# pixray/pixray

Hardware: AMD Instinct MI355X
Metric: optimisation iters/sec, VQGAN 256^2 + ViT-B/32 + 64 cutouts (higher is better)
Workload: dtype fp16

## Files before the change

### include/prx.h

```cpp
#ifndef PRX_H_
#define PRX_H_
#include <stddef.h>
#include <stdint.h>

#ifdef __cplusplus
extern "C" {
#endif

#define PRX_ABI_VERSION 3

typedef void* prx_stream_t;

const char* prx_last_error(void);
int prx_abi_version(void);
int prx_device_info(int* cu_count, char* arch_name, int arch_name_len);


#define PRX_ACT_NONE 0
#define PRX_ACT_QUICKGELU 1
#define PRX_ACT_MUL_DQUICKGELU 2
#define PRX_ACT_RELU 3
#define PRX_ACT_MUL_RELUMASK 4
#define PRX_ACT_RELUMASK_POST 5
#define PRX_ACT_GELU 6
// ... 38 lines not shown
long long prx_gemm_row_launches(void);

int prx_k_groupnorm_fwd(const float* x, const float* gamma, const float* beta, double* stats, void* out_bf16,
                        float* out_f32, int NB, int P, int C, int swish, float eps, prx_stream_t s);
int prx_k_groupnorm_bwd(const float* g, const float* x, const float* gamma, const float* beta, const double* fstats,
                        double* bstats, const float* add, float* dx, int NB, int P, int C, int swish, float eps,
                        prx_stream_t s);
int prx_k_layernorm_fwd(const float* x, long long ldx, const float* gamma, const float* beta, void* out_bf16,
                        float* out_f32, float* mean, float* rstd, int rows, int C, float eps, prx_stream_t s);
int prx_k_layernorm_bwd(const float* g, long long ldg, const float* x, long long ldx, const float* gamma,
                        const float* mean, const float* rstd, const float* add, long long ldadd, float* dx,
                        long long lddx, int rows, int C, prx_stream_t s);
int prx_k_transpose_bf16(const void* in, int ldin, void* out, int ldout, int R, int C, prx_stream_t s);
int prx_k_softmax_rows(const float* S, int lds_, float scale, void* P, int ldp, void* PT, int ldpt, int rows, int cols,
                       prx_stream_t s);
int prx_k_softmax_rows_bwd(const void* P, int ldp, const float* dP, int lddp, float scale, void* dS, int ldds,
                           void* dST, int lddst, int rows, int cols, prx_stream_t s);
int prx_k_upsample2x_bwd(const float* hi, float* low, int NB, int Hl, int Wl, int C, prx_stream_t s);
int prx_k_nchw_to_nhwc(const float* in, float* out_f32, void* out_bf16, int NB, int C, int HW, int Cpad,
                       prx_stream_t s);
int prx_k_nhwc_to_nchw(const float* in, int ldc, float* out, int NB, int C, int HW, prx_stream_t s);
int prx_k_image_head_fwd(const float* x, int ldc, float* img, int NB, int C, int HW, prx_stream_t s);
int prx_k_image_head_bwd(const float* x, int ldc, const float* gimg, float* dx, void* dx_bf16, int ldo, int NB, int C,
                         int HW, prx_stream_t s);
int prx_k_mha_fwd(const void* qkv, void* out, int N, int T, int C, int heads, prx_stream_t s);
int prx_k_mha_bwd(const void* qkv, const void* dout, void* dqkv, int N, int T, int C, int heads, prx_stream_t s);

int prx_k_groupnorm_fwd_op(const void* x, const float* gamma, const float* beta, double* stats, void* out16, float* out_f32,
                           int NB, int P, int C, int swish, float eps, int zero_stats, int stats_ready, int h16, int s16,
                           prx_stream_t s);
int prx_k_groupnorm_bwd_op(const void* g, const void* x, const float* gamma, const float* beta, const double* fstats,
                           double* bstats, const void* add, float* dx, void* dx16, int NB, int P, int C, int swish, float eps,
                           int zero_stats, int stats_ready, int h16, int s16, prx_stream_t s);
int prx_k_layernorm_fwd_op(const void* x, long long ldx, const float* gamma, const float* beta, void* out16, float* out_f32,
                           float* mean, float* rstd, int rows, int C, float eps, int h16, int s16, prx_stream_t s);
int prx_k_layernorm_bwd_op(const void* g, long long ldg, const void* x, long long ldx, const float* gamma, const float* mean,
                           const float* rstd, const void* add, long long ldadd, float* dx, long long lddx, void* dx16,
                           long long lddxb, int rows, int C, int h16, int add_every, int s16, prx_stream_t s);
int prx_k_mha_fwd_op(const void* qkv, void* out, int N, int T, int C, int heads, int h16, prx_stream_t s);
int prx_k_mha_bwd_op(const void* qkv, const void* dout, void* dqkv, int N, int T, int C, int heads, int h16, prx_stream_t s);
int prx_k_mha_fwd_gen_op(const void* qkv, void* out, float* lse, int N, int T, int C, int heads, int h16, prx_stream_t s);
int prx_k_mha_bwd_gen_op(const void* qkv, const void* out, const void* dout, const float* lse, void* dqkv, int N, int T, int C,
                         int heads, int h16, prx_stream_t s);
int prx_k_mha_fwd_hd_op(const void* qkv, void* out, float* lse, int N, int T, int C, int heads, int h16, int head_cols, prx_stream_t s);
int prx_k_mha_bwd_hd_op(const void* qkv, const void* out, const void* dout, const float* lse, void* dqkv, int N, int T, int C,
                        int heads, int h16, int head_cols, prx_stream_t s);
int prx_k_vit_pad_heads(const float* qkv_w, float* qkv_w_pad, const float* out_w, float* out_w_pad, int width, int heads, int hd, int hp,
                        prx_stream_t s);
int prx_k_mha_fwd_causal_op(const void* qkv, void* out, int N, int T, int C, int heads, int h16, prx_stream_t s);
int prx_k_softmax_rows_op(const float* S, int lds_, float scale, void* P, int ldp, void* PT, int ldpt, int rows, int cols,
                          int prec, prx_stream_t s);
int prx_k_softmax_rows_bwd_op(const void* P, int ldp, const float* dP, int lddp, float scale, void* dS, int ldds, void* dST,
                              int lddst, int rows, int cols, int prec, prx_stream_t s);
int prx_k_transpose_op(const void* in, int ldin, void* out, int ldout, int R, int C, int f32, prx_stream_t s);
int prx_k_upsample2x_bwd_op(const void* hi, float* low, void* low16, int NB, int Hl, int Wl, int C, int h16, int s16,
                            prx_stream_t s);
int prx_k_nchw_to_nhwc_op(const float* in, float* out_f32, void* out16, int NB, int C, int HW, int Cpad, int h16, prx_stream_t s);
int prx_k_image_head_bwd_op(const float* x, int ldc, const float* gimg, float* dx, void* dx16, int ldo, int NB, int C, int HW,
                            int h16, const float* gscale, prx_stream_t s);
int prx_k_image_head_bwd_im2col(const float* x, int ldc, const float* gimg, void* col, int ldk, int C, int H, int W, int h16,
                                const float* gscale, prx_stream_t s);
int prx_k_grad_scale(const float* g, size_t n, float* part, int nparts, int target_log2, float* scale2, prx_stream_t s);
int prx_k_grad_scale_multi(const float* const* gs, const size_t* ns, int count, float* part, int nparts_each, int target_log2,
                           float* scale2, prx_stream_t s);
int prx_k_scale_dev(float* x, size_t n, const float* scale, void* out16, int h16, prx_stream_t s);
int prx_k_f32_to_op16(const float* in, void* out16, size_t n, int h16, prx_stream_t s);
int prx_k_add_f32(const float* a, const float* b, float* out, size_t n, prx_stream_t s);

int prx_k_rn_pack_conv3x3(const float* w, void* Wf, void* Wd, int Cout, int Cin, int prec, prx_stream_t s);
int prx_k_stem1_fwd(const float* cut, const float* mm, const float* w, const float* b, void* out, int N, int S, int CO, int prec,
                    prx_stream_t s);
int prx_k_stem1_bwd(const void* g, const float* w, float* dY, int N, int S, int CO, const float* oscale_dev, int prec, prx_stream_t s);
int prx_k_avgpool2_fwd(const void* x, void* out, int N, int H, int W, int C, int prec, prx_stream_t s);
int prx_k_avgpool2_bwd(const float* g, const void* mask, float* dx_f32, void* dx_op, int N, int H, int W, int C, int prec,
                       prx_stream_t s);
int prx_k_relu_mask(float* g, const void* out, void* g_op, size_t n, int prec, prx_stream_t s);
int prx_k_tokens_fwd(const float* x, const float* pos, void* t, int N, int P, int C, int prec, prx_stream_t s);
int prx_k_tokens_bwd(const float* dt, float* dx, int N, int P, int C, int prec, prx_stream_t s);
int prx_k_tok0_gather(const void* t, void* out, int N, int T, int C, int prec, prx_stream_t s);
int prx_k_tok0_scatter(const void* g0, void* dt, int N, int T, int C, int prec, prx_stream_t s);
int prx_k_minmax(const float* x, size_t n, float* part, int nparts, float* mm, prx_stream_t s);
int prx_k_patchify_fwd(const float* cut, const float* mm, void* A, int prec, int N, int S, int P, int T, float m0, float m1, float m2,
                       float s0, float s1, float s2, prx_stream_t s);
int prx_k_patchify_bwd_reduce(const float* cut, const float* mm, const float* dA, double* acc, int N, int S, int P, int T, float m0,
                              float m1, float m2, float s0, float s1, float s2, prx_stream_t s);
int prx_k_patchify_bwd_apply(const float* cut, const float* mm, const float* dA, const double* acc, float* gcut, int N, int S, int P,
                             int T, float m0, float m1, float m2, float s0, float s1, float s2, prx_stream_t s);
int prx_k_preproc_bwd_reduce(const float* cut, const float* mm, const float* dY, double* acc, int N, int S, prx_stream_t s);
int prx_k_preproc_bwd_apply(const float* cut, const float* mm, const float* dY, const double* acc, float* gcut, int N, int S,
                            prx_stream_t s);
int prx_k_pool_fwd(const float* img, float* pooled, int* argmax, const unsigned char* mask, int C, int H, int W, int S, prx_stream_t s);
int prx_k_pool_bwd(const float* g, const int* argmax, const unsigned char* mask, float* gimg, int C, int H, int W, int S, prx_stream_t s);
int prx_k_rescale_fwd(const float* pooled, float* base, int C, int S, int Hb, int Wb, prx_stream_t s);
int prx_k_rescale_bwd(const float* g_base, float* g_pooled, int C, int S, int Hb, int Wb, prx_stream_t s);
int prx_k_warp_a_fwd(const float* src, int Hs, int Ws, const double* desc, float* out, int n_cut, int Ha, int Wa, prx_stream_t s);
// ... 323 lines not shown
```

### pixray_amd/csrc/api_kernels.hip

```cpp
#include "common.h"
#include "norms.h"
#include "elementwise.h"
#include "attention.h"
#include "resnet.h"
#include "cutouts.h"
#include "vgg.h"
#include "vit.h"
#include "clip_text.h"
#include "prompt_vq.h"
#include "vqgan.h"
#include "vqgan_enc.h"
#include "../../include/prx.h"

#define S_(x) ((hipStream_t)(x))
#define B_(x) ((bf16_t*)(x))
#define CB_(x) ((const bf16_t*)(x))

extern "C" {

int prx_k_groupnorm_fwd(const float* x, const float* gamma, const float* beta, double* stats, void* out_bf16,
                        float* out_f32, int NB, int P, int C, int swish, float eps, prx_stream_t s) {
    return prx_groupnorm_fwd(x, gamma, beta, stats, B_(out_bf16), out_f32, NB, P, C, swish, eps, S_(s));
}
int prx_k_groupnorm_bwd(const float* g, const float* x, const float* gamma, const float* beta, const double* fstats,
// ... 42 lines not shown
    return prx_mha_fwd(CB_(qkv), B_(out), N, T, C, heads, S_(s));
}
int prx_k_mha_bwd(const void* qkv, const void* dout, void* dqkv, int N, int T, int C, int heads, prx_stream_t s) {
    return prx_mha_bwd(CB_(qkv), CB_(dout), B_(dqkv), N, T, C, heads, S_(s));
}

int prx_k_mha_fwd_gen(const void* qkv, void* out, float* lse, int N, int T, int C, int heads, prx_stream_t s) {
    return prx_mha_fwd_gen(CB_(qkv), B_(out), lse, N, T, C, heads, S_(s));
}
int prx_k_mha_bwd_gen(const void* qkv, const void* out, const void* dout, const float* lse, void* dqkv, int N, int T, int C,
                      int heads, prx_stream_t s) {
    return prx_mha_bwd_gen(CB_(qkv), CB_(out), CB_(dout), lse, B_(dqkv), N, T, C, heads, S_(s));
}

int prx_k_mha_fwd_f32(const float* qkv, float* out, float* lse, int N, int T, int C, int heads, prx_stream_t s) {
    return prx_mha_fwd_f32(qkv, out, lse, N, T, C, heads, S_(s));
}
int prx_k_mha_bwd_f32(const float* qkv, const float* out, const float* dout, const float* lse, float* dqkv, int N, int T, int C,
                      int heads, prx_stream_t s) {
    return prx_mha_bwd_f32(qkv, out, dout, lse, dqkv, N, T, C, heads, S_(s));
}

int prx_k_groupnorm_fwd_op(const void* x, const float* gamma, const float* beta, double* stats, void* out16, float* out_f32,
                           int NB, int P, int C, int swish, float eps, int zero_stats, int stats_ready, int h16, int s16,
                           prx_stream_t s) {
    return prx_groupnorm_fwd(x, gamma, beta, stats, B_(out16), out_f32, NB, P, C, swish, eps, S_(s), zero_stats, stats_ready, h16, s16);
}
int prx_k_groupnorm_bwd_op(const void* g, const void* x, const float* gamma, const float* beta, const double* fstats,
                           double* bstats, const void* add, float* dx, void* dx16, int NB, int P, int C, int swish, float eps,
                           int zero_stats, int stats_ready, int h16, int s16, prx_stream_t s) {
    return prx_groupnorm_bwd(g, x, gamma, beta, fstats, bstats, add, dx, B_(dx16), NB, P, C, swish, eps, S_(s), zero_stats,
                             stats_ready, h16, s16);
}
int prx_k_layernorm_fwd_op(const void* x, long long ldx, const float* gamma, const float* beta, void* out16, float* out_f32,
                           float* mean, float* rstd, int rows, int C, float eps, int h16, int s16, prx_stream_t s) {
    return prx_layernorm_fwd(x, ldx, gamma, beta, B_(out16), out_f32, mean, rstd, rows, C, eps, S_(s), h16, s16);
}
int prx_k_layernorm_bwd_op(const void* g, long long ldg, const void* x, long long ldx, const float* gamma, const float* mean,
                           const float* rstd, const void* add, long long ldadd, float* dx, long long lddx, void* dx16,
                           long long lddxb, int rows, int C, int h16, int add_every, int s16, prx_stream_t s) {
    return prx_layernorm_bwd(g, ldg, x, ldx, gamma, mean, rstd, add, ldadd, dx, lddx, B_(dx16), lddxb, rows, C, S_(s), h16,
                             add_every, s16);
}
int prx_k_mha_fwd_op(const void* qkv, void* out, int N, int T, int C, int heads, int h16, prx_stream_t s) {
    return prx_mha_fwd(CB_(qkv), B_(out), N, T, C, heads, S_(s), h16);
}
int prx_k_mha_bwd_op(const void* qkv, const void* dout, void* dqkv, int N, int T, int C, int heads, int h16, prx_stream_t s) {
    return prx_mha_bwd(CB_(qkv), CB_(dout), B_(dqkv), N, T, C, heads, S_(s), h16);
}
int prx_k_mha_fwd_gen_op(const void* qkv, void* out, float* lse, int N, int T, int C, int heads, int h16, prx_stream_t s) {
    return prx_mha_fwd_gen(CB_(qkv), B_(out), lse, N, T, C, heads, S_(s), h16);
}
int prx_k_mha_bwd_gen_op(const void* qkv, const void* out, const void* dout, const float* lse, void* dqkv, int N, int T, int C,
                         int heads, int h16, prx_stream_t s) {
    return prx_mha_bwd_gen(CB_(qkv), CB_(out), CB_(dout), lse, B_(dqkv), N, T, C, heads, S_(s), h16);
}
int prx_k_mha_fwd_hd_op(const void* qkv, void* out, float* lse, int N, int T, int C, int heads, int h16, int head_cols, prx_stream_t s) {
    PRX_REQUIRE(head_cols == 64 || head_cols == 96, "mha_fwd_hd: %d columns per head (64 | 96)", head_cols);
    if (head_cols == 64) return prx_mha_fwd_gen(CB_(qkv), B_(out), lse, N, T, C, heads, S_(s), h16);
    return prx_mha_fwd_hd96(CB_(qkv), B_(out), lse, N, T, C, heads, 1.f / sqrtf(80.f), S_(s), h16);
}
int prx_k_mha_bwd_hd_op(const void* qkv, const void* out, const void* dout, const float* lse, void* dqkv, int N, int T, int C,
                        int heads, int h16, int head_cols, prx_stream_t s) {
    PRX_REQUIRE(head_cols == 64 || head_cols == 96, "mha_bwd_hd: %d columns per head (64 | 96)", head_cols);
    if (head_cols == 64) return prx_mha_bwd_gen(CB_(qkv), CB_(out), CB_(dout), lse, B_(dqkv), N, T, C, heads, S_(s), h16);
    return prx_mha_bwd_hd96(CB_(qkv), CB_(out), CB_(dout), lse, B_(dqkv), N, T, C, heads, 1.f / sqrtf(80.f), S_(s), h16);
}
int prx_k_vit_pad_heads(const float* qkv_w, float* qkv_w_pad, const float* out_w, float* out_w_pad, int width, int heads, int hd, int hp,
                        prx_stream_t s) {
    PRX_REQUIRE(qkv_w && qkv_w_pad && out_w && out_w_pad && width == heads * hd, "vit_pad_heads: null argument or width != heads * head dim");
    int r = prx_vit_pad_head_rows(qkv_w, qkv_w_pad, heads, hd, hp, width, S_(s));
    return r ? r : prx_vit_pad_head_cols(out_w, out_w_pad, width, heads, hd, hp, S_(s));
}
int prx_k_mha_fwd_causal_op(const void* qkv, void* out, int N, int T, int C, int heads, int h16, prx_stream_t s) {
    return prx_mha_fwd_causal(CB_(qkv), B_(out), N, T, C, heads, S_(s), h16);
}
int prx_k_softmax_rows_op(const float* S, int lds_, float scale, void* P, int ldp, void* PT, int ldpt, int rows, int cols,
                          int prec, prx_stream_t s) {
    PRX_REQUIRE(prec_valid(prec), "softmax_rows: unknown precision %d", prec);
    return prx_softmax_rows(S, lds_, scale, P, ldp, PT, ldpt, rows, cols, prec, S_(s));
}
int prx_k_softmax_rows_bwd_op(const void* P, int ldp, const float* dP, int lddp, float scale, void* dS, int ldds, void* dST,
                              int lddst, int rows, int cols, int prec, prx_stream_t s) {
    PRX_REQUIRE(prec_valid(prec), "softmax_rows_bwd: unknown precision %d", prec);
    return prx_softmax_rows_bwd(P, ldp, dP, lddp, scale, dS, ldds, dST, lddst, rows, cols, prec, S_(s));
}
int prx_k_transpose_op(const void* in, int ldin, void* out, int ldout, int R, int C, int f32, prx_stream_t s) {
    return prx_transpose_op(in, ldin, out, ldout, R, C, f32, S_(s));
}
int prx_k_upsample2x_bwd_op(const void* hi, float* low, void* low16, int NB, int Hl, int Wl, int C, int h16, int s16,
                            prx_stream_t s) {
    return prx_upsample2x_bwd(hi, low, B_(low16), NB, Hl, Wl, C, S_(s), h16, s16);
}
int prx_k_nchw_to_nhwc_op(const float* in, float* out_f32, void* out16, int NB, int C, int HW, int Cpad, int h16, prx_stream_t s) {
    return prx_nchw_to_nhwc(in, out_f32, B_(out16), NB, C, HW, Cpad, S_(s), h16);
}
int prx_k_image_head_bwd_op(const float* x, int ldc, const float* gimg, float* dx, void* dx16, int ldo, int NB, int C, int HW,
                            int h16, const float* gscale, prx_stream_t s) {
    return prx_image_head_bwd(x, ldc, gimg, dx, B_(dx16), ldo, NB, C, HW, S_(s), h16, gscale);
}
int prx_k_image_head_bwd_im2col(const float* x, int ldc, const float* gimg, void* col, int ldk, int C, int H, int W, int h16,
                                const float* gscale, prx_stream_t s) {
    return prx_image_head_bwd_im2col(x, ldc, gimg, B_(col), ldk, C, H, W, S_(s), h16, gscale);
}
int prx_k_grad_scale(const float* g, size_t n, float* part, int nparts, int target_log2, float* scale2, prx_stream_t s) {
    return prx_grad_scale(g, n, part, nparts, target_log2, scale2, S_(s));
}
int prx_k_grad_scale_multi(const float* const* gs, const size_t* ns, int count, float* part, int nparts_each, int target_log2,
                           float* scale2, prx_stream_t s) {
    return prx_grad_scale_multi(gs, ns, count, part, nparts_each, target_log2, scale2, S_(s));
}
int prx_k_scale_dev(float* x, size_t n, const float* scale, void* out16, int h16, prx_stream_t s) {
    return prx_scale_dev(x, n, scale, S_(s), B_(out16), h16);
}
int prx_k_f32_to_op16(const float* in, void* out16, size_t n, int h16, prx_stream_t s) {
    return prx_f32_to_bf16(in, B_(out16), n, S_(s), h16);
}
int prx_k_add_f32(const float* a, const float* b, float* out, size_t n, prx_stream_t s) {
    return prx_add_f32(a, b, out, n, S_(s));
}

int prx_k_rn_pack_conv3x3(const float* w, void* Wf, void* Wd, int Cout, int Cin, int prec, prx_stream_t s) {
    return prx_rn_pack_conv3x3(w, Wf, Wd, Cout, Cin, prec, S_(s));
}
int prx_k_stem1_fwd(const float* cut, const float* mm, const float* w, const float* b, void* out, int N, int S, int CO, int prec, prx_stream_t s) {
    return prx_stem1_fwd(cut, mm, w, b, out, N, S, CO, prec, S_(s));
}
int prx_k_stem1_bwd(const void* g, const float* w, float* dY, int N, int S, int CO, const float* oscale_dev, int prec, prx_stream_t s) {
    return prx_stem1_bwd(g, w, dY, N, S, CO, oscale_dev, prec, S_(s));
}
int prx_k_avgpool2_fwd(const void* x, void* out, int N, int H, int W, int C, int prec, prx_stream_t s) {
    return prx_avgpool2_fwd(x, out, N, H, W, C, prec, S_(s));
}
int prx_k_avgpool2_bwd(const float* g, const void* mask, float* dx_f32, void* dx_op, int N, int H, int W, int C, int prec, prx_stream_t s) {
    return prx_avgpool2_bwd(g, mask, dx_f32, dx_op, N, H, W, C, prec, S_(s));
}
int prx_k_relu_mask(float* g, const void* out, void* g_op, size_t n, int prec, prx_stream_t s) {
    return prx_relu_mask(g, out, g_op, n, prec, S_(s));
}
int prx_k_tokens_fwd(const float* x, const float* pos, void* t, int N, int P, int C, int prec, prx_stream_t s) {
// ... 125 lines not shown
```

### pixray_amd/csrc/attention.h

```cpp
#pragma once
#include "common.h"
int prx_mha_fwd(const bf16_t* qkv, bf16_t* out, int N, int T, int C, int heads, hipStream_t s, int h16 = 0);
int prx_mha_bwd(const bf16_t* qkv, const bf16_t* dout, bf16_t* dqkv, int N, int T, int C, int heads, hipStream_t s, int h16 = 0);
int prx_mha_fwd_gen(const bf16_t* qkv, bf16_t* out, float* lse, int N, int T, int C, int heads, hipStream_t s, int h16 = 0);
int prx_mha_bwd_gen(const bf16_t* qkv, const bf16_t* out, const bf16_t* dout, const float* lse, bf16_t* dqkv, int N, int T,
                    int C, int heads, hipStream_t s, int h16 = 0);
int prx_mha_fwd_causal(const bf16_t* qkv, bf16_t* out, int N, int T, int C, int heads, hipStream_t s, int h16 = 0);
int prx_mha_fwd_f32(const float* qkv, float* out, float* lse, int N, int T, int C, int heads, hipStream_t s);
int prx_mha_bwd_f32(const float* qkv, const float* out, const float* dout, const float* lse, float* dqkv, int N, int T, int C,
                    int heads, hipStream_t s);
int prx_mha_fwd_hd96(const bf16_t* qkv, bf16_t* out, float* lse, int N, int T, int C, int heads, float scale, hipStream_t s, int h16 = 0);
int prx_mha_bwd_hd96(const bf16_t* qkv, const bf16_t* out, const bf16_t* dout, const float* lse, bf16_t* dqkv, int N, int T, int C,
                     int heads, float scale, hipStream_t s, int h16 = 0);
int prx_mha_fwd_f32_hd96(const float* qkv, float* out, float* lse, int N, int T, int C, int heads, hipStream_t s);
int prx_mha_bwd_f32_hd96(const float* qkv, const float* out, const float* dout, const float* lse, float* dqkv, int N, int T, int C,
                         int heads, hipStream_t s);
```

### pixray_amd/csrc/attention.hip

```cpp
#include "attention.h"
#include <stdlib.h>
#include <atomic>

constexpr int MHA_BLK_MAX_T = 640;
static std::atomic<int> g_mha_route{-1};
extern "C" int prx_mha_route(int route) { return g_mha_route.exchange(route < 0 ? -1 : (route ? 1 : 0)); }
static bool prx_mha_blk_route(int T) {
    static const bool env_tiles = [] { const char* e = getenv("PRX_MHA_TILES"); return e && e[0] == '1'; }();
    const int route = g_mha_route.load(std::memory_order_relaxed);
    return T <= MHA_BLK_MAX_T && route != 1 && !(route < 0 && env_tiles);
}

#define A16_NS att_bf16
#define a16_t bf16_t
#define a16x8 bf16x8
#define a16x4 bf16x4
#define A16_MFMA __builtin_amdgcn_mfma_f32_32x32x16_bf16
#include "attention_kernels.inc"
#undef A16_NS
#undef a16_t
#undef a16x8
#undef a16x4
#undef A16_MFMA

#define A16_NS att_f16
#define a16_t half_t
#define a16x8 f16x8
#define a16x4 f16x4
#define A16_MFMA __builtin_amdgcn_mfma_f32_32x32x16_f16
#include "attention_kernels.inc"
#undef A16_NS
#undef a16_t
#undef a16x8
#undef a16x4
#undef A16_MFMA

#define H(p) reinterpret_cast<const half_t*>(p)
#define HM(p) reinterpret_cast<half_t*>(p)
int prx_mha_fwd(const bf16_t* qkv, bf16_t* out, int N, int T, int C, int heads, hipStream_t s, int h16) {
    return h16 ? att_f16::mha_fwd(H(qkv), HM(out), N, T, C, heads, s) : att_bf16::mha_fwd(qkv, out, N, T, C, heads, s);
}
int prx_mha_bwd(const bf16_t* qkv, const bf16_t* dout, bf16_t* dqkv, int N, int T, int C, int heads, hipStream_t s, int h16) {
    return h16 ? att_f16::mha_bwd(H(qkv), H(dout), HM(dqkv), N, T, C, heads, s) : att_bf16::mha_bwd(qkv, dout, dqkv, N, T, C, heads, s);
}
int prx_mha_fwd_gen(const bf16_t* qkv, bf16_t* out, float* lse, int N, int T, int C, int heads, hipStream_t s, int h16) {
    return h16 ? att_f16::mha_fwd_gen(H(qkv), HM(out), lse, N, T, C, heads, s) : att_bf16::mha_fwd_gen(qkv, out, lse, N, T, C, heads, s);
}
int prx_mha_fwd_causal(const bf16_t* qkv, bf16_t* out, int N, int T, int C, int heads, hipStream_t s, int h16) {
    return h16 ? att_f16::mha_fwd_causal(H(qkv), HM(out), N, T, C, heads, s) : att_bf16::mha_fwd_causal(qkv, out, N, T, C, heads, s);
}
int prx_mha_bwd_gen(const bf16_t* qkv, const bf16_t* out, const bf16_t* dout, const float* lse, bf16_t* dqkv, int N, int T,
                    int C, int heads, hipStream_t s, int h16) {
    return h16 ? att_f16::mha_bwd_gen(H(qkv), H(out), H(dout), lse, HM(dqkv), N, T, C, heads, s)
               : att_bf16::mha_bwd_gen(qkv, out, dout, lse, dqkv, N, T, C, heads, s);
}
```

### pixray_amd/csrc/attention_kernels.inc

```
namespace A16_NS {
namespace {

constexpr int LD = 72;
constexpr int TILE = 64 * LD;

__device__ __forceinline__ float half_max(float v) {
#pragma unroll
    for (int o = 16; o > 0; o >>= 1) v = fmaxf(v, __shfl_xor(v, o, 64));
    return v;
}
__device__ __forceinline__ float half_sum(float v) {
#pragma unroll
    for (int o = 16; o > 0; o >>= 1) v += __shfl_xor(v, o, 64);
    return v;
}

__device__ __forceinline__ void mma_64x64x64(const a16_t* A, const a16_t* B, f32x16 (&acc)[2][2], int lane) {
    const int fr = lane & 31, fk = 8 * (lane >> 5);
#pragma unroll
    for (int ks = 0; ks < 4; ++ks) {
        a16x8 a[2], b[2];
#pragma unroll
        for (int i = 0; i < 2; ++i) {
            a[i] = *reinterpret_cast<const a16x8*>(&A[(i * 32 + fr) * LD + ks * 16 + fk]);
            b[i] = *reinterpret_cast<const a16x8*>(&B[(i * 32 + fr) * LD + ks * 16 + fk]);
        }
#pragma unroll
        for (int i = 0; i < 2; ++i)
#pragma unroll
            for (int j = 0; j < 2; ++j) acc[i][j] = A16_MFMA(a[i], b[j], acc[i][j], 0, 0, 0);
    }
}

__device__ __forceinline__ void zero_acc(f32x16 (&acc)[2][2]) {
#pragma unroll
    for (int i = 0; i < 2; ++i)
#pragma unroll
        for (int j = 0; j < 2; ++j)
#pragma unroll
            for (int r = 0; r < 16; ++r) acc[i][j][r] = 0.f;
}

__device__ __forceinline__ int tr_swz(int d) { return (((d >> 4) & 1) * 12) ^ (((d >> 5) & 1) * 16); }

__device__ __forceinline__ void tile_get(const a16_t* src, long long ld, int T, int tid, a16x8 (&v)[4]) {
#pragma unroll
    for (int i = 0; i < 4; ++i) {
        const int c = tid + 128 * i;
        const int row = c >> 3, kc = c & 7;
        const a16x8 z = {0, 0, 0, 0, 0, 0, 0, 0};
        const a16x8 x = *reinterpret_cast<const a16x8*>(src + (long long)(row < T ? row : T - 1) * ld + kc * 8);
        v[i] = row < T ? x : z;
    }
}
__device__ __forceinline__ void tile_put(const a16x8 (&v)[4], a16_t* dst, a16_t* dstT, int tid) {
#pragma unroll
    for (int i = 0; i < 4; ++i) {
        const int c = tid + 128 * i;
        const int row = c >> 3, kc = c & 7;
        if (dst) *reinterpret_cast<a16x8*>(&dst[row * LD + kc * 8]) = v[i];
        if (dstT) {
#pragma unroll
            for (int e = 0; e < 8; ++e) dstT[(kc * 8 + e) * LD + (row ^ tr_swz(kc * 8))] = v[i][e];
        }
    }
}

__device__ __forceinline__ void mma_64x32x64(const a16_t* A, const a16_t* B, int nb, f32x16 (&acc)[2], int lane) {
    const int fr = lane & 31, fk = 8 * (lane >> 5);
#pragma unroll
    for (int ks = 0; ks < 4; ++ks) {
        const a16x8 b = *reinterpret_cast<const a16x8*>(&B[(nb * 32 + fr) * LD + ks * 16 + fk]);
#pragma unroll
        for (int i = 0; i < 2; ++i) {
            const a16x8 a = *reinterpret_cast<const a16x8*>(&A[(i * 32 + fr) * LD + ks * 16 + fk]);
            acc[i] = A16_MFMA(a, b, acc[i], 0, 0, 0);
        }
    }
}
__device__ __forceinline__ void zero_acc2(f32x16 (&acc)[2]) {
#pragma unroll
    for (int i = 0; i < 2; ++i)
#pragma unroll
        for (int r = 0; r < 16; ++r) acc[i][r] = 0.f;
}
// ... 107 lines not shown
        float m = -INFINITY;
#pragma unroll
        for (int mi = 0; mi < 2; ++mi)
#pragma unroll
            for (int r = 0; r < 16; ++r) {
                const int j = mi * 32 + (r & 3) + 8 * (r >> 2) + 4 * hh;
                const float v = (j < T) ? st[mi][r] * scale : -INFINITY;
                st[mi][r] = v;
                m = fmaxf(m, v);
            }
        m = fmaxf(m, __shfl_xor(m, 32, 64));
        float sum = 0.f;
#pragma unroll
        for (int mi = 0; mi < 2; ++mi)
#pragma unroll
            for (int r = 0; r < 16; ++r) {
                const float e = __expf(st[mi][r] - m);
                st[mi][r] = e;
                sum += e;
            }
        sum += __shfl_xor(sum, 32, 64);
        const float inv = 1.f / sum;
#pragma unroll
        for (int mi = 0; mi < 2; ++mi)
#pragma unroll
            for (int r = 0; r < 16; ++r) st[mi][r] *= inv;
    }
    f32x16 o[2];
    zero_acc2(o);
    mma_acc_tr(st, Vt, o, lane);
    store_rows_global(o, w, out + (long long)n * T * C + h * 64, C, T, lane);
}

__global__ __launch_bounds__(128) void mha_bwd_kernel(const a16_t* __restrict__ qkv, const a16_t* __restrict__ dout,
                                                      a16_t* __restrict__ dqkv, int T, int C, float scale, int xcd) {
    __shared__ __attribute__((aligned(16))) a16_t smem[5 * TILE];
    __shared__ __attribute__((aligned(16))) float s_lse[64], s_D[64];
    a16_t* Qs = smem;
    a16_t* Ks = smem + TILE;
    a16_t* Vs = smem + 2 * TILE;
    a16_t* dOs = smem + 3 * TILE;
    a16_t* Tt = smem + 4 * TILE;
    const int tid = threadIdx.x, lane = tid & 63, w = tid >> 6;
    const unsigned flat = blockIdx.y * gridDim.x + blockIdx.x, nwg = gridDim.x * gridDim.y;
    const unsigned lin = xcd ? xcd_linear(flat, nwg) : flat;
    const int h = (int)(lin % gridDim.x), n = (int)(lin / gridDim.x);
    const int hh = lane >> 5;
    const long long ld = 3LL * C;
    const a16_t* base = qkv + (long long)n * T * ld + h * 64;
    const a16_t* dobase = dout + (long long)n * T * C + h * 64;
    a16x8 tq[4], tdo[4];
    {
        a16x8 tk[4], tv[4];
        tile_get(base, ld, T, tid, tq);
        tile_get(base + C, ld, T, tid, tk);
        tile_get(base + 2 * C, ld, T, tid, tv);
        tile_get(dobase, C, T, tid, tdo);
        tile_put(tq, Qs, nullptr, tid);
        tile_put(tk, Ks, Tt, tid);
        tile_put(tv, Vs, nullptr, tid);
        tile_put(tdo, dOs, nullptr, tid);
    }
    __syncthreads();
    a16_t* obase = dqkv + (long long)n * T * ld + h * 64;
    {
        f32x16 pt[2], dpt[2];
        zero_acc2(pt);
        mma_64x32x64(Ks, Qs, w, pt, lane);
        zero_acc2(dpt);
        mma_64x32x64(Vs, dOs, w, dpt, lane);
        float m = -INFINITY;
#pragma unroll
        for (int mi = 0; mi < 2; ++mi)
#pragma unroll
            for (int r = 0; r < 16; ++r) {
                const int j = mi * 32 + (r & 3) + 8 * (r >> 2) + 4 * hh;
                const float v = (j < T) ? pt[mi][r] * scale : -INFINITY;
                pt[mi][r] = v;
                m = fmaxf(m, v);
            }
        m = fmaxf(m, __shfl_xor(m, 32, 64));
        float sum = 0.f;
#pragma unroll
        for (int mi = 0; mi < 2; ++mi)
#pragma unroll
            for (int r = 0; r < 16; ++r) {
                const float e = __expf(pt[mi][r] - m);
                pt[mi][r] = e;
                sum += e;
            }
// ... 560 lines not shown
            for (int rg = 0; rg < 4; ++rg) {
                const int i0 = sb * 32 + 8 * rg + 4 * hh;
                const float4 l4 = *reinterpret_cast<const float4*>(&s_lse[i0]);
                const float4 d4 = *reinterpret_cast<const float4*>(&s_D[i0]);
                const float lv[4] = {l4.x, l4.y, l4.z, l4.w}, dvv[4] = {d4.x, d4.y, d4.z, d4.w};
#pragma unroll
                for (int qq = 0; qq < 4; ++qq) {
                    const int r = rg * 4 + qq;
                    const float pv = key_ok ? __builtin_amdgcn_exp2f(p[r] * sl2 - lv[qq]) : 0.f;
                    p[r] = pv;
                    dp[r] = scale * pv * (dp[r] - dvv[qq]);
                }
            }
            mma_acc_tr_chunk(dp, Qt, sb, dk, lane);
            mma_acc_tr_chunk(p, dOt, sb, dv, lane);
        }
    }
    if (!active) return;
    a16_t* obase = dqkv + (long long)n * T * ld + h * 64;
    store_rows_global(dk, w, obase + C, ld, T, lane);
    store_rows_global(dv, w, obase + 2 * C, ld, T, lane);
}

}


inline int mha_fwd(const a16_t* qkv, a16_t* out, int N, int T, int C, int heads, hipStream_t s) {
    PRX_REQUIRE(T <= 64 && C == heads * 64, "mha: needs T <= 64 and head dim 64 (T=%d C=%d heads=%d)", T, C, heads);
    hipLaunchKernelGGL(mha_fwd_kernel, dim3(heads, N), dim3(128), 0, s, qkv, out, T, C, 0.125f, prx_xcd_local());
    PRX_LAUNCH_CHECK();
    return 0;
}

inline int mha_bwd(const a16_t* qkv, const a16_t* dout, a16_t* dqkv, int N, int T, int C, int heads, hipStream_t s) {
    PRX_REQUIRE(T <= 64 && C == heads * 64, "mha bwd: needs T <= 64 and head dim 64 (T=%d C=%d heads=%d)", T, C, heads);
    hipLaunchKernelGGL(mha_bwd_kernel, dim3(heads, N), dim3(128), 0, s, qkv, dout, dqkv, T, C, 0.125f, prx_xcd_local());
    PRX_LAUNCH_CHECK();
    return 0;
}

inline int mha_fwd_gen(const a16_t* qkv, a16_t* out, float* lse, int N, int T, int C, int heads, hipStream_t s) {
    PRX_REQUIRE(C == heads * 64 && T >= 1, "mha(gen): needs head dim 64 (T=%d C=%d heads=%d)", T, C, heads);
    if (prx_mha_blk_route(T)) {
        const int nw = ceil_div(T, 32), nsplit = ceil_div(nw, 5), wpb = ceil_div(nw, nsplit);
        hipLaunchKernelGGL(mha_fwd_blk_kernel, dim3(heads, N, nsplit), dim3(64 * wpb), 0, s, qkv, out, lse, T, C, heads, 0.125f, prx_xcd_local());
        PRX_LAUNCH_CHECK();
        return 0;
    }
    hipLaunchKernelGGL(mha_fwd_gen_kernel<false>, dim3(ceil_div(T, 64), heads, N), dim3(64), 0, s, qkv, out, lse, T, C, heads, 0.125f);
    PRX_LAUNCH_CHECK();
    return 0;
}
inline int mha_fwd_causal(const a16_t* qkv, a16_t* out, int N, int T, int C, int heads, hipStream_t s) {
    PRX_REQUIRE(C == heads * 64 && T >= 1, "mha(causal): needs head dim 64 (T=%d C=%d heads=%d)", T, C, heads);
    hipLaunchKernelGGL(mha_fwd_gen_kernel<true>, dim3(ceil_div(T, 64), heads, N), dim3(64), 0, s, qkv, out, (float*)nullptr, T, C, heads,
                       0.125f);
    PRX_LAUNCH_CHECK();
    return 0;
}
inline int mha_bwd_gen(const a16_t* qkv, const a16_t* out, const a16_t* dout, const float* lse, a16_t* dqkv, int N, int T,
                    int C, int heads, hipStream_t s) {
    PRX_REQUIRE(C == heads * 64 && T >= 1, "mha(gen) bwd: needs head dim 64 (T=%d C=%d heads=%d)", T, C, heads);
    if (prx_mha_blk_route(T)) {
        const int nw = ceil_div(T, 32), nsplit = ceil_div(nw, 5), wpb = ceil_div(nw, nsplit);
        const dim3 g(heads, N, nsplit), b(64 * wpb);
        const int xcd = prx_xcd_local();
        hipLaunchKernelGGL(mha_bwd_dq_blk_kernel, g, b, 0, s, qkv, out, dout, lse, dqkv, T, C, heads, 0.125f, xcd);
        PRX_LAUNCH_CHECK();
        hipLaunchKernelGGL(mha_bwd_dkv_blk_kernel, g, b, 0, s, qkv, out, dout, lse, dqkv, T, C, heads, 0.125f, xcd);
// ... 13 lines not shown
```

### pixray_amd/csrc/common.h

```cpp
#pragma once
#include <hip/hip_runtime.h>
#include <stdint.h>

typedef __bf16 bf16_t;
typedef _Float16 half_t;
typedef __attribute__((ext_vector_type(8))) _Float16 f16x8;
typedef __attribute__((ext_vector_type(4))) _Float16 f16x4;
typedef __attribute__((ext_vector_type(8))) __bf16 bf16x8;
typedef __attribute__((ext_vector_type(4))) __bf16 bf16x4;
typedef __attribute__((ext_vector_type(2))) __bf16 bf16x2;
typedef __attribute__((ext_vector_type(16))) float f32x16;
typedef __attribute__((ext_vector_type(4))) float f32x4;

#define PRX_WAVE 64

enum { PRX_PREC_BF16 = 0, PRX_PREC_F32 = 1, PRX_PREC_F16 = 2 };
static inline int prec_is_f32(int precision) { return precision == PRX_PREC_F32; }
static inline int prec_is_h16(int precision) { return precision == PRX_PREC_F16; }
static inline bool prec_valid(int precision) { return precision >= PRX_PREC_BF16 && precision <= PRX_PREC_F16; }
static inline size_t op_esz(int f32) { return f32 ? 4 : 2; }
static inline void* op_off(void* p, size_t elems, int f32) { return p ? (char*)p + elems * op_esz(f32) : nullptr; }
static inline const void* op_off(const void* p, size_t elems, int f32) { return p ? (const char*)p + elems * op_esz(f32) : nullptr; }

void prx_set_error(const char* fmt, ...);
// ... 110 lines not shown
template <> __device__ __forceinline__ void op_st4<float>(float* p, size_t i, float a, float b, float c, float d) {
    *reinterpret_cast<float4*>(p + i) = make_float4(a, b, c, d);
}

__device__ __forceinline__ float wave_sum(float v) {
#pragma unroll
    for (int o = 32; o > 0; o >>= 1) v += __shfl_xor(v, o, 64);
    return v;
}
__device__ __forceinline__ float wave_max(float v) {
#pragma unroll
    for (int o = 32; o > 0; o >>= 1) v = fmaxf(v, __shfl_xor(v, o, 64));
    return v;
}
__device__ __forceinline__ float wave_min(float v) {
#pragma unroll
    for (int o = 32; o > 0; o >>= 1) v = fminf(v, __shfl_xor(v, o, 64));
    return v;
}
__device__ __forceinline__ double wave_sum_d(double v) {
#pragma unroll
    for (int o = 32; o > 0; o >>= 1) v += __shfl_xor(v, o, 64);
    return v;
}

__device__ __forceinline__ float sigmoidf_(float x) { return 1.f / (1.f + __expf(-x)); }

__device__ __forceinline__ unsigned xcd_linear(unsigned bid, unsigned nwg) {
    const unsigned xcd = bid & 7u, local = bid >> 3, q = nwg >> 3, r = nwg & 7u;
    return (xcd < r ? xcd * (q + 1) : r * (q + 1) + (xcd - r) * q) + local;
}
int prx_xcd_local();
int prx_grad_target_log2();

static inline int ceil_div(int a, int b) { return (a + b - 1) / b; }
static inline long long ceil_div_ll(long long a, long long b) { return (a + b - 1) / b; }
```

### pixray_amd/csrc/elementwise.h

```cpp
#pragma once
#include "common.h"
int prx_transpose_op(const void* in, int ldin, void* out, int ldout, int R, int C, int f32, hipStream_t s);
int prx_softmax_rows(const float* S, int lds_, float scale, void* P, int ldp, void* PT, int ldpt, int rows,
                     int cols, int prec, hipStream_t s);
int prx_softmax_rows_bwd(const void* P, int ldp, const float* dP, int lddp, float scale, void* dS, int ldds,
                         void* dST, int lddst, int rows, int cols, int prec, hipStream_t s);
int prx_upsample2x_bwd(const void* hi, float* low, bf16_t* low_bf16, int NB, int Hl, int Wl, int C, hipStream_t s, int h16 = 0, int s16 = 0);
int prx_nchw_to_nhwc(const float* in, float* out_f32, bf16_t* out_bf16, int NB, int C, int HW, int Cpad, hipStream_t s, int h16 = 0);
int prx_nhwc_to_nchw(const float* in, int ldc, float* out, int NB, int C, int HW, hipStream_t s);
int prx_image_head_fwd(const float* x, int ldc, float* img, int NB, int C, int HW, hipStream_t s);
int prx_image_head_bwd(const float* x, int ldc, const float* gimg, float* dx, bf16_t* dx_bf16, int ldo, int NB, int C,
                       int HW, hipStream_t s, int h16 = 0, const float* gscale = nullptr);
int prx_image_head_bwd_im2col(const float* x, int ldc, const float* gimg, bf16_t* col, int ldk, int C, int H, int W, hipStream_t s, int h16 = 0,
                              const float* gscale = nullptr);
int prx_grad_scale(const float* g, size_t n, float* part, int nparts, int target_log2, float* scale2, hipStream_t s);
int prx_adam_clamp(float* z, float* m, float* v, const float* g, const float* zmin, const float* zmax, int hw,
                   size_t n, float lr, float b1, float b2, float eps, int step, hipStream_t s);
int prx_adam_clamp_dev(float* z, float* m, float* v, const float* g, const float* zmin, const float* zmax, int hw,
                       size_t n, const float* hyper, float b1, float b2, float eps, hipStream_t s);
int prx_f32_to_bf16(const float* in, bf16_t* out, size_t n, hipStream_t s, int h16 = 0);
int prx_grad_scale_multi(const float* const* gs, const size_t* ns, int count, float* part, int nparts_each, int target_log2,
                         float* scale2, hipStream_t s);
int prx_add_f32(const float* a, const float* b, float* out, size_t n, hipStream_t s);
int prx_scale_dev(float* x, size_t n, const float* scale, hipStream_t s, bf16_t* out16 = nullptr, int h16 = 0);
```

### pixray_amd/csrc/elementwise.hip

```cpp
#include "elementwise.h"
#include <algorithm>

namespace {

inline int ew_grid(size_t total, int per = 256) { return (int)std::min<size_t>((total + per - 1) / per, 8192); }

template <typename T>
__global__ __launch_bounds__(256) void transpose_op_kernel(const T* __restrict__ in, int ldin,
                                                           T* __restrict__ out, int ldout, int R, int C) {
    __shared__ T tile[32][33];
    const int tx = threadIdx.x & 31, ty = threadIdx.x >> 5;
    const int r0 = blockIdx.y * 32, c0 = blockIdx.x * 32;
#pragma unroll
    for (int i = 0; i < 4; ++i) {
        int r = r0 + ty + 8 * i, c = c0 + tx;
        tile[ty + 8 * i][tx] = (r < R && c < C) ? in[(size_t)r * ldin + c] : (T)0.f;
    }
    __syncthreads();
#pragma unroll
    for (int i = 0; i < 4; ++i) {
        int c = c0 + ty + 8 * i, r = r0 + tx;
        if (c < C && r < R) out[(size_t)c * ldout + r] = tile[tx][ty + 8 * i];
    }
}
// ... 185 lines not shown
        }
        z[i] = zi;
    }
}

__global__ __launch_bounds__(256) void f32_to_bf16_kernel(const float* __restrict__ in, bf16_t* __restrict__ out,
                                                          size_t n, int h16) {
    for (size_t i = (size_t)blockIdx.x * blockDim.x + threadIdx.x; i < n; i += (size_t)gridDim.x * blockDim.x)
        out[i] = to_op16(in[i], h16);
}

__global__ __launch_bounds__(256) void amax_partial_kernel(const float* __restrict__ g, size_t n, float* __restrict__ part) {
    float m = 0.f;
    for (size_t i = (size_t)blockIdx.x * blockDim.x + threadIdx.x; i < n; i += (size_t)gridDim.x * blockDim.x) {
        const float a = fabsf(g[i]);
        m = fmaxf(m, a == a ? a : INFINITY);
    }
    m = wave_max(m);
    __shared__ float s[4];
    if ((threadIdx.x & 63) == 0) s[threadIdx.x >> 6] = m;
    __syncthreads();
    if (threadIdx.x == 0) part[blockIdx.x] = fmaxf(fmaxf(s[0], s[1]), fmaxf(s[2], s[3]));
}
__global__ __launch_bounds__(256) void grad_scale_final_kernel(const float* __restrict__ part, int nparts, int target_log2,
                                                               float* __restrict__ scale2) {
    float m = 0.f;
    for (int i = threadIdx.x; i < nparts; i += blockDim.x) m = fmaxf(m, part[i]);
    m = wave_max(m);
    __shared__ float s[4];
    if ((threadIdx.x & 63) == 0) s[threadIdx.x >> 6] = m;
    __syncthreads();
    if (threadIdx.x == 0) {
        m = fmaxf(fmaxf(s[0], s[1]), fmaxf(s[2], s[3]));
        float S = 1.f;
        if (m > 0.f && m < INFINITY) {
            int e;
            (void)frexpf(m, &e);
            int k = target_log2 - e;
            k = k < -40 ? -40 : (k > 60 ? 60 : k);
            S = ldexpf(1.f, k);
        }
        scale2[0] = S;
        scale2[1] = 1.f / S;
    }
}

__global__ __launch_bounds__(256) void scale_dev_kernel(float* __restrict__ x, size_t n, const float* __restrict__ scale, bf16_t* __restrict__ out16, int h16) {
    const float sc = *scale;
    for (size_t i = (size_t)blockIdx.x * blockDim.x + threadIdx.x; i < n; i += (size_t)gridDim.x * blockDim.x) {
        const float v = x[i] * sc;
        x[i] = v;
        if (out16) out16[i] = to_op16(v, h16);
    }
}

__global__ __launch_bounds__(256) void add_f32_kernel(const float* __restrict__ a, const float* __restrict__ b,
                                                      float* __restrict__ out, size_t n) {
    for (size_t i = (size_t)blockIdx.x * blockDim.x + threadIdx.x; i < n; i += (size_t)gridDim.x * blockDim.x)
        out[i] = a[i] + b[i];
}

}

int prx_transpose_op(const void* in, int ldin, void* out, int ldout, int R, int C, int f32, hipStream_t s) {
    dim3 grid(ceil_div(C, 32), ceil_div(R, 32));
    if (f32) hipLaunchKernelGGL(transpose_op_kernel<float>, grid, dim3(256), 0, s, (const float*)in, ldin, (float*)out, ldout, R, C);
    else     hipLaunchKernelGGL(transpose_op_kernel<bf16_t>, grid, dim3(256), 0, s, (const bf16_t*)in, ldin, (bf16_t*)out, ldout, R, C);
    PRX_LAUNCH_CHECK();
    return 0;
}
int prx_softmax_rows(const float* S, int lds_, float scale, void* P, int ldp, void* PT, int ldpt, int rows,
                     int cols, int prec, hipStream_t s) {
    PRX_OP_DISPATCH(prec_is_f32(prec), prec_is_h16(prec), T,
                    hipLaunchKernelGGL(softmax_rows_kernel<T>, dim3(ceil_div(rows, 4)), dim3(256), 0, s, S, lds_, scale, (T*)P, ldp,
// ... 7 lines not shown
                    hipLaunchKernelGGL(softmax_rows_bwd_kernel<T>, dim3(ceil_div(rows, 4)), dim3(256), 0, s, (const T*)P, ldp, dP, lddp,
                                       scale, (T*)dS, ldds, (T*)dST, lddst, rows, cols));
    PRX_LAUNCH_CHECK();
    return 0;
}
int prx_upsample2x_bwd(const void* hi, float* low, bf16_t* low_bf16, int NB, int Hl, int Wl, int C, hipStream_t s, int h16, int s16) {
    PRX_REQUIRE(C % 4 == 0 && (low || low_bf16), "upsample2x_bwd: C %% 4 != 0, or no output");
    if (s16) hipLaunchKernelGGL(upsample2x_bwd_kernel<true>, dim3(ew_grid((size_t)NB * Hl * Wl * C / 4)), dim3(256), 0, s, hi, low, low_bf16,
                                NB, Hl, Wl, C, h16);
    else hipLaunchKernelGGL(upsample2x_bwd_kernel<false>, dim3(ew_grid((size_t)NB * Hl * Wl * C / 4)), dim3(256), 0, s, hi, low, low_bf16,
                            NB, Hl, Wl, C, h16);
    PRX_LAUNCH_CHECK();
    return 0;
}
int prx_nchw_to_nhwc(const float* in, float* out_f32, bf16_t* out_bf16, int NB, int C, int HW, int Cpad,
                     hipStream_t s, int h16) {
    hipLaunchKernelGGL(nchw_to_nhwc_kernel, dim3(ew_grid((size_t)NB * HW * Cpad)), dim3(256), 0, s, in, out_f32,
                       out_bf16, NB, C, HW, Cpad, h16);
    PRX_LAUNCH_CHECK();
    return 0;
}
int prx_nhwc_to_nchw(const float* in, int ldc, float* out, int NB, int C, int HW, hipStream_t s) {
    hipLaunchKernelGGL(nhwc_to_nchw_kernel, dim3(ew_grid((size_t)NB * HW * C)), dim3(256), 0, s, in, ldc, out, NB, C,
                       HW);
    PRX_LAUNCH_CHECK();
    return 0;
}
int prx_image_head_fwd(const float* x, int ldc, float* img, int NB, int C, int HW, hipStream_t s) {
    hipLaunchKernelGGL(image_head_fwd_kernel, dim3(ew_grid((size_t)NB * HW * C)), dim3(256), 0, s, x, ldc, img, NB, C,
                       HW);
    PRX_LAUNCH_CHECK();
    return 0;
}
int prx_grad_scale(const float* g, size_t n, float* part, int nparts, int target_log2, float* scale2, hipStream_t s) {
    PRX_REQUIRE(nparts >= 1 && nparts <= 1024, "grad_scale: 1..1024 partials");
    const int blocks = (int)std::min<size_t>((n + 1023) / 1024 + 1, (size_t)nparts);
    hipLaunchKernelGGL(amax_partial_kernel, dim3(blocks), dim3(256), 0, s, g, n, part);
    PRX_LAUNCH_CHECK();
    hipLaunchKernelGGL(grad_scale_final_kernel, dim3(1), dim3(256), 0, s, part, blocks, target_log2, scale2);
    PRX_LAUNCH_CHECK();
    return 0;
}
int prx_grad_scale_multi(const float* const* gs, const size_t* ns, int count, float* part, int nparts_each, int target_log2,
                         float* scale2, hipStream_t s) {
    PRX_REQUIRE(count >= 1 && nparts_each >= 1 && (long long)count * nparts_each <= 4096, "grad_scale_multi: bad partial layout");
    int used = 0;
    for (int i = 0; i < count; ++i) {
        if (!gs[i] || ns[i] == 0) continue;
        const int blocks = (int)std::min<size_t>((ns[i] + 1023) / 1024 + 1, (size_t)nparts_each);
        hipLaunchKernelGGL(amax_partial_kernel, dim3(blocks), dim3(256), 0, s, gs[i], ns[i], part + used);
        PRX_LAUNCH_CHECK();
        used += blocks;
    }
    PRX_REQUIRE(used > 0, "grad_scale_multi: no gradient tensor");
    hipLaunchKernelGGL(grad_scale_final_kernel, dim3(1), dim3(256), 0, s, part, used, target_log2, scale2);
    PRX_LAUNCH_CHECK();
    return 0;
}
int prx_scale_dev(float* x, size_t n, const float* scale, hipStream_t s, bf16_t* out16, int h16) {
    hipLaunchKernelGGL(scale_dev_kernel, dim3(ew_grid(n)), dim3(256), 0, s, x, n, scale, out16, h16);
    PRX_LAUNCH_CHECK();
    return 0;
}
int prx_image_head_bwd(const float* x, int ldc, const float* gimg, float* dx, bf16_t* dx_bf16, int ldo, int NB, int C,
                       int HW, hipStream_t s, int h16, const float* gscale) {
    hipLaunchKernelGGL(image_head_bwd_kernel, dim3(ew_grid((size_t)NB * HW * ldo)), dim3(256), 0, s, x, ldc, gimg, dx,
                       dx_bf16, ldo, NB, C, HW, h16, gscale);
    PRX_LAUNCH_CHECK();
    return 0;
// ... 38 lines not shown
```

### pixray_amd/csrc/norms.h

```cpp
#pragma once
#include "common.h"
#include <algorithm>
int prx_groupnorm_fwd(const void* x, const float* gamma, const float* beta, double* stats, bf16_t* out_bf16,
                      float* out_f32, int NB, int P, int C, int swish, float eps, hipStream_t s, int zero_stats = 1,
                      int stats_ready = 0, int h16 = 0, int s16 = 0);
int prx_groupnorm_bwd(const void* g, const void* x, const float* gamma, const float* beta, const double* fstats,
                      double* bstats, const void* add, float* dx, bf16_t* dx_bf16, int NB, int P, int C, int swish,
                      float eps, hipStream_t s, int zero_stats = 1, int stats_ready = 0, int h16 = 0, int s16 = 0);
int prx_groupnorm_bwd_stats(const float* g, const float* x, const float* gamma, const float* beta, const double* fstats,
                            double* bstats, int NB, int P, int C, int swish, float eps, hipStream_t s);
int prx_layernorm_fwd(const void* x, long long ldx, const float* gamma, const float* beta, bf16_t* out_bf16,
                      float* out_f32, float* mean, float* rstd, int rows, int C, float eps, hipStream_t s, int h16 = 0, int s16 = 0,
                      int ragged = 0);
int prx_layernorm_bwd(const void* g, long long ldg, const void* x, long long ldx, const float* gamma,
                      const float* mean, const float* rstd, const void* add, long long ldadd, float* dx,
                      long long lddx, bf16_t* dx_bf16, long long lddxb, int rows, int C, hipStream_t s, int h16 = 0,
                      int add_every = 0, int s16 = 0, int ragged = 0);
```

### pixray_amd/csrc/norms.hip

```cpp
#include "norms.h"

namespace {

struct GNArgs {
    const void* x;
    const void* g;
    const double* fstats;
    const float* gamma;
    const float* beta;
    double* stats;
    int P, C, swish;
    float eps;
    int s16, h16;
};

__device__ __forceinline__ void gn_mean_rstd(const double* st, double n, float eps, float& mean, float& rstd) {
    double m = st[0] / n;
    double var = st[1] / n - m * m;
    if (var < 0) var = 0;
    mean = (float)m;
    rstd = (float)(1.0 / sqrt(var + (double)eps));
}

__device__ __forceinline__ float swish_grad(float y) {
// ... 154 lines not shown
    L.ga = reinterpret_cast<const float4*>(a.gamma)[cq];
    L.be = reinterpret_cast<const float4*>(a.beta)[cq];
    gn_lane_load<true>(a, bstats, NB == 1 ? 0 : (int)(i0 / per_b), cq, L);
    auto one = [&](unsigned id, const float4& v, const float4& gg, const float4& ad) {
        if (NB != 1) { const int b = (int)(id / per_b); if (b != L.b) gn_lane_load<true>(a, bstats, b, cq, L); }
        const float xv[4] = {v.x, v.y, v.z, v.w}, gv[4] = {gg.x, gg.y, gg.z, gg.w};
        const float gav[4] = {L.ga.x, L.ga.y, L.ga.z, L.ga.w}, bev[4] = {L.be.x, L.be.y, L.be.z, L.be.w};
        float o[4];
#pragma unroll
        for (int i = 0; i < 4; ++i) {
            float xh = (xv[i] - L.mean) * L.rstd;
            float gy = gv[i];
            if (a.swish) gy *= swish_grad(xh * gav[i] + bev[i]);
            float dxh = gy * gav[i];
            o[i] = L.rstd * (dxh - L.m1 - xh * L.m2);
        }
        o[0] += ad.x; o[1] += ad.y; o[2] += ad.z; o[3] += ad.w;
        if (dx) reinterpret_cast<float4*>(dx)[id] = make_float4(o[0], o[1], o[2], o[3]);
        if (dx_bf16) reinterpret_cast<bf16x4*>(dx_bf16)[id] = to_op16x4(o[0], o[1], o[2], o[3], h16);
    };
    for (; idx + step < i1; idx += 2 * step) {
        const unsigned nx = idx + 2 * step;
        const bool m0 = nx < i1, m1 = nx + step < i1;
        const float4 nv0 = m0 ? stream_ld4<S16>(a.x, nx, a.h16) : z4, ng0 = m0 ? stream_ld4<S16>(a.g, nx, a.h16) : z4;
        const float4 na0 = (m0 && add) ? stream_ld4<S16>(add, nx, a.h16) : z4;
        const float4 nv1 = m1 ? stream_ld4<S16>(a.x, nx + step, a.h16) : z4, ng1 = m1 ? stream_ld4<S16>(a.g, nx + step, a.h16) : z4;
        const float4 na1 = (m1 && add) ? stream_ld4<S16>(add, nx + step, a.h16) : z4;
        one(idx, v0, g0, a0); one(idx + step, v1, g1, a1);
        v0 = nv0; g0 = ng0; a0 = na0; v1 = nv1; g1 = ng1; a1 = na1;
    }
    if (idx < i1) one(idx, v0, g0, a0);
}

template <bool RAG>
__device__ __forceinline__ bool ln_own(int i, int nv, int lane, int C) {
    return RAG ? (i * 64 + lane) * 4 < C : i < nv;
}
template <int MAXV, bool S16, bool RAG = false>
__global__ __launch_bounds__(256) void ln_fwd_kernel(const void* __restrict__ x, const float* __restrict__ gamma,
                                                     const float* __restrict__ beta, bf16_t* __restrict__ out_bf16,
                                                     float* __restrict__ out_f32, float* __restrict__ mean_out,
                                                     float* __restrict__ rstd_out, int rows, int C, long long ldx,
                                                     float eps, int xcd, int h16) {
    const int lane = threadIdx.x & 63;
    const int row = (xcd ? xcd_linear(blockIdx.x, gridDim.x) : blockIdx.x) * 4 + (threadIdx.x >> 6);
    if (row >= rows) return;
    const int nv = (C + 255) >> 8;
    const size_t xr4 = (size_t)row * ldx / 4;
    float4 v[MAXV], gav[MAXV], bev[MAXV];
#pragma unroll
    for (int i = 0; i < MAXV; ++i) v[i] = stream_ld4<S16>(x, xr4 + (ln_own<RAG>(i, nv, lane, C) ? i * 64 + lane : (RAG ? 0 : lane)), h16);
#pragma unroll
    for (int i = 0; i < MAXV; ++i) {
        gav[i] = reinterpret_cast<const float4*>(gamma)[(ln_own<RAG>(i, nv, lane, C) ? i * 64 + lane : (RAG ? 0 : lane))];
        bev[i] = reinterpret_cast<const float4*>(beta)[(ln_own<RAG>(i, nv, lane, C) ? i * 64 + lane : (RAG ? 0 : lane))];
    }
    float s = 0.f;
#pragma unroll
    for (int i = 0; i < MAXV; ++i) s += ln_own<RAG>(i, nv, lane, C) ? (v[i].x + v[i].y) + (v[i].z + v[i].w) : 0.f;
    const float mean = wave_sum(s) / (float)C;
    float ss = 0.f;
#pragma unroll
    for (int i = 0; i < MAXV; ++i)
        if (ln_own<RAG>(i, nv, lane, C)) {
            float a0 = v[i].x - mean, a1 = v[i].y - mean, a2 = v[i].z - mean, a3 = v[i].w - mean;
            ss += (a0 * a0 + a1 * a1) + (a2 * a2 + a3 * a3);
        }
    const float var = wave_sum(ss) / (float)C;
    const float rstd = rsqrtf(var + eps);
    if (lane == 0) {
        if (mean_out) mean_out[row] = mean;
        if (rstd_out) rstd_out[row] = rstd;
    }
#pragma unroll
    for (int i = 0; i < MAXV; ++i)
        if (ln_own<RAG>(i, nv, lane, C)) {
            const int c4 = i * 64 + lane;
            const float4 ga = gav[i], be = bev[i];
            float o0 = (v[i].x - mean) * rstd * ga.x + be.x;
            float o1 = (v[i].y - mean) * rstd * ga.y + be.y;
            float o2 = (v[i].z - mean) * rstd * ga.z + be.z;
            float o3 = (v[i].w - mean) * rstd * ga.w + be.w;
            if (out_bf16) {
                reinterpret_cast<bf16x4*>(out_bf16 + (size_t)row * C)[c4] = to_op16x4(o0, o1, o2, o3, h16);
// ... 34 lines not shown
        for (int i = 0; i < MAXV; ++i) {
            xh[i] = make_float4((xv[i].x - mean) * rstd, (xv[i].y - mean) * rstd, (xv[i].z - mean) * rstd, (xv[i].w - mean) * rstd);
            dh[i] = make_float4(gv[i].x * ga[i].x, gv[i].y * ga[i].y, gv[i].z * ga[i].z, gv[i].w * ga[i].w);
        }
    }
    float s1 = 0.f, s2 = 0.f;
#pragma unroll
    for (int i = 0; i < MAXV; ++i) {
        s1 += ln_own<RAG>(i, nv, lane, C) ? (dh[i].x + dh[i].y) + (dh[i].z + dh[i].w) : 0.f;
        s2 += ln_own<RAG>(i, nv, lane, C) ? (dh[i].x * xh[i].x + dh[i].y * xh[i].y) + (dh[i].z * xh[i].z + dh[i].w * xh[i].w) : 0.f;
    }
    const float m1 = wave_sum(s1) / (float)C;
    const float m2 = wave_sum(s2) / (float)C;
#pragma unroll
    for (int i = 0; i < MAXV; ++i)
        if (ln_own<RAG>(i, nv, lane, C)) {
            const int c4 = i * 64 + lane;
            float4 o = make_float4(rstd * (dh[i].x - m1 - xh[i].x * m2), rstd * (dh[i].y - m1 - xh[i].y * m2),
                                   rstd * (dh[i].z - m1 - xh[i].z * m2), rstd * (dh[i].w - m1 - xh[i].w * m2));
            if (add) { o.x += adv[i].x; o.y += adv[i].y; o.z += adv[i].z; o.w += adv[i].w; }
            if (dx) reinterpret_cast<float4*>(dx + (size_t)row * lddx)[c4] = o;
            if (dx_bf16) {
                reinterpret_cast<bf16x4*>(dx_bf16 + (size_t)row * lddxb)[c4] = to_op16x4(o.x, o.y, o.z, o.w, h16);
            }
        }
}

int gn_grid(size_t total) { return (int)std::min<size_t>((total + 255) / 256, 2048); }

}

int prx_groupnorm_fwd(const void* x, const float* gamma, const float* beta, double* stats, bf16_t* out_bf16,
                      float* out_f32, int NB, int P, int C, int swish, float eps, hipStream_t s, int zero_stats,
                      int stats_ready, int h16, int s16) {
    PRX_REQUIRE(C % 32 == 0 && (C / 32) % 4 == 0 && 256 % (C / 4) == 0, "groupnorm: unsupported C=%d", C);
    GNArgs a{};
    a.x = x; a.gamma = gamma; a.beta = beta; a.stats = stats; a.P = P; a.C = C; a.swish = swish; a.eps = eps; a.s16 = s16; a.h16 = h16;
    if (!stats_ready) {
        if (zero_stats) PRX_CHECK_HIP(hipMemsetAsync(stats, 0, sizeof(double) * NB * 64, s));
        const int ppb = 256 / (C / 4);
        int blocks = std::min(ceil_div(P, ppb * 4), 256);
        if (s16) hipLaunchKernelGGL((gn_stats_kernel<0, true>), dim3(blocks, NB), dim3(256), 0, s, a);
        else hipLaunchKernelGGL((gn_stats_kernel<0, false>), dim3(blocks, NB), dim3(256), 0, s, a);
        PRX_LAUNCH_CHECK();
    }
    if (out_bf16 || out_f32) {
        PRX_REQUIRE((unsigned long long)NB * P * C / 4 < (1ull << 31), "groupnorm: %d x %d x %d elements exceed the 32-bit index range", NB, P, C);
        if (s16) hipLaunchKernelGGL(gn_apply_fwd_kernel<true>, dim3(gn_grid((size_t)NB * P * C / 4)), dim3(256), 0, s, a, out_bf16,
                                    out_f32, NB, prx_xcd_local(), h16);
        else hipLaunchKernelGGL(gn_apply_fwd_kernel<false>, dim3(gn_grid((size_t)NB * P * C / 4)), dim3(256), 0, s, a, out_bf16,
                                out_f32, NB, prx_xcd_local(), h16);
        PRX_LAUNCH_CHECK();
    }
    return 0;
}

int prx_groupnorm_bwd_stats(const float* g, const float* x, const float* gamma, const float* beta, const double* fstats,
                            double* bstats, int NB, int P, int C, int swish, float eps, hipStream_t s) {
    PRX_REQUIRE(256 % (C / 4) == 0 && (C / 32) % 4 == 0, "groupnorm bwd: unsupported C=%d", C);
    GNArgs a{};
    a.x = x; a.g = g; a.fstats = fstats; a.gamma = gamma; a.beta = beta; a.stats = bstats;
    a.P = P; a.C = C; a.swish = swish; a.eps = eps; a.s16 = 0; a.h16 = 0;
    const int ppb = 256 / (C / 4);
    int blocks = std::min(ceil_div(P, ppb * 4), 256);
    hipLaunchKernelGGL((gn_stats_kernel<1, false>), dim3(blocks, NB), dim3(256), 0, s, a);
    PRX_LAUNCH_CHECK();
    return 0;
}

int prx_groupnorm_bwd(const void* g, const void* x, const float* gamma, const float* beta, const double* fstats,
                      double* bstats, const void* add, float* dx, bf16_t* dx_bf16, int NB, int P, int C, int swish,
                      float eps, hipStream_t s, int zero_stats, int stats_ready, int h16, int s16) {
    PRX_REQUIRE(256 % (C / 4) == 0 && (C / 32) % 4 == 0, "groupnorm bwd: unsupported C=%d", C);
    GNArgs a{};
    a.x = x; a.g = g; a.fstats = fstats; a.gamma = gamma; a.beta = beta; a.stats = bstats;
    a.P = P; a.C = C; a.swish = swish; a.eps = eps; a.s16 = s16; a.h16 = h16;
    if (!stats_ready) {
        if (zero_stats) PRX_CHECK_HIP(hipMemsetAsync(bstats, 0, sizeof(double) * NB * 64, s));
        const int ppb = 256 / (C / 4);
        int blocks = std::min(ceil_div(P, ppb * 4), 256);
        if (s16) hipLaunchKernelGGL((gn_stats_kernel<1, true>), dim3(blocks, NB), dim3(256), 0, s, a);
        else hipLaunchKernelGGL((gn_stats_kernel<1, false>), dim3(blocks, NB), dim3(256), 0, s, a);
        PRX_LAUNCH_CHECK();
    }
    PRX_REQUIRE((unsigned long long)NB * P * C / 4 < (1ull << 31), "groupnorm bwd: %d x %d x %d elements exceed the 32-bit index range", NB, P, C);
    if (s16) hipLaunchKernelGGL(gn_apply_bwd_kernel<true>, dim3(gn_grid((size_t)NB * P * C / 4)), dim3(256), 0, s, a, bstats, add, dx,
                                dx_bf16, NB, prx_xcd_local(), h16);
    else hipLaunchKernelGGL(gn_apply_bwd_kernel<false>, dim3(gn_grid((size_t)NB * P * C / 4)), dim3(256), 0, s, a, bstats, add, dx,
                            dx_bf16, NB, prx_xcd_local(), h16);
    PRX_LAUNCH_CHECK();
    return 0;
}

int prx_layernorm_fwd(const void* x, long long ldx, const float* gamma, const float* beta, bf16_t* out_bf16,
                      float* out_f32, float* mean, float* rstd, int rows, int C, float eps, hipStream_t s, int h16, int s16, int ragged) {
    PRX_REQUIRE((C % 256 == 0 || (ragged && C % 128 == 0 && C <= 1024)) && C <= 2048 && ldx % 4 == 0,
                "layernorm: C must be a multiple of 256 and <= 2048 (C=%d), ldx a multiple of 4", C);
    dim3 grid(ceil_div(rows, 4));
    if (C % 256 != 0) {
#define PRX_LN_FWD_R(S16) hipLaunchKernelGGL((ln_fwd_kernel<4, S16, true>), grid, dim3(256), 0, s, x, gamma, beta, out_bf16, out_f32, mean, rstd, \
                                             rows, C, ldx, eps, prx_xcd_local(), h16)
        if (s16) PRX_LN_FWD_R(true); else PRX_LN_FWD_R(false);
#undef PRX_LN_FWD_R
        PRX_LAUNCH_CHECK();
        return 0;
    }
#define PRX_LN_FWD(MAXV, S16) hipLaunchKernelGGL((ln_fwd_kernel<MAXV, S16>), grid, dim3(256), 0, s, x, gamma, beta, out_bf16, out_f32, mean, rstd, \
                                                 rows, C, ldx, eps, prx_xcd_local(), h16)
    if (C <= 1024) { if (s16) PRX_LN_FWD(4, true); else PRX_LN_FWD(4, false); }
    else { if (s16) PRX_LN_FWD(8, true); else PRX_LN_FWD(8, false); }
#undef PRX_LN_FWD
    PRX_LAUNCH_CHECK();
    return 0;
}

int prx_layernorm_bwd(const void* g, long long ldg, const void* x, long long ldx, const float* gamma,
                      const float* mean, const float* rstd, const void* add, long long ldadd, float* dx,
                      long long lddx, bf16_t* dx_bf16, long long lddxb, int rows, int C, hipStream_t s, int h16, int add_every, int s16, int ragged) {
    PRX_REQUIRE((C % 256 == 0 || (ragged && C % 128 == 0 && C <= 1024)) && C <= 2048, "layernorm bwd: C must be a multiple of 256 and <= 2048 (C=%d)", C);
    PRX_REQUIRE(ldg % 4 == 0 && ldx % 4 == 0 && ldadd % 4 == 0 && (dx || dx_bf16), "layernorm bwd: leading dimensions must be multiples of 4, one output is needed");
    PRX_REQUIRE(s16 == 0 || s16 == 1 || s16 == 2 || s16 == 7, "layernorm bwd: stream layouts in use are 0, 1 (x), 2 (g), 7 (x, g, add): got %d", s16);
    dim3 grid(ceil_div(rows, 4));
    if (C % 256 != 0) {
#define PRX_LN_BWD_R(S16) hipLaunchKernelGGL((ln_bwd_kernel<4, S16, true>), grid, dim3(256), 0, s, g, ldg, x, ldx, gamma, mean, rstd, add, ldadd, dx, \
                                             lddx, dx_bf16, lddxb, rows, C, prx_xcd_local(), h16, add_every)
        if (s16 == 0) PRX_LN_BWD_R(0); else if (s16 == 1) PRX_LN_BWD_R(1); else if (s16 == 2) PRX_LN_BWD_R(2); else PRX_LN_BWD_R(7);
#undef PRX_LN_BWD_R
        PRX_LAUNCH_CHECK();
        return 0;
    }
#define PRX_LN_BWD(MAXV, S16) hipLaunchKernelGGL((ln_bwd_kernel<MAXV, S16>), grid, dim3(256), 0, s, g, ldg, x, ldx, gamma, mean, rstd, add, ldadd, dx, \
                                                 lddx, dx_bf16, lddxb, rows, C, prx_xcd_local(), h16, add_every)
#define PRX_LN_BWD_S(MAXV) do { if (s16 == 0) PRX_LN_BWD(MAXV, 0); else if (s16 == 1) PRX_LN_BWD(MAXV, 1); else if (s16 == 2) PRX_LN_BWD(MAXV, 2); \
                                else PRX_LN_BWD(MAXV, 7); } while (0)
    if (C <= 1024) PRX_LN_BWD_S(4); else PRX_LN_BWD_S(8);
#undef PRX_LN_BWD_S
#undef PRX_LN_BWD
    PRX_LAUNCH_CHECK();
    return 0;
}
```

### pixray_amd/csrc/prompt_vq.h

```cpp
#pragma once
#include "common.h"
int prx_prompt_loss(const float* x, const float* embed, int n, int m, int D, float weight, float stop, float denom,
                    float* rowloss, float* grad, float* loss, unsigned* ticket, hipStream_t s);
int prx_l2norm_fwd(const float* e, float* out, int n, int D, hipStream_t s);
int prx_l2norm_bwd(const float* e, const float* g, float* de, int n, int D, hipStream_t s);
int prx_sqnorm_rows(const float* w, float* out, int rows, int D, hipStream_t s);
int prx_vq_nearest(const float* z, long long tok_stride, long long ch_stride, const float* codebook, const float* cnorm,
                   int P, int NC, int D, float* pmin, int* pidx, int* idx_out, float* zq, hipStream_t s);
```

### pixray_amd/csrc/prompt_vq.hip

```cpp
#include "prompt_vq.h"
#include <algorithm>

namespace {

__device__ __forceinline__ float prompt_loss_row(const float* __restrict__ x, const float* __restrict__ embed, int i, int lane,
                                                int n, int m, int D, float weight, float stop, float denom,
                                                float* __restrict__ rowloss, float* __restrict__ grad) {
    constexpr int MAXE = 16;
    const int ne = D / 64;
    float xv[MAXE], gacc[MAXE];
    float ss = 0.f;
#pragma unroll
    for (int e = 0; e < MAXE; ++e) xv[e] = x[(size_t)i * D + (e < ne ? e : 0) * 64 + lane];
#pragma unroll
    for (int e = 0; e < MAXE; ++e)
        if (e < ne) { ss += xv[e] * xv[e]; gacc[e] = 0.f; }
    const float xnorm = fmaxf(sqrtf(wave_sum(ss)), 1e-12f);
    const float ixn = 1.f / xnorm;
    const float sgn = (weight > 0.f) ? 1.f : ((weight < 0.f) ? -1.f : 0.f);
    float loss = 0.f;
    for (int j = 0; j < m; ++j) {
        float ev[MAXE];
        float es = 0.f;
#pragma unroll
// ... 46 lines not shown
    if (!last || threadIdx.x >= 64) return;
    __threadfence();
    float t = 0.f;
    for (int r = lane; r < n; r += 64) t += *reinterpret_cast<const volatile float*>(rowloss + r);
    t = wave_sum(t);
    if (lane == 0) *loss_out = t * (fabsf(weight) / denom);
}

__global__ __launch_bounds__(256) void l2norm_fwd_kernel(const float* __restrict__ e, float* __restrict__ out, int n, int D) {
    const int lane = threadIdx.x & 63;
    const int i = blockIdx.x * 4 + (threadIdx.x >> 6);
    if (i >= n) return;
    float ss = 0.f;
    for (int c = lane; c < D; c += 64) { float v = e[(size_t)i * D + c]; ss += v * v; }
    const float inv = 1.f / sqrtf(wave_sum(ss));
    for (int c = lane; c < D; c += 64) out[(size_t)i * D + c] = e[(size_t)i * D + c] * inv;
}
__global__ __launch_bounds__(256) void l2norm_bwd_kernel(const float* __restrict__ e, const float* __restrict__ g,
                                                         float* __restrict__ de, int n, int D) {
    const int lane = threadIdx.x & 63;
    const int i = blockIdx.x * 4 + (threadIdx.x >> 6);
    if (i >= n) return;
    float ss = 0.f, dot = 0.f;
    for (int c = lane; c < D; c += 64) {
        float v = e[(size_t)i * D + c];
        ss += v * v; dot += v * g[(size_t)i * D + c];
    }
    ss = wave_sum(ss); dot = wave_sum(dot);
    const float inv = 1.f / sqrtf(ss);
    for (int c = lane; c < D; c += 64) {
        float v = e[(size_t)i * D + c];
        de[(size_t)i * D + c] = (g[(size_t)i * D + c] - v * dot / ss) * inv;
    }
}

__global__ __launch_bounds__(256) void sqnorm_rows_kernel(const float* __restrict__ w, float* __restrict__ out, int rows, int D) {
    const int lane = threadIdx.x & 63;
    const int i = blockIdx.x * 4 + (threadIdx.x >> 6);
    if (i >= rows) return;
    float ss = 0.f;
    for (int c = lane; c < D; c += 64) { float v = w[(size_t)i * D + c]; ss += v * v; }
    ss = wave_sum(ss);
    if (lane == 0) out[i] = ss;
}

typedef float vq_f32x2 __attribute__((ext_vector_type(2)));
constexpr int VQ_CODES = 128, VQ_CPAD = VQ_CODES + 4;
__global__ __launch_bounds__(256) void vq_dist_kernel(const float* __restrict__ z, long long tok_stride,
                                                      long long ch_stride, const float* __restrict__ codebook,
                                                      const float* __restrict__ cnorm, int P, int NC, int D,
                                                      float* __restrict__ pmin, int* __restrict__ pidx) {
    __shared__ __attribute__((aligned(16))) float Xs[16][64];
    __shared__ __attribute__((aligned(16))) float Cs[16][VQ_CPAD];
    __shared__ float red_v[64][16];
    __shared__ int red_i[64][16];
    const int tid = threadIdx.x;
    const int tx = tid & 15, ty = tid >> 4;
    const int p0 = blockIdx.y * 64, c0 = blockIdx.x * VQ_CODES;
    vq_f32x2 acc[4][4];
    float xn[4] = {0, 0, 0, 0};
#pragma unroll
    for (int i = 0; i < 4; ++i)
#pragma unroll
        for (int j = 0; j < 4; ++j) acc[i][j] = vq_f32x2{0.f, 0.f};
    float xr[4];
    float4 cr[2];
// ... 44 lines not shown
            }
        }
        __syncthreads();
    }
#pragma unroll
    for (int i = 0; i < 4; ++i) {
        float best = INFINITY; int bi = 0x7fffffff;
#pragma unroll
        for (int j = 0; j < 8; ++j) {
            const int c = c0 + (j < 4 ? tx * 4 + j : 64 + tx * 4 + (j - 4));
            if (c < NC) {
                const float a = (j & 1) ? acc[i][j >> 1].y : acc[i][j >> 1].x;
                float d = (xn[i] + cnorm[c]) - 2.f * a;
                if (d < best) { best = d; bi = c; }
            }
        }
        red_v[ty * 4 + i][tx] = best;
        red_i[ty * 4 + i][tx] = bi;
    }
    __syncthreads();
    if (tid < 64) {
        float best = red_v[tid][0]; int bi = red_i[tid][0];
        for (int j = 1; j < 16; ++j) {
            const float v = red_v[tid][j]; const int id = red_i[tid][j];
            if (v < best || (v == best && id < bi)) { best = v; bi = id; }
        }
        int p = p0 + tid;
        if (p < P) { pmin[(size_t)p * gridDim.x + blockIdx.x] = best; pidx[(size_t)p * gridDim.x + blockIdx.x] = bi; }
    }
}

__global__ __launch_bounds__(256) void vq_select_kernel(const float* __restrict__ pmin, const int* __restrict__ pidx,
                                                        int ntiles, const float* __restrict__ codebook, int D,
                                                        int* __restrict__ idx_out, float* __restrict__ zq, int P) {
    const int p = blockIdx.x;
    __shared__ float sv[256];
    __shared__ int si[256];
    float best = INFINITY; int bi = 0x7fffffff;
    for (int t = threadIdx.x; t < ntiles; t += blockDim.x) {
        float v = pmin[(size_t)p * ntiles + t]; int id = pidx[(size_t)p * ntiles + t];
        if (v < best || (v == best && id < bi)) { best = v; bi = id; }
    }
    sv[threadIdx.x] = best; si[threadIdx.x] = bi;
    __syncthreads();
    for (int o = 128; o > 0; o >>= 1) {
        if (threadIdx.x < o) {
            float v = sv[threadIdx.x + o]; int id = si[threadIdx.x + o];
            if (v < sv[threadIdx.x] || (v == sv[threadIdx.x] && id < si[threadIdx.x])) { sv[threadIdx.x] = v; si[threadIdx.x] = id; }
        }
        __syncthreads();
    }
    const int sel = si[0];
    if (threadIdx.x == 0 && idx_out) idx_out[p] = sel;
    for (int c = threadIdx.x; c < D; c += blockDim.x) zq[(size_t)p * D + c] = codebook[(size_t)sel * D + c];
}

}

int prx_prompt_loss(const float* x, const float* embed, int n, int m, int D, float weight, float stop, float denom,
                    float* rowloss, float* grad, float* loss, unsigned* ticket, hipStream_t s) {
    PRX_REQUIRE(D % 64 == 0 && D <= 1024, "prompt_loss: D must be a multiple of 64 and <= 1024 (D=%d)", D);
    PRX_REQUIRE(!loss || ticket, "prompt_loss: the scalar result needs a zeroed ticket word");
    hipLaunchKernelGGL(prompt_loss_kernel, dim3(ceil_div(n, 4)), dim3(256), 0, s, x, embed, n, m, D, weight, stop, denom,
                       rowloss, grad, loss, ticket);
    PRX_LAUNCH_CHECK();
    return 0;
}
int prx_l2norm_fwd(const float* e, float* out, int n, int D, hipStream_t s) {
    hipLaunchKernelGGL(l2norm_fwd_kernel, dim3(ceil_div(n, 4)), dim3(256), 0, s, e, out, n, D);
    PRX_LAUNCH_CHECK();
    return 0;
}
int prx_l2norm_bwd(const float* e, const float* g, float* de, int n, int D, hipStream_t s) {
    hipLaunchKernelGGL(l2norm_bwd_kernel, dim3(ceil_div(n, 4)), dim3(256), 0, s, e, g, de, n, D);
    PRX_LAUNCH_CHECK();
    return 0;
}
int prx_sqnorm_rows(const float* w, float* out, int rows, int D, hipStream_t s) {
    hipLaunchKernelGGL(sqnorm_rows_kernel, dim3(ceil_div(rows, 4)), dim3(256), 0, s, w, out, rows, D);
    PRX_LAUNCH_CHECK();
    return 0;
}
int prx_vq_nearest(const float* z, long long tok_stride, long long ch_stride, const float* codebook, const float* cnorm,
                   int P, int NC, int D, float* pmin, int* pidx, int* idx_out, float* zq, hipStream_t s) {
    PRX_REQUIRE(D % 16 == 0, "vq: D %% 16 != 0");
    PRX_REQUIRE(((uintptr_t)codebook & 15) == 0, "vq: the codebook must be 16-byte aligned");
    const int ntiles = ceil_div(NC, VQ_CODES);
    hipLaunchKernelGGL(vq_dist_kernel, dim3(ntiles, ceil_div(P, 64)), dim3(256), 0, s, z, tok_stride, ch_stride, codebook,
                       cnorm, P, NC, D, pmin, pidx);
    PRX_LAUNCH_CHECK();
    hipLaunchKernelGGL(vq_select_kernel, dim3(P), dim3(256), 0, s, pmin, pidx, ntiles, codebook, D, idx_out, zq, P);
    PRX_LAUNCH_CHECK();
    return 0;
}
```

### pixray_amd/csrc/vit.hip

```cpp
#include "vit.h"
#include <stdlib.h>
#include "gemm.h"
#include "norms.h"
#include "attention.h"
#include "cutouts.h"
#include "prompt_vq.h"
#include "elementwise.h"
#include "dev_arena.h"
#include <vector>
#include <memory>

namespace {

template <typename TOp>
__global__ __launch_bounds__(256) void pack_transpose_kernel(const float* __restrict__ in, TOp* __restrict__ out,
                                                             int R, int C) {
    __shared__ float tile[32][33];
    const int tx = threadIdx.x & 31, ty = threadIdx.x >> 5;
    const int r0 = blockIdx.y * 32, c0 = blockIdx.x * 32;
#pragma unroll
    for (int i = 0; i < 4; ++i) {
        int r = r0 + ty + 8 * i, c = c0 + tx;
        tile[ty + 8 * i][tx] = (r < R && c < C) ? in[(size_t)r * C + c] : 0.f;
    }
// ... 95 lines not shown
    PRX_REQUIRE(W >= 1 && heads >= 1 && hd >= 1 && hp >= hd, "pad_head_cols: %d heads of %d -> %d", heads, hd, hp);
    PRX_CHECK_HIP(hipMemsetAsync(dst, 0, sizeof(float) * (size_t)W * heads * hp, s));
    PRX_CHECK_HIP(hipMemcpy2DAsync(dst, sizeof(float) * hp, src, sizeof(float) * hd, sizeof(float) * hd, (size_t)W * heads, hipMemcpyDeviceToDevice, s));
    return 0;
}

struct VitLayer {
    float *ln1_g, *ln1_b, *bqkv, *bo, *ln2_g, *ln2_b, *b1, *b2;
    void *Wqkv, *WqkvT, *Wo, *WoT, *W1, *W1T, *W2, *W2T;
    void *x_in, *x_mid;
    float *mean1, *rstd1, *mean2, *rstd2;
    void *qkv, *t;
    void* o_save;
    float* lse;
};

struct PrxVit {
    int res, patch, width, layers, heads, out_dim, T, max_n, KP;
    int hd, hp, aw;
    int prec;
    int f32, h16;
    float* gs;
    GemmCtx gctx;
    DevArena mem;
    void *Wp, *WpT, *projT, *proj;
    float *cls, *pos, *lnpre_g, *lnpre_b, *lnpost_g, *lnpost_b;
    std::vector<VitLayer> L;
    void *A0, *h, *att_o, *u, *hpost, *dt, *do_, *dqkv, *dx_bf, *dh_bf, *de16;
    float *xpre, *mean_pre, *rstd_pre, *mean_post, *rstd_post, *e, *dx, *dh, *dA0, *de, *dhpost, *mm_part;
    void* x_final;
    int lean;
    VitFamily fam;
    float* bp;
    int cls_tail;
    float* ws; size_t ws_bytes;
    int cur_n;
};

namespace {
int pack_both(PrxVit* v, void** W, void** WT, const float* src, int out, int in, hipStream_t s) {
    DEV_ALLOC(v->mem, alloc_op, *W, (size_t)out * in, v->f32);
    DEV_ALLOC(v->mem, alloc_op, *WT, (size_t)out * in, v->f32);
    int r = prx_pack_op(src, *W, (size_t)out * in, v->prec, s);
    if (r) return r;
    return prx_pack_transpose_op(src, *WT, out, in, v->prec, s);
}
}

VitFamily prx_vit_family_clip() {
    VitFamily f;
    f.patch_bias = 0; f.ln_pre = 1; f.eps = 1e-5f; f.act = PRX_ACT_QUICKGELU; f.dact = PRX_ACT_MUL_DQUICKGELU;
    f.norm = prx_patch_norm_clip(); f.head_dim = 64;
    return f;
}

int prx_vit_create_impl(PrxVit** out, int res, int patch, int width, int layers, int heads, int out_dim, int max_n,
                        int precision, const float* const* w, int n_w, hipStream_t s, const VitFamily* family) {
    const VitFamily fam = family ? *family : prx_vit_family_clip();
    const int n_head = 3 + (fam.patch_bias ? 1 : 0) + (fam.ln_pre ? 2 : 0);
    PRX_REQUIRE(prec_valid(precision), "vit_create: unknown precision %d", precision);
    PRX_REQUIRE(n_w == n_head + 12 * layers + 3, "vit_create: expected %d weight tensors, got %d", n_head + 12 * layers + 3, n_w);
    const int hd = fam.head_dim > 0 ? fam.head_dim : 64;
    PRX_REQUIRE(res % patch == 0 && width == heads * hd && width % 128 == 0 && (hd == 64 || hd == 32 || hd == 16 || hd == 80),
                "vit_create: unsupported geometry (width %d, %d heads of %d)", width, heads, hd);
    PRX_REQUIRE(fam.ln_pre || layers >= 1, "vit_create: a tower without ln_pre needs at least one block");
    PRX_REQUIRE(fam.eps > 0.f && fam.norm.std[0] > 0.f && fam.norm.std[1] > 0.f && fam.norm.std[2] > 0.f,
                "vit_create: LayerNorm eps and the channel std must be positive");
    const int G = res / patch;
    const int T = G * G + 1;
    const int hp = hd == 80 ? 96 : 64;
    PRX_REQUIRE(hp == 64 || T <= 640 || prec_is_f32(precision), "vit_create: heads of %d run on the 96-wide attention kernels, which take at most 640 tokens (got %d)", hd, T);
    std::unique_ptr<PrxVit> guard(new PrxVit());
    PrxVit* v = guard.get();
    DevArena& m = v->mem;
    const int f32 = prec_is_f32(precision);
    v->mem.describe("vit_create", ": the runner keeps one forward's activations for max_batch = %d cutouts of %d tokens (width %d, %d layers)",
                    max_n, T, width, layers);
    v->T = T; v->max_n = max_n;
    v->res = res; v->patch = patch; v->width = width; v->layers = layers; v->heads = heads; v->out_dim = out_dim;
    v->prec = precision; v->f32 = prec_is_f32(precision); v->h16 = prec_is_h16(precision);
    v->gs = nullptr; v->fam = fam; v->bp = nullptr; v->hd = hd; v->hp = hp; v->aw = heads * hp;
    const int AW = v->aw;
    float *pad_w = nullptr, *pad_b = nullptr;
    if (hd != 64) {
        DEV_ALLOC(m, alloc, pad_w, (size_t)3 * AW * width);
        DEV_ALLOC(m, alloc, pad_b, (size_t)3 * AW);
    }
    { const char* e = getenv("PRX_LEAN"); v->lean = (v->h16 && !(e && atoi(e) == 0)) ? 1 : 0; }
    { const char* e = getenv("PRX_VIT_CLS_TAIL"); v->cls_tail = (e && atoi(e) == 0) ? 0 : 1; }
    v->T = T; v->max_n = max_n; v->KP = (3 * patch * patch + 7) / 8 * 8; v->cur_n = 0;
    const int W = width, KP = v->KP;
    int r;
    {
        const int K0 = 3 * patch * patch;
        float* padded;
        DEV_ALLOC(m, alloc, padded, (size_t)W * KP);
        PRX_CHECK_HIP(hipMemsetAsync(padded, 0, sizeof(float) * (size_t)W * KP, s));
        PRX_CHECK_HIP(hipMemcpy2DAsync(padded, sizeof(float) * KP, w[0], sizeof(float) * K0, sizeof(float) * K0, W,
                                       hipMemcpyDeviceToDevice, s));
        if ((r = pack_both(v, &v->Wp, &v->WpT, padded, W, KP, s))) return r;
    }
    const float* const* wh = w + 1;
    if (fam.patch_bias) { if ((r = v->mem.copy_f32(&v->bp, *wh++, W, s))) return r; }
    if ((r = v->mem.copy_f32(&v->cls, *wh++, W, s))) return r;
    if ((r = v->mem.copy_f32(&v->pos, *wh++, (size_t)T * W, s))) return r;
    v->lnpre_g = v->lnpre_b = nullptr;
    if (fam.ln_pre) {
        if ((r = v->mem.copy_f32(&v->lnpre_g, *wh++, W, s))) return r;
        if ((r = v->mem.copy_f32(&v->lnpre_b, *wh++, W, s))) return r;
    }
    v->L.resize(layers);
    const size_t R = (size_t)max_n * T;
    for (int l = 0; l < layers; ++l) {
        const float* const* q = w + n_head + 12 * l;
        VitLayer& y = v->L[l];
        if ((r = v->mem.copy_f32(&y.ln1_g, q[0], W, s))) return r;
        if ((r = v->mem.copy_f32(&y.ln1_b, q[1], W, s))) return r;
        if (hd == 64) {
            if ((r = pack_both(v, &y.Wqkv, &y.WqkvT, q[2], 3 * W, W, s))) return r;
            if ((r = v->mem.copy_f32(&y.bqkv, q[3], 3 * W, s))) return r;
            if ((r = pack_both(v, &y.Wo, &y.WoT, q[4], W, W, s))) return r;
        } else {
// ... 11 lines not shown
        }
        if ((r = v->mem.copy_f32(&y.bo, q[5], W, s))) return r;
        if ((r = v->mem.copy_f32(&y.ln2_g, q[6], W, s))) return r;
        if ((r = v->mem.copy_f32(&y.ln2_b, q[7], W, s))) return r;
        if ((r = pack_both(v, &y.W1, &y.W1T, q[8], 4 * W, W, s))) return r;
        if ((r = v->mem.copy_f32(&y.b1, q[9], 4 * W, s))) return r;
        if ((r = pack_both(v, &y.W2, &y.W2T, q[10], W, 4 * W, s))) return r;
        if ((r = v->mem.copy_f32(&y.b2, q[11], W, s))) return r;
        if (v->lean) { DEV_ALLOC(m, alloc_op, y.x_in, R * W, f32); DEV_ALLOC(m, alloc_op, y.x_mid, R * W, f32); }
        else { float *a_, *b_; DEV_ALLOC(m, alloc, a_, R * W); DEV_ALLOC(m, alloc, b_, R * W); y.x_in = a_; y.x_mid = b_; }
        DEV_ALLOC(m, alloc, y.mean1, R); DEV_ALLOC(m, alloc, y.rstd1, R); DEV_ALLOC(m, alloc, y.mean2, R); DEV_ALLOC(m, alloc, y.rstd2, R);
        DEV_ALLOC(m, alloc_op, y.qkv, R * 3 * AW, f32); DEV_ALLOC(m, alloc_op, y.t, R * 4 * W, f32);
        y.o_save = nullptr; y.lse = nullptr;
        if (T > 64 || v->f32 || hp == 96) { DEV_ALLOC(m, alloc_op, y.o_save, R * AW, f32); DEV_ALLOC(m, alloc, y.lse, (size_t)max_n * heads * T); }
    }
    const float* const* q = w + n_head + 12 * layers;
    if ((r = v->mem.copy_f32(&v->lnpost_g, q[0], W, s))) return r;
    if ((r = v->mem.copy_f32(&v->lnpost_b, q[1], W, s))) return r;
    if ((r = pack_both(v, &v->proj, &v->projT, q[2], W, out_dim, s))) return r;
    DEV_ALLOC(m, alloc_op, v->A0, R * KP, f32); DEV_ALLOC(m, alloc_op, v->h, R * W, f32);
    DEV_ALLOC(m, alloc_op, v->att_o, R * AW, f32); DEV_ALLOC(m, alloc_op, v->u, R * 4 * W, f32);
    DEV_ALLOC(m, alloc_op, v->hpost, (size_t)max_n * W, f32); DEV_ALLOC(m, alloc_op, v->de16, (size_t)max_n * out_dim, f32);
    DEV_ALLOC(m, alloc_op, v->dt, R * 4 * W, f32); DEV_ALLOC(m, alloc_op, v->do_, R * AW, f32); DEV_ALLOC(m, alloc_op, v->dqkv, R * 3 * AW, f32);
    DEV_ALLOC(m, alloc, v->xpre, R * W); DEV_ALLOC(m, alloc, v->mean_pre, R); DEV_ALLOC(m, alloc, v->rstd_pre, R);
    if (v->lean) DEV_ALLOC(m, alloc_op, v->x_final, R * W, f32);
    else { float* a_; DEV_ALLOC(m, alloc, a_, R * W); v->x_final = a_; }
    DEV_ALLOC(m, alloc, v->mean_post, max_n); DEV_ALLOC(m, alloc, v->rstd_post, max_n); DEV_ALLOC(m, alloc, v->e, (size_t)max_n * out_dim);
    v->dx = v->dh = nullptr;
    if (!v->lean) { DEV_ALLOC(m, alloc, v->dx, R * W); DEV_ALLOC(m, alloc, v->dh, R * W); }
    DEV_ALLOC(m, alloc, v->dA0, R * KP); DEV_ALLOC(m, alloc, v->de, (size_t)max_n * out_dim);
    if (v->f32) { v->dx_bf = v->dx; v->dh_bf = v->dh; }
    else { DEV_ALLOC(m, alloc_op, v->dx_bf, R * W, f32); DEV_ALLOC(m, alloc_op, v->dh_bf, R * W, f32); }
    DEV_ALLOC(m, alloc, v->dhpost, (size_t)max_n * W); DEV_ALLOC(m, alloc, v->mm_part, 2 * 1024);
    if (v->h16) DEV_ALLOC(m, alloc, v->gs, 2 + 64);
    v->ws_bytes = (size_t)64 << 20;
    DEV_ALLOC(m, alloc, v->ws, v->ws_bytes / sizeof(float));
    *out = guard.release();
    return 0;
}

void prx_vit_destroy_impl(PrxVit* v) { delete v; }

static int vit_gemm(PrxVit* v, GemmDesc& d, hipStream_t s) {
    if (v->f32) { d.f32 = 1; d.a_is_f32 = 0; }
    d.h16 = v->h16;
    return prx_gemm_launch(d, v->ws, v->ws_bytes, s, &v->gctx);
}
GemmCtx* prx_vit_gemm_ctx_impl(PrxVit* v) { return v ? &v->gctx : nullptr; }
long long prx_vit_debug_dqkv_impl(PrxVit* v, void* dst, long long max_bytes, hipStream_t s) {
    if (!v || v->cur_n < 1) return -1;
    const long long bytes = (long long)op_esz(v->f32) * v->cur_n * v->T * 3 * v->aw;
    if (bytes > max_bytes || hipMemcpyAsync(dst, v->dqkv, bytes, hipMemcpyDeviceToDevice, s) != hipSuccess) return -1;
    return bytes;
}

static int ln_op(PrxVit* v, const void* x, long long ldx, const float* g, const float* b, void* out, float* mean, float* rstd,
                 int rows, hipStream_t s) {
    return prx_layernorm_fwd(x, ldx, g, b, v->f32 ? nullptr : (bf16_t*)out, v->f32 ? (float*)out : nullptr, mean, rstd, rows,
                             v->width, v->fam.eps, s, v->h16, v->lean, 1);
}
static int ln_bwd_op(PrxVit* v, const void* g, long long ldg, const void* x, long long ldx, const float* gamma, const float* mean,
                     const float* rstd, const void* add, long long ldadd, float* dx, long long lddx, void* dx_op, int rows,
                     hipStream_t s, int add_every = 0, int s16 = 0) {
    return prx_layernorm_bwd(g, ldg, x, ldx, gamma, mean, rstd, add, ldadd, dx, lddx, v->f32 ? nullptr : (bf16_t*)dx_op, lddx, rows,
                             v->width, s, v->h16, add_every, s16, 1);
}

int prx_vit_minmax_impl(PrxVit* v, const float* cutouts, int n, float* mm, hipStream_t s) {
    PRX_REQUIRE(n >= 1 && n <= v->max_n, "vit: batch %d exceeds handle capacity %d", n, v->max_n);
    return prx_minmax(cutouts, (size_t)n * 3 * v->res * v->res, v->mm_part, 1024, mm, s);
}

int prx_vit_forward_impl(PrxVit* v, const float* cutouts, int n, const float* mm, float* embeds, hipStream_t s) {
    PRX_REQUIRE(n >= 1 && n <= v->max_n, "vit: batch %d exceeds handle capacity %d", n, v->max_n);
    const int W = v->width, T = v->T, R = n * T, KP = v->KP, AW = v->aw;
    int r;
    v->cur_n = n;
    if ((r = prx_patchify_fwd(cutouts, mm, v->A0, v->prec, n, v->res, v->patch, T, s, v->fam.norm))) return r;
    {
        GemmDesc d; d.A = v->A0; d.lda = KP; d.B = v->Wp; d.ldb = KP; d.M = R; d.N = W; d.K = KP;
        d.bias_n = v->bp;
        d.out_f32 = v->xpre; d.ldc_f32 = W;
        if ((r = vit_gemm(v, d, s))) return r;
    }
    const int lean = v->lean;
    void* x0 = v->layers > 0 ? v->L[0].x_in : v->x_final;
    if (v->fam.ln_pre) {
        if ((r = prx_vit_add_cls_pos(v->xpre, v->cls, v->pos, n, T, W, s))) return r;
        if ((r = prx_layernorm_fwd(v->xpre, W, v->lnpre_g, v->lnpre_b, lean ? (bf16_t*)x0 : nullptr, lean ? nullptr : (float*)x0, v->mean_pre,
                                   v->rstd_pre, R, W, v->fam.eps, s, v->h16, 0, 1))) return r;
    } else {
        if ((r = prx_vit_embed_tokens(v->xpre, v->cls, v->pos, x0, lean, n, T, W, s))) return r;
    }
    for (int l = 0; l < v->layers; ++l) {
        VitLayer& y = v->L[l];
        void* x_next = (l + 1 < v->layers) ? v->L[l + 1].x_in : v->x_final;
        if ((r = ln_op(v, y.x_in, W, y.ln1_g, y.ln1_b, v->h, y.mean1, y.rstd1, R, s))) return r;
        {   GemmDesc d; d.A = v->h; d.lda = W; d.B = y.Wqkv; d.ldb = W; d.M = R; d.N = 3 * AW; d.K = W;
            d.bias_n = y.bqkv; d.out_bf16 = y.qkv; d.ldc_bf16 = 3 * AW;
            if ((r = vit_gemm(v, d, s))) return r; }
        const void* att = v->att_o;
        if (v->hp == 96) {
            if (v->f32) { if ((r = prx_mha_fwd_f32_hd96((const float*)y.qkv, (float*)y.o_save, y.lse, n, T, AW, v->heads, s))) return r; }
            else if ((r = prx_mha_fwd_hd96((const bf16_t*)y.qkv, (bf16_t*)y.o_save, y.lse, n, T, AW, v->heads, 1.f / sqrtf((float)v->hd), s, v->h16))) return r;
            att = y.o_save;
        }
        else if (v->f32) { if ((r = prx_mha_fwd_f32((const float*)y.qkv, (float*)y.o_save, y.lse, n, T, AW, v->heads, s))) return r; att = y.o_save; }
        else if (T <= 64) { if ((r = prx_mha_fwd((const bf16_t*)y.qkv, (bf16_t*)v->att_o, n, T, AW, v->heads, s, v->h16))) return r; }
        else { if ((r = prx_mha_fwd_gen((const bf16_t*)y.qkv, (bf16_t*)y.o_save, y.lse, n, T, AW, v->heads, s, v->h16))) return r; att = y.o_save; }
        const bool tail = v->cls_tail && l == v->layers - 1;
        const int rows = tail ? n : R;
        const int ldt = tail ? T * W : W;
        {   GemmDesc d; d.A = att; d.lda = tail ? T * AW : AW; d.B = y.Wo; d.ldb = AW; d.M = rows; d.N = W; d.K = AW;
            d.bias_n = y.bo; d.ldr = ldt;
            if (lean) { d.resid = (const float*)y.x_in; d.row16 = 1; d.out_bf16 = y.x_mid; d.ldc_bf16 = ldt; }
            else { d.resid = (const float*)y.x_in; d.out_f32 = (float*)y.x_mid; d.ldc_f32 = ldt; }
            if ((r = vit_gemm(v, d, s))) return r; }
        if ((r = ln_op(v, y.x_mid, ldt, y.ln2_g, y.ln2_b, v->h, y.mean2, y.rstd2, rows, s))) return r;
        {   GemmDesc d; d.A = v->h; d.lda = W; d.B = y.W1; d.ldb = W; d.M = rows; d.N = 4 * W; d.K = W;
            d.bias_n = y.b1; d.act = v->fam.act; d.out_bf16 = v->u; d.out_bf16_pre = y.t; d.ldc_bf16 = 4 * W;
            const bool own_pass = v->f32 && v->fam.act == PRX_ACT_GELU;
            if (own_pass) { d.act = PRX_ACT_NONE; d.out_bf16 = y.t; d.out_bf16_pre = nullptr; }
            if ((r = vit_gemm(v, d, s))) return r;
            if (own_pass) {
                if ((r = prx_vit_gelu_f32((const float*)y.t, (float*)v->u, (size_t)rows * 4 * W, 0, s))) return r;
            } }
        {   GemmDesc d; d.A = v->u; d.lda = 4 * W; d.B = y.W2; d.ldb = 4 * W; d.M = rows; d.N = W; d.K = 4 * W;
            d.bias_n = y.b2; d.ldr = ldt;
            if (lean) { d.resid = (const float*)y.x_mid; d.row16 = 1; d.out_bf16 = x_next; d.ldc_bf16 = ldt; }
            else { d.resid = (const float*)y.x_mid; d.out_f32 = (float*)x_next; d.ldc_f32 = ldt; }
            if ((r = vit_gemm(v, d, s))) return r; }
    }
    if ((r = ln_op(v, v->x_final, (long long)T * W, v->lnpost_g, v->lnpost_b, v->hpost, v->mean_post, v->rstd_post, n, s))) return r;
    {   GemmDesc d; d.A = v->hpost; d.lda = W; d.B = v->projT; d.ldb = W; d.M = n; d.N = v->out_dim; d.K = W;
        d.out_f32 = v->e; d.ldc_f32 = v->out_dim;
        if ((r = vit_gemm(v, d, s))) return r; }
    return prx_l2norm_fwd(v->e, embeds, n, v->out_dim, s);
}

int prx_vit_backward_a_impl(PrxVit* v, const float* cutouts, const float* mm, const float* d_embeds, double* acc,
                            hipStream_t s) {
    const int n = v->cur_n;
    PRX_REQUIRE(n >= 1, "vit backward: no forward in flight on this handle");
    const int W = v->width, T = v->T, R = n * T, KP = v->KP, AW = v->aw;
    int r;
    if ((r = prx_l2norm_bwd(v->e, d_embeds, v->de, n, v->out_dim, s))) return r;
    {   GemmDesc d; d.A = v->de; d.a_is_f32 = 1; d.lda = v->out_dim; d.B = v->proj; d.ldb = v->out_dim;
        d.M = n; d.N = W; d.K = v->out_dim; d.out_f32 = v->dhpost; d.ldc_f32 = W;
        if (v->h16) {
            if ((r = prx_grad_scale(v->de, (size_t)n * v->out_dim, v->gs + 2, 64, prx_grad_target_log2(), v->gs, s))) return r;
            if ((r = prx_scale_dev(v->de, (size_t)n * v->out_dim, v->gs, s, (bf16_t*)v->de16, v->h16))) return r;
            d.A = v->de16; d.a_is_f32 = 0;
        }
        if ((r = vit_gemm(v, d, s))) return r; }
    const int lean = v->lean;
    if (v->layers == 0 || !v->cls_tail) PRX_CHECK_HIP(hipMemsetAsync(lean ? v->dx_bf : (void*)v->dx, 0, (lean ? sizeof(bf16_t) : sizeof(float)) * (size_t)R * W, s));
    const void* dxs = lean ? v->dx_bf : (const void*)v->dx;
    const void* dhs = lean ? v->dh_bf : (const void*)v->dh;
    if ((r = ln_bwd_op(v, v->dhpost, W, v->x_final, (long long)T * W, v->lnpost_g, v->mean_post, v->rstd_post,
                       nullptr, 0, v->dx, (long long)T * W, v->dx_bf, n, s, 0, lean ? 1 : 0))) return r;
    for (int l = v->layers - 1; l >= 0; --l) {
        VitLayer& y = v->L[l];
        const bool tail = v->cls_tail && l == v->layers - 1;
        const int rows = tail ? n : R;
        const int ldt = tail ? T * W : W;
        {   GemmDesc d; d.A = v->dx_bf; d.lda = ldt; d.B = y.W2T; d.ldb = W; d.M = rows; d.N = 4 * W; d.K = W;
            d.act = v->fam.dact; d.aux = y.t; d.ldaux = 4 * W; d.out_bf16 = v->dt; d.ldc_bf16 = 4 * W;
            const bool own_pass = v->f32 && v->fam.dact == PRX_ACT_MUL_DGELU;
            if (own_pass) { d.act = PRX_ACT_NONE; d.aux = nullptr; }
            if ((r = vit_gemm(v, d, s))) return r;
            if (own_pass) {
                if ((r = prx_vit_gelu_f32((const float*)y.t, (float*)v->dt, (size_t)rows * 4 * W, 1, s))) return r;
            } }
        {   GemmDesc d; d.A = v->dt; d.lda = 4 * W; d.B = y.W1T; d.ldb = 4 * W; d.M = rows; d.N = W; d.K = 4 * W;
            if (lean) { d.out_bf16 = v->dh_bf; d.ldc_bf16 = W; } else { d.out_f32 = v->dh; d.ldc_f32 = W; }
            if ((r = vit_gemm(v, d, s))) return r; }
        if ((r = ln_bwd_op(v, dhs, W, y.x_mid, ldt, y.ln2_g, y.mean2, y.rstd2, dxs, ldt, v->dx, ldt, v->dx_bf, rows, s, 0, lean ? 7 : 0))) return r;
        if (tail)
            PRX_CHECK_HIP(hipMemsetAsync(v->do_, 0, op_esz(v->f32) * (size_t)R * AW, s));
        {   GemmDesc d; d.A = v->dx_bf; d.lda = ldt; d.B = y.WoT; d.ldb = W; d.M = rows; d.N = AW; d.K = W;
            d.out_bf16 = v->do_; d.ldc_bf16 = tail ? T * AW : AW;
            if ((r = vit_gemm(v, d, s))) return r; }
        if (v->hp == 96) {
            if (v->f32) { if ((r = prx_mha_bwd_f32_hd96((const float*)y.qkv, (const float*)y.o_save, (const float*)v->do_, y.lse, (float*)v->dqkv, n, T, AW, v->heads, s))) return r; }
            else if ((r = prx_mha_bwd_hd96((const bf16_t*)y.qkv, (const bf16_t*)y.o_save, (const bf16_t*)v->do_, y.lse, (bf16_t*)v->dqkv, n, T, AW, v->heads,
                                           1.f / sqrtf((float)v->hd), s, v->h16))) return r;
        }
        else if (v->f32) { if ((r = prx_mha_bwd_f32((const float*)y.qkv, (const float*)y.o_save, (const float*)v->do_, y.lse, (float*)v->dqkv, n, T, AW, v->heads, s))) return r; }
        else if (T <= 64) { if ((r = prx_mha_bwd((const bf16_t*)y.qkv, (const bf16_t*)v->do_, (bf16_t*)v->dqkv, n, T, AW, v->heads, s, v->h16))) return r; }
        else { if ((r = prx_mha_bwd_gen((const bf16_t*)y.qkv, (const bf16_t*)y.o_save, (const bf16_t*)v->do_, y.lse, (bf16_t*)v->dqkv, n, T, AW, v->heads, s, v->h16))) return r; }
        {   GemmDesc d; d.A = v->dqkv; d.lda = 3 * AW; d.B = y.WqkvT; d.ldb = 3 * AW; d.M = R; d.N = W; d.K = 3 * AW;
            if (lean) { d.out_bf16 = v->dh_bf; d.ldc_bf16 = W; } else { d.out_f32 = v->dh; d.ldc_f32 = W; }
            if ((r = vit_gemm(v, d, s))) return r; }
        if ((r = ln_bwd_op(v, dhs, W, y.x_in, W, y.ln1_g, y.mean1, y.rstd1, dxs, W, v->dx, W, v->dx_bf, R, s, tail ? T : 0, lean ? 7 : 0))) return r;
    }
    if (v->fam.ln_pre) { if ((r = ln_bwd_op(v, dxs, W, v->xpre, W, v->lnpre_g, v->mean_pre, v->rstd_pre, nullptr, 0, v->dh, W, v->dh_bf, R, s, 0, lean ? 2 : 0))) return r; }
    {   GemmDesc d; d.A = v->fam.ln_pre ? v->dh_bf : v->dx_bf; d.lda = W; d.B = v->WpT; d.ldb = W; d.M = R; d.N = KP; d.K = W;
        d.out_f32 = v->dA0; d.ldc_f32 = KP;
        if (v->h16) d.alpha_dev = v->gs + 1;
        if ((r = vit_gemm(v, d, s))) return r; }
    return prx_patchify_bwd_reduce(cutouts, mm, v->dA0, acc, n, v->res, v->patch, T, s, v->fam.norm);
}

int prx_vit_backward_b_impl(PrxVit* v, const float* cutouts, const float* mm, const double* acc, float* g_cutouts,
                            hipStream_t s) {
    const int n = v->cur_n;
    PRX_REQUIRE(n >= 1, "vit backward: no forward in flight on this handle");
    int r = prx_patchify_bwd_apply(cutouts, mm, v->dA0, acc, g_cutouts, n, v->res, v->patch, v->T, s, v->fam.norm);
    return r;
}
```

### pixray_amd/csrc/vqgan.hip

```cpp
#include "vqgan.h"
#include "gemm.h"
#include "norms.h"
#include "elementwise.h"
#include "prompt_vq.h"
#include "vit.h"
#include "dev_arena.h"
#include <vector>
#include <memory>
#include <stdlib.h>

namespace {

template <typename TOp>
__global__ __launch_bounds__(256) void pack_conv3x3_kernel(const float* __restrict__ w, TOp* __restrict__ Wf,
                                                           TOp* __restrict__ Wd, int Cout, int Cin, int CoP) {
    const size_t total_f = (size_t)Cout * 9 * Cin;
    const size_t total_d = (size_t)Cin * 9 * CoP;
    for (size_t i = (size_t)blockIdx.x * blockDim.x + threadIdx.x; i < total_f + total_d;
         i += (size_t)gridDim.x * blockDim.x) {
        if (i < total_f) {
            int ci = (int)(i % Cin);
            int tap = (int)((i / Cin) % 9);
            int co = (int)(i / ((size_t)9 * Cin));
            Wf[i] = op_cvt<TOp>(w[(((size_t)co * Cin + ci) * 3 + tap / 3) * 3 + tap % 3]);
// ... 29 lines not shown
int prx_colminmax(const float* w, float* mn, float* mx, int rows, int D, hipStream_t s) {
    hipLaunchKernelGGL(colminmax_kernel, dim3(ceil_div(D, 256)), dim3(256), 0, s, w, mn, mx, rows, D);
    PRX_LAUNCH_CHECK();
    return 0;
}

static inline int pad8(int P) { return (P + 7) & ~7; }

struct Conv3 { int Cin, Cout, CoP; void *Wf, *Wd; float* b; };
struct Conv1 { int Cin, Cout; void *W, *WT; float* b; };
struct GN { int C; float *g, *b; double *stats, *bstats; int id; };

struct ResBlock {
    int Cin, Cout, rh, rw;
    GN n1, n2; Conv3 c1, c2; Conv1 sc; bool has_sc;
    void *x_in, *h1, *scbuf, *out;
    void *x_in_bf, *out_bf;
};
struct AttnBlock {
    int C, rh, rw;
    GN n; Conv1 qkv, proj;
    void* x_in; void *qkvb, *Pm, *PT; void* out; void* out_bf;
    void* qkvT;
};
struct UpBlock { int C, rh, rw; Conv3 c; void *x_in, *out; void *x_in_bf, *out_bf; };

struct Stage { int kind; int idx; };

struct PrxVqgan {
    int zc, D, NC, ch, out_ch, h0, w0, H, W, nstage;
    int prec;
    int f32, h16;
    int lean;
    float* gs;
    GemmCtx gctx;
    DevArena mem;
    float *codebook, *cnorm, *zmin, *zmax;
    Conv1 pq; Conv3 conv_in, conv_out; GN norm_out;
    std::vector<ResBlock> res; std::vector<AttnBlock> attn; std::vector<UpBlock> ups; std::vector<Stage> stages;
    float *zq, *y, *dzq; void* h_in; int* idx; void *pqo_bf, *h_in_bf, *dpq_bf;
    float *pmin; int* pidx;
    void* a;
    void *tA, *tB, *tC, *tD, *dqkv, *dy8;
    void *dycol, *Wd_col;
    float* S;
    void *g0, *g1, *g2;
    void *g0b, *g1b, *g2b;
    double* all_stats; int n_gn;
    float* ws; size_t ws_bytes;
    void* x_last;
};

namespace {
int alloc_stream(PrxVqgan* v, void** p, size_t count) { return v->mem.alloc_op(p, count, !v->lean); }

struct WCursor { const float* const* w; int n, pos; };
#define NEXTW(cur, dst) do { PRX_REQUIRE((cur).pos < (cur).n, "vqgan_create: weight list too short"); (dst) = (cur).w[(cur).pos++]; } while (0)

int make_gn(PrxVqgan* v, GN& g, int C, WCursor& cur, hipStream_t s) {
    const float *w, *b; NEXTW(cur, w); NEXTW(cur, b);
    g.C = C;
    int r;
    if ((r = v->mem.copy_f32(&g.g, w, C, s))) return r;
    if ((r = v->mem.copy_f32(&g.b, b, C, s))) return r;
    g.id = v->n_gn++;
    g.stats = g.bstats = nullptr;
// ... 67 lines not shown
    PRX_CHECK_HIP(hipMemsetAsync(ab.qkvT, 0, (size_t)3 * C * P8 * op_esz(v->f32), s));
    PRX_CHECK_HIP(hipMemsetAsync(ab.Pm, 0, P * P8 * op_esz(v->f32), s));
    PRX_CHECK_HIP(hipMemsetAsync(ab.PT, 0, P * P8 * op_esz(v->f32), s));
    v->stages.push_back({1, (int)v->attn.size()});
    v->attn.push_back(ab);
    return 0;
}
int make_up(PrxVqgan* v, int C, int rh, int rw, WCursor& cur, hipStream_t s) {
    UpBlock ub{};
    ub.C = C; ub.rh = rh; ub.rw = rw;
    int r;
    if ((r = make_conv3(v, ub.c, C, C, cur, s))) return r;
    if ((r = alloc_stream(v, &ub.out, (size_t)rh * rw * C))) return r;
    v->stages.push_back({2, (int)v->ups.size()});
    v->ups.push_back(ub);
    return 0;
}
}

int prx_vqgan_create_impl(PrxVqgan** out, int ch, const int* ch_mult, int n_mult, int num_res_blocks, int attn_res,
                          int resolution, int z_channels, int embed_dim, int n_embed, int out_ch, int h0, int w0,
                          int precision, const float* const* w, int n_w, hipStream_t s) {
    PRX_REQUIRE(h0 >= 1 && w0 >= 1, "vqgan_create: bad latent size %dx%d", h0, w0);
    PRX_REQUIRE(prec_valid(precision), "vqgan_create: unknown precision %d", precision);
    PRX_REQUIRE(embed_dim == z_channels, "vqgan_create: embed_dim must equal z_channels");
    std::unique_ptr<PrxVqgan> guard(new PrxVqgan());
    PrxVqgan* v = guard.get();
    DevArena& m = v->mem;
    const int f32 = prec_is_f32(precision);
    m.describe("vqgan_create", ": the decoder keeps one forward's activations and the backward's gradient streams for a %d x %d latent", h0, w0);
    v->prec = precision; v->f32 = prec_is_f32(precision); v->h16 = prec_is_h16(precision);
    v->gs = nullptr;
    { const char* e = getenv("PRX_LEAN"); v->lean = (v->h16 && !(e && atoi(e) == 0)) ? 1 : 0; }
    v->n_gn = 0; v->zc = z_channels; v->D = embed_dim; v->NC = n_embed; v->ch = ch; v->out_ch = out_ch; v->h0 = h0; v->w0 = w0;
    WCursor cur{w, n_w, 0};
    int r;
    const float* cb; NEXTW(cur, cb);
    if ((r = m.copy_f32(&v->codebook, cb, (size_t)n_embed * embed_dim, s))) return r;
    DEV_ALLOC(m, alloc, v->cnorm, n_embed); DEV_ALLOC(m, alloc, v->zmin, embed_dim); DEV_ALLOC(m, alloc, v->zmax, embed_dim);
    if ((r = prx_sqnorm_rows(v->codebook, v->cnorm, n_embed, embed_dim, s))) return r;
    if ((r = prx_colminmax(v->codebook, v->zmin, v->zmax, n_embed, embed_dim, s))) return r;
    if ((r = make_conv1(v, v->pq, embed_dim, z_channels, cur, s))) return r;
    int block_in = ch * ch_mult[n_mult - 1];
    int rh = h0, rw = w0;
    if ((r = make_conv3(v, v->conv_in, z_channels, block_in, cur, s))) return r;
    if ((r = make_res(v, block_in, block_in, rh, rw, cur, s))) return r;
    if ((r = make_attn(v, block_in, rh, rw, cur, s))) return r;
    if ((r = make_res(v, block_in, block_in, rh, rw, cur, s))) return r;
    int nominal = resolution >> (n_mult - 1);
    for (int lvl = n_mult - 1; lvl >= 0; --lvl) {
        int block_out = ch * ch_mult[lvl];
        for (int b = 0; b < num_res_blocks + 1; ++b) {
            if ((r = make_res(v, block_in, block_out, rh, rw, cur, s))) return r;
            block_in = block_out;
            if (nominal == attn_res) { if ((r = make_attn(v, block_in, rh, rw, cur, s))) return r; }
        }
        if (lvl != 0) {
            rh *= 2; rw *= 2; nominal *= 2;
            if ((r = make_up(v, block_in, rh, rw, cur, s))) return r;
        }
    }
    v->H = rh; v->W = rw;
    if ((r = make_gn(v, v->norm_out, block_in, cur, s))) return r;
    if ((r = make_conv3(v, v->conv_out, block_in, out_ch, cur, s))) return r;
    PRX_REQUIRE(cur.pos == n_w, "vqgan_create: %d weight tensors given, %d consumed", n_w, cur.pos);
    const size_t P0 = (size_t)h0 * w0, PH = (size_t)rh * rw;
// ... 18 lines not shown
        PRX_CHECK_HIP(hipMemsetAsync(v->Wd_col, 0, (size_t)Cin * 128 * sizeof(bf16_t), s));
        PRX_CHECK_HIP(hipMemcpy2DAsync(v->Wd_col, 128 * sizeof(bf16_t), v->conv_out.Wd, 72 * sizeof(bf16_t), 72 * sizeof(bf16_t), Cin, hipMemcpyDeviceToDevice, s));
    }
    DEV_ALLOC(m, alloc, v->S, maxAttnPC);
    for (void** g : {&v->g0, &v->g1, &v->g2})
        if ((r = alloc_stream(v, g, maxPC))) return r;
    if (v->f32 || v->lean) { v->g0b = v->g0; v->g1b = v->g1; v->g2b = v->g2; }
    else { DEV_ALLOC(m, alloc_op, v->g0b, maxPC, f32); DEV_ALLOC(m, alloc_op, v->g1b, maxPC, f32); DEV_ALLOC(m, alloc_op, v->g2b, maxPC, f32); }
    v->h_in_bf = nullptr;
    for (size_t i = 0; i < v->stages.size(); ++i) {
        const Stage& st = v->stages[i];
        const bool need = (st.kind == 0 && v->res[st.idx].has_sc) || st.kind == 2;
        if (!need) continue;
        void** slot; size_t cnt; void* self;
        if (i == 0) { slot = &v->h_in_bf; cnt = P0 * (size_t)(ch * ch_mult[n_mult - 1]); self = v->h_in; }
        else {
            const Stage& pr = v->stages[i - 1];
            if (pr.kind == 0) { ResBlock& b = v->res[pr.idx]; slot = &b.out_bf; cnt = (size_t)b.rh * b.rw * b.Cout; self = b.out; }
            else if (pr.kind == 1) { AttnBlock& b = v->attn[pr.idx]; slot = &b.out_bf; cnt = (size_t)b.rh * b.rw * b.C; self = b.out; }
            else { UpBlock& b = v->ups[pr.idx]; slot = &b.out_bf; cnt = (size_t)b.rh * b.rw * b.C; self = b.out; }
        }
        if (v->f32 || v->lean) *slot = self;
        else DEV_ALLOC(m, alloc_op, *slot, cnt, f32);
    }
    {
        DEV_ALLOC(m, alloc, v->all_stats, (size_t)2 * v->n_gn * 64);
        auto fix = [&](GN& g) { g.stats = v->all_stats + (size_t)g.id * 64; g.bstats = v->all_stats + (size_t)(v->n_gn + g.id) * 64; };
        for (auto& b : v->res) { fix(b.n1); fix(b.n2); }
        for (auto& b : v->attn) fix(b.n);
        fix(v->norm_out);
    }
    v->ws_bytes = (size_t)64 << 20;
    DEV_ALLOC(m, alloc, v->ws, v->ws_bytes / sizeof(float));
    if (v->h16) DEV_ALLOC(m, alloc, v->gs, 2 + 256);
    *out = guard.release();
    return 0;
}

void prx_vqgan_destroy_impl(PrxVqgan* v) { delete v; }

static bool fusable(const PrxVqgan* v, int C) {
    static const bool f32_fuse = [] { const char* e = getenv("PRX_F32_GN_FUSE"); return !(e && atoi(e) == 0); }();
    const int gs = C / 32;
    return (!v->f32 || f32_fuse) && C % 32 == 0 && gs >= 4 && (gs & (gs - 1)) == 0;
}

static int zero_if_padded(const PrxVqgan* v, void* buf, size_t rows, int P, hipStream_t s) {
    if (pad8(P) != P) PRX_CHECK_HIP(hipMemsetAsync(buf, 0, rows * (size_t)pad8(P) * op_esz(v->f32), s));
    return 0;
}


static void vq_trace(const PrxVqgan* v, const char* tag, int i, const void* p_, size_t n, hipStream_t s) {
    static const bool on = getenv("PRX_VQ_TRACE") != nullptr;
    if (!on || !p_ || v->lean) return;
    const float* p = (const float*)p_;
    std::vector<float> h(n);
    (void)hipStreamSynchronize(s);
    (void)hipMemcpy(h.data(), p, n * sizeof(float), hipMemcpyDeviceToHost);
    double q = 0, mx = 0;
    for (float x : h) { q += (double)x * x; mx = fabs(x) > mx ? fabs(x) : mx; }
    fprintf(stderr, "[vq] %s %2d n=%zu l2 %.9e max %.6e\n", tag, i, n, sqrt(q), mx);
}

static int vg(PrxVqgan* v, GemmDesc& d, hipStream_t s) {
    if (v->f32) {
        d.f32 = 1; d.a_is_f32 = 0;
// ... 20 lines not shown
    d.B = c.Wf; d.ldb = 9 * c.Cin; d.M = rh * rw; d.N = c.CoP; d.K = 9 * c.Cin;
    d.H = rh; d.W = rw; d.Cin = c.Cin; d.up = up; d.bias_n = c.b;
    resid_stream(v, d, resid, c.Cout);
    if (f32_out) { d.out_f32 = (float*)out; d.ldc_f32 = ldc; }
    else { out_stream(v, d, out, ldc, out_bf); if (!v->lean) d.ldc_bf16 = c.Cout; }
    if (stats_for && stats_for->C == c.Cout && fusable(v, c.Cout)) { d.gn_stats = stats_for->stats; d.gn_gs = c.Cout / 32; }
    return vg(v, d, s);
}
static void set_gnb(const PrxVqgan* v, GemmDesc& d, const GN* gnb, const void* gnb_x, int swish) {
    if (!gnb || !fusable(v, gnb->C) || d.N != gnb->C) return;
    d.gn_stats = gnb->bstats; d.gn_gs = gnb->C / 32;
    d.gnb_x = (const float*)gnb_x;
    if (v->lean) d.row16 |= 2;
    d.gnb_fstats = gnb->stats; d.gnb_gamma = gnb->g; d.gnb_beta = gnb->b; d.gnb_swish = swish; d.gnb_eps = 1e-6f;
}
static int conv3_bwd(PrxVqgan* v, const Conv3& c, const void* dy, bool dy_f32, int rh, int rw, void* dx, hipStream_t s,
                     void* dx_bf = nullptr, const GN* gnb = nullptr, const void* gnb_x = nullptr, int gnb_swish = 1) {
    GemmDesc d; d.A = dy; d.a_is_f32 = dy_f32; d.a_mode = PRX_A_CONV3X3; d.lda = c.CoP;
    d.B = c.Wd; d.ldb = 9 * c.CoP; d.M = rh * rw; d.N = c.Cin; d.K = 9 * c.CoP;
    d.H = rh; d.W = rw; d.Cin = c.CoP; d.up = 0;
    out_stream(v, d, dx, c.Cin, dx_bf);
    set_gnb(v, d, gnb, gnb_x, gnb_swish);
    return vg(v, d, s);
}
static const GN* first_norm(const PrxVqgan* v, int si) {
    if (si >= (int)v->stages.size()) return &v->norm_out;
    const Stage& st = v->stages[si];
    if (st.kind == 0) return &v->res[st.idx].n1;
    if (st.kind == 1) return &v->attn[st.idx].n;
    return nullptr;
}
static int gn_fwd(PrxVqgan* v, const GN& g, const void* x, int P, int swish, hipStream_t s, bool stats_ready = false) {
    return prx_groupnorm_fwd(x, g.g, g.b, g.stats, v->f32 ? nullptr : (bf16_t*)v->a, v->f32 ? (float*)v->a : nullptr, 1, P, g.C, swish,
                             1e-6f, s, 0, stats_ready ? 1 : 0, v->h16, v->lean);
}
static int gn_bwd(PrxVqgan* v, const GN& g, const void* grad, const void* x, const void* add, void* dx,
                  void* dx_bf, int P, int swish, hipStream_t s, bool stats_ready = false) {
    return prx_groupnorm_bwd(grad, x, g.g, g.b, g.stats, g.bstats, add, v->lean ? nullptr : (float*)dx, v->f32 ? nullptr : (bf16_t*)dx_bf, 1, P, g.C,
                             swish, 1e-6f, s, 0, stats_ready && fusable(v, g.C) ? 1 : 0, v->h16, v->lean);
}

int prx_vqgan_bounds_impl(PrxVqgan* v, float* zmin, float* zmax, hipStream_t s) {
    PRX_CHECK_HIP(hipMemcpyAsync(zmin, v->zmin, sizeof(float) * v->D, hipMemcpyDeviceToDevice, s));
    PRX_CHECK_HIP(hipMemcpyAsync(zmax, v->zmax, sizeof(float) * v->D, hipMemcpyDeviceToDevice, s));
    return 0;
}

int prx_vqgan_synth_impl(PrxVqgan* v, const float* z, float* img, int* indices, int quantize, hipStream_t s) {
    const int P0 = v->h0 * v->w0;
    int r;
    PRX_CHECK_HIP(hipMemsetAsync(v->all_stats, 0, sizeof(double) * (size_t)v->n_gn * 64, s));
    if (quantize) {
        if ((r = prx_vq_nearest(z, 1, P0, v->codebook, v->cnorm, P0, v->NC, v->D, v->pmin, v->pidx, v->idx, v->zq, s))) return r;
        if (indices) PRX_CHECK_HIP(hipMemcpyAsync(indices, v->idx, sizeof(int) * P0, hipMemcpyDeviceToDevice, s));
    } else {
        if ((r = prx_nchw_to_nhwc(z, v->zq, nullptr, 1, v->zc, P0, v->zc, s))) return r;
    }
    {   GemmDesc d; d.A = v->zq; d.a_is_f32 = 1; d.lda = v->D; d.B = v->pq.W; d.ldb = v->D; d.M = P0; d.N = v->zc; d.K = v->D;
        d.bias_n = v->pq.b; d.out_bf16 = v->pqo_bf; d.ldc_bf16 = v->zc;
        if ((r = vg(v, d, s))) return r; }
    const GN* nx = first_norm(v, 0);
    if ((r = conv3_fwd(v, v->conv_in, v->pqo_bf, false, v->h0, v->w0, false, nullptr, v->h_in, v->conv_in.Cout, s, v->h_in_bf, nx))) return r;
    bool sr = nx && nx->C == v->conv_in.Cout && fusable(v, nx->C);
    void* x = v->h_in;
    void* x_bf = v->h_in_bf;
    for (int si = 0; si < (int)v->stages.size(); ++si) {
        const Stage& st = v->stages[si];
        nx = first_norm(v, si + 1);
        if (st.kind == 0) {
            ResBlock& b = v->res[st.idx];
            const int P = b.rh * b.rw;
            b.x_in = x; b.x_in_bf = x_bf;
            if ((r = gn_fwd(v, b.n1, x, P, 1, s, sr))) return r;
            if ((r = conv3_fwd(v, b.c1, v->a, false, b.rh, b.rw, false, nullptr, b.h1, b.Cout, s, nullptr, &b.n2))) return r;
            const void* resid = x;
            if (b.has_sc) {
                PRX_REQUIRE(x_bf != nullptr, "vqgan: missing bf16 twin for the shortcut input");
                GemmDesc d; d.A = x_bf; d.lda = b.Cin; d.B = b.sc.W; d.ldb = b.Cin; d.M = P; d.N = b.Cout; d.K = b.Cin;
                d.bias_n = b.sc.b; out_stream(v, d, b.scbuf, b.Cout, nullptr);
                if ((r = vg(v, d, s))) return r;
                resid = b.scbuf;
            }
            if ((r = gn_fwd(v, b.n2, b.h1, P, 1, s, fusable(v, b.Cout)))) return r;
            if ((r = conv3_fwd(v, b.c2, v->a, false, b.rh, b.rw, false, resid, b.out, b.Cout, s, b.out_bf, nx))) return r;
            sr = nx && nx->C == b.Cout && fusable(v, b.Cout);
            x = b.out; x_bf = b.out_bf;
        } else if (st.kind == 1) {
// ... 32 lines not shown
            vq_trace(v, "fwd", si, x, (size_t)Pq * Cq, s); }
    }
    v->x_last = x;
    const int PH = v->H * v->W;
    if ((r = gn_fwd(v, v->norm_out, x, PH, 1, s, sr))) return r;
    if ((r = conv3_fwd(v, v->conv_out, v->a, false, v->H, v->W, false, nullptr, v->y, v->conv_out.CoP, s, nullptr, nullptr, true))) return r;
    return prx_image_head_fwd(v->y, v->conv_out.CoP, img, 1, v->out_ch, PH, s);
}

long long prx_vqgan_debug_stage_impl(PrxVqgan* v, int stage, float* dst, long long max_floats, hipStream_t s) {
    const void* src = nullptr; long long n = 0;
    PRX_REQUIRE(!v->lean || stage == -2 || stage >= (int)v->stages.size(), "vqgan debug_stage: the stage outputs are 16-bit in the lean layout (PRX_LEAN=0 for fp32 streams)");
    const int ns = (int)v->stages.size();
    if (stage == -2) { src = v->zq; n = (long long)v->h0 * v->w0 * v->D; }
    else if (stage == -1) { src = v->h_in; n = (long long)v->h0 * v->w0 * v->conv_in.Cout; }
    else if (stage >= 0 && stage < ns) {
        const Stage& st = v->stages[stage];
        if (st.kind == 0) { const ResBlock& b = v->res[st.idx]; src = b.out; n = (long long)b.rh * b.rw * b.Cout; }
        else if (st.kind == 1) { const AttnBlock& b = v->attn[st.idx]; src = b.out; n = (long long)b.rh * b.rw * b.C; }
        else { const UpBlock& b = v->ups[st.idx]; src = b.out; n = (long long)b.rh * b.rw * b.C; }
    } else if (stage == ns) { src = v->y; n = (long long)v->H * v->W * v->conv_out.CoP; }
    else if (stage == ns + 1) { src = reinterpret_cast<const float*>(v->all_stats); n = (long long)v->n_gn * 64 * 2; }
    else return -1;
    if (n > max_floats) n = max_floats;
    if (hipMemcpyAsync(dst, src, sizeof(float) * n, hipMemcpyDeviceToDevice, s) != hipSuccess) return -1;
    return n;
}

int prx_vqgan_backward_impl(PrxVqgan* v, const float* g_img, float* dz, hipStream_t s) {
    const int PH = v->H * v->W;
    int r;
    PRX_REQUIRE(v->x_last != nullptr, "vqgan backward: no forward in flight on this handle");
    PRX_CHECK_HIP(hipMemsetAsync(v->all_stats + (size_t)v->n_gn * 64, 0, sizeof(double) * (size_t)v->n_gn * 64, s));
    if (v->h16 && (r = prx_grad_scale(g_img, (size_t)v->out_ch * PH, v->gs + 2, 256, prx_grad_target_log2(), v->gs, s))) return r;
    struct GB { void* f; void* b; };
    GB g{v->g0, v->g0b}, t1{v->g1, v->g1b}, t2{v->g2, v->g2b};
    if (v->dycol) {
        if ((r = prx_image_head_bwd_im2col(v->y, v->conv_out.CoP, g_img, (bf16_t*)v->dycol, 128, v->out_ch, v->H, v->W, s, v->h16, v->gs))) return r;
        GemmDesc d; d.A = v->dycol; d.lda = 128; d.B = v->Wd_col; d.ldb = 128; d.M = PH; d.N = v->conv_out.Cin; d.K = 128;
        out_stream(v, d, t1.f, v->conv_out.Cin, nullptr);
        set_gnb(v, d, &v->norm_out, v->x_last, 1);
        if ((r = vg(v, d, s))) return r;
    } else {
        if ((r = prx_image_head_bwd(v->y, v->conv_out.CoP, g_img, v->f32 ? (float*)v->dy8 : nullptr, v->f32 ? nullptr : (bf16_t*)v->dy8, v->conv_out.CoP, 1,
                                    v->out_ch, PH, s, v->h16, v->gs))) return r;
        if ((r = conv3_bwd(v, v->conv_out, v->dy8, false, v->H, v->W, t1.f, s, nullptr, &v->norm_out, v->x_last, 1))) return r;
    }
    if ((r = gn_bwd(v, v->norm_out, t1.f, v->x_last, nullptr, g.f, g.b, PH, 1, s, true))) return r;
    for (int si = (int)v->stages.size() - 1; si >= 0; --si) {
        const Stage& st = v->stages[si];
        if (st.kind == 0) {
            ResBlock& b = v->res[st.idx];
            const int P = b.rh * b.rw;
            if ((r = conv3_bwd(v, b.c2, g.b, false, b.rh, b.rw, t1.f, s, nullptr, &b.n2, b.h1, 1))) return r;
            if ((r = gn_bwd(v, b.n2, t1.f, b.h1, nullptr, v->f32 ? t2.f : nullptr, t2.b, P, 1, s, true))) return r;
            if ((r = conv3_bwd(v, b.c1, t2.b, false, b.rh, b.rw, t1.f, s, nullptr, &b.n1, b.x_in, 1))) return r;
            const void* add = g.f;
            if (b.has_sc) {
                GemmDesc d; d.A = g.b; d.lda = b.Cout; d.B = b.sc.WT; d.ldb = b.Cout; d.M = P; d.N = b.Cin; d.K = b.Cout;
                out_stream(v, d, t2.f, b.Cin, nullptr);
                if ((r = vg(v, d, s))) return r;
                add = t2.f;
            }
            GB& dst = (add == g.f) ? t2 : g;
            if ((r = gn_bwd(v, b.n1, t1.f, b.x_in, add, dst.f, dst.b, P, 1, s, true))) return r;
            if (&dst != &g) std::swap(g, t2);
        } else if (st.kind == 1) {
// ... 49 lines not shown
```

Measured before the change: 166.9.

## Fold glue kernels: single-pass grad scale, fused cls/pos into LN, row0 mha bwd, wide groupnorm

Adds several fusions on by default through env flags. The grad-scale max reduction becomes one kernel that uses a last-block ticket instead of a two-pass reduction. The ViT cls/pos add is folded into the pre-LayerNorm. The l2norm backward is fused with the grad scale and fp16 conversion. Attention backward reads only dout row 0 for the tail layer, which removes a memset. VQ index copy-out is folded into the nearest-codebook kernel, and a 'wide' groupnorm variant is enabled. The aim is to cut launches and memsets, at the cost of more complex kernels and reliance on the ticket counter resetting correctly.

```diff
diff --git a/include/prx.h b/include/prx.h
--- a/include/prx.h
+++ b/include/prx.h
@@ -94,6 +94,12 @@
 int prx_k_groupnorm_bwd_op(const void* g, const void* x, const float* gamma, const float* beta, const double* fstats,
                            double* bstats, const void* add, float* dx, void* dx16, int NB, int P, int C, int swish, float eps,
                            int zero_stats, int stats_ready, int h16, int s16, prx_stream_t s);
+int prx_k_groupnorm_fwd_wide(const void* x, const float* gamma, const float* beta, double* stats, void* out16, float* out_f32,
+                             int NB, int P, int C, int swish, float eps, int zero_stats, int stats_ready, int h16, int s16,
+                             int wide, int xcd, int* took_wide, prx_stream_t s);
+int prx_k_groupnorm_bwd_wide(const void* g, const void* x, const float* gamma, const float* beta, const double* fstats,
+                             double* bstats, const void* add, float* dx, void* dx16, int NB, int P, int C, int swish, float eps,
+                             int zero_stats, int stats_ready, int h16, int s16, int wide, int xcd, int* took_wide, prx_stream_t s);
 int prx_k_layernorm_fwd_op(const void* x, long long ldx, const float* gamma, const float* beta, void* out16, float* out_f32,
                            float* mean, float* rstd, int rows, int C, float eps, int h16, int s16, prx_stream_t s);
 int prx_k_layernorm_bwd_op(const void* g, long long ldg, const void* x, long long ldx, const float* gamma, const float* mean,
@@ -101,6 +107,9 @@
                            long long lddxb, int rows, int C, int h16, int add_every, int s16, prx_stream_t s);
 int prx_k_mha_fwd_op(const void* qkv, void* out, int N, int T, int C, int heads, int h16, prx_stream_t s);
 int prx_k_mha_bwd_op(const void* qkv, const void* dout, void* dqkv, int N, int T, int C, int heads, int h16, prx_stream_t s);
+int prx_k_mha_bwd_row0_op(const void* qkv, const void* dout, void* dqkv, int N, int T, int C, int heads, int h16, int dout_row0, prx_stream_t s);
+int prx_k_layernorm_fwd_emb(float* x, long long ldx, const float* gamma, const float* beta, void* out16, float* out_f32, float* mean, float* rstd,
+                            int rows, int C, float eps, int h16, const float* cls, const float* pos, int T, prx_stream_t s);
 int prx_k_mha_fwd_gen_op(const void* qkv, void* out, float* lse, int N, int T, int C, int heads, int h16, prx_stream_t s);
 int prx_k_mha_bwd_gen_op(const void* qkv, const void* out, const void* dout, const float* lse, void* dqkv, int N, int T, int C,
                          int heads, int h16, prx_stream_t s);
@@ -123,6 +132,9 @@
 int prx_k_image_head_bwd_im2col(const float* x, int ldc, const float* gimg, void* col, int ldk, int C, int H, int W, int h16,
                                 const float* gscale, prx_stream_t s);
 int prx_k_grad_scale(const float* g, size_t n, float* part, int nparts, int target_log2, float* scale2, prx_stream_t s);
+int prx_k_grad_scale_one(const float* g, size_t n, float* part, int nparts, int target_log2, float* scale2, unsigned* ticket, prx_stream_t s);
+int prx_k_l2norm_bwd_scaled(const float* e, const float* g, float* de, void* de16, int n, int D, int target_log2, float* scale2, int h16,
+                            prx_stream_t s);
 int prx_k_grad_scale_multi(const float* const* gs, const size_t* ns, int count, float* part, int nparts_each, int target_log2,
                            float* scale2, prx_stream_t s);
 int prx_k_scale_dev(float* x, size_t n, const float* scale, void* out16, int h16, prx_stream_t s);
diff --git a/pixray_amd/csrc/api_kernels.hip b/pixray_amd/csrc/api_kernels.hip
--- a/pixray_amd/csrc/api_kernels.hip
+++ b/pixray_amd/csrc/api_kernels.hip
@@ -98,6 +98,18 @@
     return prx_groupnorm_bwd(g, x, gamma, beta, fstats, bstats, add, dx, B_(dx16), NB, P, C, swish, eps, S_(s), zero_stats,
                              stats_ready, h16, s16);
 }
+int prx_k_groupnorm_fwd_wide(const void* x, const float* gamma, const float* beta, double* stats, void* out16, float* out_f32,
+                             int NB, int P, int C, int swish, float eps, int zero_stats, int stats_ready, int h16, int s16,
+                             int wide, int xcd, int* took_wide, prx_stream_t s) {
+    return prx_groupnorm_fwd(x, gamma, beta, stats, B_(out16), out_f32, NB, P, C, swish, eps, S_(s), zero_stats, stats_ready, h16, s16,
+                             wide, xcd, took_wide);
+}
+int prx_k_groupnorm_bwd_wide(const void* g, const void* x, const float* gamma, const float* beta, const double* fstats,
+                             double* bstats, const void* add, float* dx, void* dx16, int NB, int P, int C, int swish, float eps,
+                             int zero_stats, int stats_ready, int h16, int s16, int wide, int xcd, int* took_wide, prx_stream_t s) {
+    return prx_groupnorm_bwd(g, x, gamma, beta, fstats, bstats, add, dx, B_(dx16), NB, P, C, swish, eps, S_(s), zero_stats,
+                             stats_ready, h16, s16, wide, xcd, took_wide);
+}
 int prx_k_layernorm_fwd_op(const void* x, long long ldx, const float* gamma, const float* beta, void* out16, float* out_f32,
                            float* mean, float* rstd, int rows, int C, float eps, int h16, int s16, prx_stream_t s) {
     return prx_layernorm_fwd(x, ldx, gamma, beta, B_(out16), out_f32, mean, rstd, rows, C, eps, S_(s), h16, s16);
@@ -114,6 +126,13 @@
 int prx_k_mha_bwd_op(const void* qkv, const void* dout, void* dqkv, int N, int T, int C, int heads, int h16, prx_stream_t s) {
     return prx_mha_bwd(CB_(qkv), CB_(dout), B_(dqkv), N, T, C, heads, S_(s), h16);
 }
+int prx_k_mha_bwd_row0_op(const void* qkv, const void* dout, void* dqkv, int N, int T, int C, int heads, int h16, int dout_row0, prx_stream_t s) {
+    return prx_mha_bwd(CB_(qkv), CB_(dout), B_(dqkv), N, T, C, heads, S_(s), h16, dout_row0);
+}
+int prx_k_layernorm_fwd_emb(float* x, long long ldx, const float* gamma, const float* beta, void* out16, float* out_f32, float* mean, float* rstd,
+                            int rows, int C, float eps, int h16, const float* cls, const float* pos, int T, prx_stream_t s) {
+    return prx_layernorm_fwd(x, ldx, gamma, beta, B_(out16), out_f32, mean, rstd, rows, C, eps, S_(s), h16, 0, 1, cls, pos, T);
+}
 int prx_k_mha_fwd_gen_op(const void* qkv, void* out, float* lse, int N, int T, int C, int heads, int h16, prx_stream_t s) {
     return prx_mha_fwd_gen(CB_(qkv), B_(out), lse, N, T, C, heads, S_(s), h16);
 }
@@ -172,6 +191,14 @@
 int prx_k_grad_scale(const float* g, size_t n, float* part, int nparts, int target_log2, float* scale2, prx_stream_t s) {
     return prx_grad_scale(g, n, part, nparts, target_log2, scale2, S_(s));
 }
+int prx_k_grad_scale_one(const float* g, size_t n, float* part, int nparts, int target_log2, float* scale2, unsigned* ticket, prx_stream_t s) {
+    PRX_REQUIRE(ticket != nullptr, "grad_scale_one: needs a zeroed ticket word");
+    return prx_grad_scale(g, n, part, nparts, target_log2, scale2, S_(s), ticket);
+}
+int prx_k_l2norm_bwd_scaled(const float* e, const float* g, float* de, void* de16, int n, int D, int target_log2, float* scale2, int h16,
+                            prx_stream_t s) {
+    return prx_l2norm_bwd_scaled(e, g, de, B_(de16), n, D, target_log2, scale2, h16, S_(s));
+}
 int prx_k_grad_scale_multi(const float* const* gs, const size_t* ns, int count, float* part, int nparts_each, int target_log2,
                            float* scale2, prx_stream_t s) {
     return prx_grad_scale_multi(gs, ns, count, part, nparts_each, target_log2, scale2, S_(s));
diff --git a/pixray_amd/csrc/attention.h b/pixray_amd/csrc/attention.h
--- a/pixray_amd/csrc/attention.h
+++ b/pixray_amd/csrc/attention.h
@@ -1,7 +1,7 @@
 #pragma once
 #include "common.h"
 int prx_mha_fwd(const bf16_t* qkv, bf16_t* out, int N, int T, int C, int heads, hipStream_t s, int h16 = 0);
-int prx_mha_bwd(const bf16_t* qkv, const bf16_t* dout, bf16_t* dqkv, int N, int T, int C, int heads, hipStream_t s, int h16 = 0);
+int prx_mha_bwd(const bf16_t* qkv, const bf16_t* dout, bf16_t* dqkv, int N, int T, int C, int heads, hipStream_t s, int h16 = 0, int dout_row0 = 0);
 int prx_mha_fwd_gen(const bf16_t* qkv, bf16_t* out, float* lse, int N, int T, int C, int heads, hipStream_t s, int h16 = 0);
 int prx_mha_bwd_gen(const bf16_t* qkv, const bf16_t* out, const bf16_t* dout, const float* lse, bf16_t* dqkv, int N, int T,
                     int C, int heads, hipStream_t s, int h16 = 0);
diff --git a/pixray_amd/csrc/attention.hip b/pixray_amd/csrc/attention.hip
--- a/pixray_amd/csrc/attention.hip
+++ b/pixray_amd/csrc/attention.hip
@@ -40,8 +40,8 @@
 int prx_mha_fwd(const bf16_t* qkv, bf16_t* out, int N, int T, int C, int heads, hipStream_t s, int h16) {
     return h16 ? att_f16::mha_fwd(H(qkv), HM(out), N, T, C, heads, s) : att_bf16::mha_fwd(qkv, out, N, T, C, heads, s);
 }
-int prx_mha_bwd(const bf16_t* qkv, const bf16_t* dout, bf16_t* dqkv, int N, int T, int C, int heads, hipStream_t s, int h16) {
-    return h16 ? att_f16::mha_bwd(H(qkv), H(dout), HM(dqkv), N, T, C, heads, s) : att_bf16::mha_bwd(qkv, dout, dqkv, N, T, C, heads, s);
+int prx_mha_bwd(const bf16_t* qkv, const bf16_t* dout, bf16_t* dqkv, int N, int T, int C, int heads, hipStream_t s, int h16, int dout_row0) {
+    return h16 ? att_f16::mha_bwd(H(qkv), H(dout), HM(dqkv), N, T, C, heads, s, dout_row0) : att_bf16::mha_bwd(qkv, dout, dqkv, N, T, C, heads, s, dout_row0);
 }
 int prx_mha_fwd_gen(const bf16_t* qkv, bf16_t* out, float* lse, int N, int T, int C, int heads, hipStream_t s, int h16) {
     return h16 ? att_f16::mha_fwd_gen(H(qkv), HM(out), lse, N, T, C, heads, s) : att_bf16::mha_fwd_gen(qkv, out, lse, N, T, C, heads, s);
diff --git a/pixray_amd/csrc/attention_kernels.inc b/pixray_amd/csrc/attention_kernels.inc
--- a/pixray_amd/csrc/attention_kernels.inc
+++ b/pixray_amd/csrc/attention_kernels.inc
@@ -43,14 +43,14 @@
 
 __device__ __forceinline__ int tr_swz(int d) { return (((d >> 4) & 1) * 12) ^ (((d >> 5) & 1) * 16); }
 
-__device__ __forceinline__ void tile_get(const a16_t* src, long long ld, int T, int tid, a16x8 (&v)[4]) {
+__device__ __forceinline__ void tile_get(const a16_t* src, long long ld, int T, int tid, a16x8 (&v)[4], int row0 = 0) {
 #pragma unroll
     for (int i = 0; i < 4; ++i) {
         const int c = tid + 128 * i;
         const int row = c >> 3, kc = c & 7;
         const a16x8 z = {0, 0, 0, 0, 0, 0, 0, 0};
-        const a16x8 x = *reinterpret_cast<const a16x8*>(src + (long long)(row < T ? row : T - 1) * ld + kc * 8);
-        v[i] = row < T ? x : z;
+        const a16x8 x = *reinterpret_cast<const a16x8*>(src + (long long)(row0 ? 0 : (row < T ? row : T - 1)) * ld + kc * 8);
+        v[i] = (row0 ? row == 0 : row < T) ? x : z;
     }
 }
 __device__ __forceinline__ void tile_put(const a16x8 (&v)[4], a16_t* dst, a16_t* dstT, int tid) {
@@ -224,6 +224,7 @@
     store_rows_global(o, w, out + (long long)n * T * C + h * 64, C, T, lane);
 }
 
+template <bool ROW0>
 __global__ __launch_bounds__(128) void mha_bwd_kernel(const a16_t* __restrict__ qkv, const a16_t* __restrict__ dout,
                                                       a16_t* __restrict__ dqkv, int T, int C, float scale, int xcd) {
     __shared__ __attribute__((aligned(16))) a16_t smem[5 * TILE];
@@ -247,7 +248,7 @@
         tile_get(base, ld, T, tid, tq);
         tile_get(base + C, ld, T, tid, tk);
         tile_get(base + 2 * C, ld, T, tid, tv);
-        tile_get(dobase, C, T, tid, tdo);
+        tile_get(dobase, C, T, tid, tdo, ROW0 ? 1 : 0);
         tile_put(tq, Qs, nullptr, tid);
         tile_put(tk, Ks, Tt, tid);
         tile_put(tv, Vs, nullptr, tid);
@@ -874,9 +875,10 @@
     return 0;
 }
 
-inline int mha_bwd(const a16_t* qkv, const a16_t* dout, a16_t* dqkv, int N, int T, int C, int heads, hipStream_t s) {
+inline int mha_bwd(const a16_t* qkv, const a16_t* dout, a16_t* dqkv, int N, int T, int C, int heads, hipStream_t s, int dout_row0) {
     PRX_REQUIRE(T <= 64 && C == heads * 64, "mha bwd: needs T <= 64 and head dim 64 (T=%d C=%d heads=%d)", T, C, heads);
-    hipLaunchKernelGGL(mha_bwd_kernel, dim3(heads, N), dim3(128), 0, s, qkv, dout, dqkv, T, C, 0.125f, prx_xcd_local());
+    if (dout_row0) hipLaunchKernelGGL(mha_bwd_kernel<true>, dim3(heads, N), dim3(128), 0, s, qkv, dout, dqkv, T, C, 0.125f, prx_xcd_local());
+    else hipLaunchKernelGGL(mha_bwd_kernel<false>, dim3(heads, N), dim3(128), 0, s, qkv, dout, dqkv, T, C, 0.125f, prx_xcd_local());
     PRX_LAUNCH_CHECK();
     return 0;
 }
diff --git a/pixray_amd/csrc/common.h b/pixray_amd/csrc/common.h
--- a/pixray_amd/csrc/common.h
+++ b/pixray_amd/csrc/common.h
@@ -166,6 +166,17 @@
 }
 int prx_xcd_local();
 int prx_grad_target_log2();
+__device__ __forceinline__ float grad_scale_pow2(float m, int target_log2) {
+    float S = 1.f;
+    if (m > 0.f && m < INFINITY) {
+        int e;
+        (void)frexpf(m, &e);
+        int k = target_log2 - e;
+        k = k < -40 ? -40 : (k > 60 ? 60 : k);
+        S = ldexpf(1.f, k);
+    }
+    return S;
+}
 
 static inline int ceil_div(int a, int b) { return (a + b - 1) / b; }
 static inline long long ceil_div_ll(long long a, long long b) { return (a + b - 1) / b; }
diff --git a/pixray_amd/csrc/elementwise.h b/pixray_amd/csrc/elementwise.h
--- a/pixray_amd/csrc/elementwise.h
+++ b/pixray_amd/csrc/elementwise.h
@@ -13,7 +13,7 @@
                        int HW, hipStream_t s, int h16 = 0, const float* gscale = nullptr);
 int prx_image_head_bwd_im2col(const float* x, int ldc, const float* gimg, bf16_t* col, int ldk, int C, int H, int W, hipStream_t s, int h16 = 0,
                               const float* gscale = nullptr);
-int prx_grad_scale(const float* g, size_t n, float* part, int nparts, int target_log2, float* scale2, hipStream_t s);
+int prx_grad_scale(const float* g, size_t n, float* part, int nparts, int target_log2, float* scale2, hipStream_t s, unsigned* ticket = nullptr);
 int prx_adam_clamp(float* z, float* m, float* v, const float* g, const float* zmin, const float* zmax, int hw,
                    size_t n, float lr, float b1, float b2, float eps, int step, hipStream_t s);
 int prx_adam_clamp_dev(float* z, float* m, float* v, const float* g, const float* zmin, const float* zmax, int hw,
diff --git a/pixray_amd/csrc/elementwise.hip b/pixray_amd/csrc/elementwise.hip
--- a/pixray_amd/csrc/elementwise.hip
+++ b/pixray_amd/csrc/elementwise.hip
@@ -241,14 +241,45 @@
     __syncthreads();
     if (threadIdx.x == 0) {
         m = fmaxf(fmaxf(s[0], s[1]), fmaxf(s[2], s[3]));
-        float S = 1.f;
-        if (m > 0.f && m < INFINITY) {
-            int e;
-            (void)frexpf(m, &e);
-            int k = target_log2 - e;
-            k = k < -40 ? -40 : (k > 60 ? 60 : k);
-            S = ldexpf(1.f, k);
-        }
+        const float S = grad_scale_pow2(m, target_log2);
+        scale2[0] = S;
+        scale2[1] = 1.f / S;
+    }
+}
+
+__global__ __launch_bounds__(256) void grad_scale_one_kernel(const float* __restrict__ g, size_t n, float* __restrict__ part, int target_log2,
+                                                             float* __restrict__ scale2, unsigned* __restrict__ ticket) {
+    float m = 0.f;
+    const size_t n4 = ((uintptr_t)g & 15) == 0 ? n / 4 : 0;
+    for (size_t i = (size_t)blockIdx.x * blockDim.x + threadIdx.x; i < n4; i += (size_t)gridDim.x * blockDim.x) {
+        const float4 v = reinterpret_cast<const float4*>(g)[i];
+        const float a0 = fabsf(v.x), a1 = fabsf(v.y), a2 = fabsf(v.z), a3 = fabsf(v.w);
+        m = fmaxf(fmaxf(fmaxf(m, a0 == a0 ? a0 : INFINITY), a1 == a1 ? a1 : INFINITY), fmaxf(a2 == a2 ? a2 : INFINITY, a3 == a3 ? a3 : INFINITY));
+    }
+    for (size_t i = 4 * n4 + (size_t)blockIdx.x * blockDim.x + threadIdx.x; i < n; i += (size_t)gridDim.x * blockDim.x) {
+        const float a = fabsf(g[i]);
+        m = fmaxf(m, a == a ? a : INFINITY);
+    }
+    m = wave_max(m);
+    __shared__ float s[4];
+    __shared__ unsigned last;
+    if ((threadIdx.x & 63) == 0) s[threadIdx.x >> 6] = m;
+    __syncthreads();
+    if (threadIdx.x == 0) {
+        part[blockIdx.x] = fmaxf(fmaxf(s[0], s[1]), fmaxf(s[2], s[3]));
+        __threadfence();
+        last = atomicInc(ticket, gridDim.x - 1) == gridDim.x - 1 ? 1u : 0u;
+    }
+    __syncthreads();
+    if (!last) return;
+    __threadfence();
+    m = 0.f;
+    for (int i = threadIdx.x; i < (int)gridDim.x; i += blockDim.x) m = fmaxf(m, *reinterpret_cast<const volatile float*>(part + i));
+    m = wave_max(m);
+    if ((threadIdx.x & 63) == 0) s[threadIdx.x >> 6] = m;
+    __syncthreads();
+    if (threadIdx.x == 0) {
+        const float S = grad_scale_pow2(fmaxf(fmaxf(s[0], s[1]), fmaxf(s[2], s[3])), target_log2);
         scale2[0] = S;
         scale2[1] = 1.f / S;
     }
@@ -322,9 +353,14 @@
     PRX_LAUNCH_CHECK();
     return 0;
 }
-int prx_grad_scale(const float* g, size_t n, float* part, int nparts, int target_log2, float* scale2, hipStream_t s) {
+int prx_grad_scale(const float* g, size_t n, float* part, int nparts, int target_log2, float* scale2, hipStream_t s, unsigned* ticket) {
     PRX_REQUIRE(nparts >= 1 && nparts <= 1024, "grad_scale: 1..1024 partials");
     const int blocks = (int)std::min<size_t>((n + 1023) / 1024 + 1, (size_t)nparts);
+    if (ticket) {
+        hipLaunchKernelGGL(grad_scale_one_kernel, dim3(blocks), dim3(256), 0, s, g, n, part, target_log2, scale2, ticket);
+        PRX_LAUNCH_CHECK();
+        return 0;
+    }
     hipLaunchKernelGGL(amax_partial_kernel, dim3(blocks), dim3(256), 0, s, g, n, part);
     PRX_LAUNCH_CHECK();
     hipLaunchKernelGGL(grad_scale_final_kernel, dim3(1), dim3(256), 0, s, part, blocks, target_log2, scale2);
diff --git a/pixray_amd/csrc/norms.h b/pixray_amd/csrc/norms.h
--- a/pixray_amd/csrc/norms.h
+++ b/pixray_amd/csrc/norms.h
@@ -3,15 +3,17 @@
 #include <algorithm>
 int prx_groupnorm_fwd(const void* x, const float* gamma, const float* beta, double* stats, bf16_t* out_bf16,
                       float* out_f32, int NB, int P, int C, int swish, float eps, hipStream_t s, int zero_stats = 1,
-                      int stats_ready = 0, int h16 = 0, int s16 = 0);
+                      int stats_ready = 0, int h16 = 0, int s16 = 0, int wide = 0, int xcd = -1, int* took_wide = nullptr);
 int prx_groupnorm_bwd(const void* g, const void* x, const float* gamma, const float* beta, const double* fstats,
                       double* bstats, const void* add, float* dx, bf16_t* dx_bf16, int NB, int P, int C, int swish,
-                      float eps, hipStream_t s, int zero_stats = 1, int stats_ready = 0, int h16 = 0, int s16 = 0);
+                      float eps, hipStream_t s, int zero_stats = 1, int stats_ready = 0, int h16 = 0, int s16 = 0, int wide = 0, int xcd = -1,
+                      int* took_wide = nullptr);
 int prx_groupnorm_bwd_stats(const float* g, const float* x, const float* gamma, const float* beta, const double* fstats,
                             double* bstats, int NB, int P, int C, int swish, float eps, hipStream_t s);
 int prx_layernorm_fwd(const void* x, long long ldx, const float* gamma, const float* beta, bf16_t* out_bf16,
                       float* out_f32, float* mean, float* rstd, int rows, int C, float eps, hipStream_t s, int h16 = 0, int s16 = 0,
-                      int ragged = 0);
+                      int ragged = 0,
+                      const float* emb_cls = nullptr, const float* emb_pos = nullptr, int emb_T = 0);
 int prx_layernorm_bwd(const void* g, long long ldg, const void* x, long long ldx, const float* gamma,
                       const float* mean, const float* rstd, const void* add, long long ldadd, float* dx,
                       long long lddx, bf16_t* dx_bf16, long long lddxb, int rows, int C, hipStream_t s, int h16 = 0,
diff --git a/pixray_amd/csrc/norms.hip b/pixray_amd/csrc/norms.hip
--- a/pixray_amd/csrc/norms.hip
+++ b/pixray_amd/csrc/norms.hip
@@ -210,16 +210,142 @@
     if (idx < i1) one(idx, v0, g0, a0);
 }
 
+__device__ __forceinline__ bf16x8 stream_ld8(const void* p, unsigned i8) { return reinterpret_cast<const bf16x8*>(p)[i8]; }
+__device__ __forceinline__ float4 op16_quad(const bf16x8& t, int hi, int h16) {
+    return hi ? make_float4(from_op16(t[4], h16), from_op16(t[5], h16), from_op16(t[6], h16), from_op16(t[7], h16))
+              : make_float4(from_op16(t[0], h16), from_op16(t[1], h16), from_op16(t[2], h16), from_op16(t[3], h16));
+}
+__device__ __forceinline__ bf16x8 to_op16x8(const float4& lo, const float4& hi, int h16) {
+    bf16x8 r;
+    r[0] = to_op16(lo.x, h16); r[1] = to_op16(lo.y, h16); r[2] = to_op16(lo.z, h16); r[3] = to_op16(lo.w, h16);
+    r[4] = to_op16(hi.x, h16); r[5] = to_op16(hi.y, h16); r[6] = to_op16(hi.z, h16); r[7] = to_op16(hi.w, h16);
+    return r;
+}
+template <bool BWD>
+__device__ __forceinline__ void gn_lane_load2(const GNArgs& a, const double* bstats, int b, int co, GnLane& L0, GnLane& L1) {
+    gn_lane_load<BWD>(a, bstats, b, 2 * co, L0);
+    if (a.C < 256) gn_lane_load<BWD>(a, bstats, b, 2 * co + 1, L1);
+    else { L1.mean = L0.mean; L1.rstd = L0.rstd; L1.m1 = L0.m1; L1.m2 = L0.m2; L1.b = b; }
+}
+__device__ __forceinline__ float4 gn_fwd_quad(const GNArgs& a, const GnLane& L, const float4& v) {
+    const float xv[4] = {v.x, v.y, v.z, v.w};
+    const float gav[4] = {L.ga.x, L.ga.y, L.ga.z, L.ga.w}, bev[4] = {L.be.x, L.be.y, L.be.z, L.be.w};
+    float o[4];
+#pragma unroll
+    for (int i = 0; i < 4; ++i) {
+        float y = (xv[i] - L.mean) * L.rstd * gav[i] + bev[i];
+        o[i] = a.swish ? y * sigmoidf_(y) : y;
+    }
+    return make_float4(o[0], o[1], o[2], o[3]);
+}
+__device__ __forceinline__ float4 gn_bwd_quad(const GNArgs& a, const GnLane& L, const float4& v, const float4& gg, const float4& ad) {
+    const float xv[4] = {v.x, v.y, v.z, v.w}, gv[4] = {gg.x, gg.y, gg.z, gg.w};
+    const float gav[4] = {L.ga.x, L.ga.y, L.ga.z, L.ga.w}, bev[4] = {L.be.x, L.be.y, L.be.z, L.be.w};
+    float o[4];
+#pragma unroll
+    for (int i = 0; i < 4; ++i) {
+        float xh = (xv[i] - L.mean) * L.rstd;
+        float gy = gv[i];
+        if (a.swish) gy *= swish_grad(xh * gav[i] + bev[i]);
+        float dxh = gy * gav[i];
+        o[i] = L.rstd * (dxh - L.m1 - xh * L.m2);
+    }
+    o[0] += ad.x; o[1] += ad.y; o[2] += ad.z; o[3] += ad.w;
+    return make_float4(o[0], o[1], o[2], o[3]);
+}
+
+__global__ __launch_bounds__(256) void gn_apply_fwd8_kernel(const GNArgs a, bf16_t* out_bf16, float* out_f32, int NB, int xcd, int h16) {
+    const unsigned C8 = (unsigned)a.C >> 3;
+    const unsigned total = (unsigned)NB * (unsigned)a.P * C8, per_b = (unsigned)a.P * C8;
+    unsigned i0 = blockIdx.x * blockDim.x + threadIdx.x, i1 = total, step = gridDim.x * blockDim.x;
+    if (xcd) {
+        const unsigned per = (total + gridDim.x - 1) / gridDim.x, lo = per * xcd_linear(blockIdx.x, gridDim.x);
+        i0 = lo + threadIdx.x; i1 = lo + per < total ? lo + per : total; step = blockDim.x;
+    }
+    if (i0 >= i1) return;
+    const bf16x8 z8 = {};
+    unsigned idx = i0;
+    bf16x8 v0 = stream_ld8(a.x, idx);
+    bf16x8 v1 = idx + step < i1 ? stream_ld8(a.x, idx + step) : z8;
+    const int co = (int)(i0 % C8);
+    GnLane L0 = {}, L1 = {};
+    L0.ga = reinterpret_cast<const float4*>(a.gamma)[2 * co]; L1.ga = reinterpret_cast<const float4*>(a.gamma)[2 * co + 1];
+    L0.be = reinterpret_cast<const float4*>(a.beta)[2 * co]; L1.be = reinterpret_cast<const float4*>(a.beta)[2 * co + 1];
+    gn_lane_load2<false>(a, nullptr, NB == 1 ? 0 : (int)(i0 / per_b), co, L0, L1);
+    auto one = [&](unsigned id, const bf16x8& v) {
+        if (NB != 1) { const int b = (int)(id / per_b); if (b != L0.b) gn_lane_load2<false>(a, nullptr, b, co, L0, L1); }
+        const float4 lo = gn_fwd_quad(a, L0, op16_quad(v, 0, a.h16)), hi = gn_fwd_quad(a, L1, op16_quad(v, 1, a.h16));
+        if (out_bf16) reinterpret_cast<bf16x8*>(out_bf16)[id] = to_op16x8(lo, hi, h16);
+        if (out_f32) { reinterpret_cast<float4*>(out_f32)[2 * (size_t)id] = lo; reinterpret_cast<float4*>(out_f32)[2 * (size_t)id + 1] = hi; }
+    };
+    for (; idx + step < i1; idx += 2 * step) {
+        const unsigned nx = idx + 2 * step;
+        const bf16x8 n0 = nx < i1 ? stream_ld8(a.x, nx) : z8;
+        const bf16x8 n1 = nx + step < i1 ? stream_ld8(a.x, nx + step) : z8;
+        one(idx, v0); one(idx + step, v1);
+        v0 = n0; v1 = n1;
+    }
+    if (idx < i1) one(idx, v0);
+}
+
+__global__ __launch_bounds__(256) void gn_apply_bwd8_kernel(const GNArgs a, const double* bstats, const void* add,
+                                                            float* dx, bf16_t* dx_bf16, int NB, int xcd, int h16) {
+    const unsigned C8 = (unsigned)a.C >> 3;
+    const unsigned total = (unsigned)NB * (unsigned)a.P * C8, per_b = (unsigned)a.P * C8;
+    unsigned i0 = blockIdx.x * blockDim.x + threadIdx.x, i1 = total, step = gridDim.x * blockDim.x;
+    if (xcd) {
+        const unsigned per = (total + gridDim.x - 1) / gridDim.x, lo = per * xcd_linear(blockIdx.x, gridDim.x);
+        i0 = lo + threadIdx.x; i1 = lo + per < total ? lo + per : total; step = blockDim.x;
+    }
+    if (i0 >= i1) return;
+    const bf16x8 z8 = {};
+    unsigned idx = i0;
+    const bool two0 = idx + step < i1;
+    bf16x8 v0 = stream_ld8(a.x, idx), g0 = stream_ld8(a.g, idx), a0 = add ? stream_ld8(add, idx) : z8;
+    bf16x8 v1 = two0 ? stream_ld8(a.x, idx + step) : z8, g1 = two0 ? stream_ld8(a.g, idx + step) : z8;
+    bf16x8 a1 = (two0 && add) ? stream_ld8(add, idx + step) : z8;
+    const int co = (int)(i0 % C8);
+    GnLane L0 = {}, L1 = {};
+    L0.ga = reinterpret_cast<const float4*>(a.gamma)[2 * co]; L1.ga = reinterpret_cast<const float4*>(a.gamma)[2 * co + 1];
+    L0.be = reinterpret_cast<const float4*>(a.beta)[2 * co]; L1.be = reinterpret_cast<const float4*>(a.beta)[2 * co + 1];
+    gn_lane_load2<true>(a, bstats, NB == 1 ? 0 : (int)(i0 / per_b), co, L0, L1);
+    auto one = [&](unsigned id, const bf16x8& v, const bf16x8& gg, const bf16x8& ad) {
+        if (NB != 1) { const int b = (int)(id / per_b); if (b != L0.b) gn_lane_load2<true>(a, bstats, b, co, L0, L1); }
+        const float4 lo = gn_bwd_quad(a, L0, op16_quad(v, 0, a.h16), op16_quad(gg, 0, a.h16), op16_quad(ad, 0, a.h16));
+        const float4 hi = gn_bwd_quad(a, L1, op16_quad(v, 1, a.h16), op16_quad(gg, 1, a.h16), op16_quad(ad, 1, a.h16));
+        if (dx) { reinterpret_cast<float4*>(dx)[2 * (size_t)id] = lo; reinterpret_cast<float4*>(dx)[2 * (size_t)id + 1] = hi; }
+        if (dx_bf16) reinterpret_cast<bf16x8*>(dx_bf16)[id] = to_op16x8(lo, hi, h16);
+    };
+    for (; idx + step < i1; idx += 2 * step) {
+        const unsigned nx = idx + 2 * step;
+        const bool m0 = nx < i1, m1 = nx + step < i1;
+        const bf16x8 nv0 = m0 ? stream_ld8(a.x, nx) : z8, ng0 = m0 ? stream_ld8(a.g, nx) : z8;
+        const bf16x8 na0 = (m0 && add) ? stream_ld8(add, nx) : z8;
+        const bf16x8 nv1 = m1 ? stream_ld8(a.x, nx + step) : z8, ng1 = m1 ? stream_ld8(a.g, nx + step) : z8;
+        const bf16x8 na1 = (m1 && add) ? stream_ld8(add, nx + step) : z8;
+        one(idx, v0, g0, a0); one(idx + step, v1, g1, a1);
+        v0 = nv0; g0 = ng0; a0 = na0; v1 = nv1; g1 = ng1; a1 = na1;
+    }
+    if (idx < i1) one(idx, v0, g0, a0);
+}
+
+bool gn_wide_ok(int wide, int s16, int NB, int P, int C, const void* p0, const void* p1, const void* p2, const void* p3, const void* p4) {
+    if (!wide || !s16 || C % 8 != 0 || C / 32 < 4 || 256 % (C / 8) != 0) return false;
+    if ((unsigned long long)NB * P * C / 8 >= (1ull << 31)) return false;
+    return (((uintptr_t)p0 | (uintptr_t)p1 | (uintptr_t)p2 | (uintptr_t)p3 | (uintptr_t)p4) & 15) == 0;
+}
+
 template <bool RAG>
 __device__ __forceinline__ bool ln_own(int i, int nv, int lane, int C) {
     return RAG ? (i * 64 + lane) * 4 < C : i < nv;
 }
-template <int MAXV, bool S16, bool RAG = false>
+template <int MAXV, bool S16, bool RAG = false, bool EMB = false>
 __global__ __launch_bounds__(256) void ln_fwd_kernel(const void* __restrict__ x, const float* __restrict__ gamma,
                                                      const float* __restrict__ beta, bf16_t* __restrict__ out_bf16,
                                                      float* __restrict__ out_f32, float* __restrict__ mean_out,
                                                      float* __restrict__ rstd_out, int rows, int C, long long ldx,
-                                                     float eps, int xcd, int h16) {
+                                                     float eps, int xcd, int h16, float* emb_x = nullptr,
+                                                     const float* __restrict__ cls = nullptr, const float* __restrict__ pos = nullptr, int T = 1) {
     const int lane = threadIdx.x & 63;
     const int row = (xcd ? xcd_linear(blockIdx.x, gridDim.x) : blockIdx.x) * 4 + (threadIdx.x >> 6);
     if (row >= rows) return;
@@ -227,7 +353,24 @@
     const size_t xr4 = (size_t)row * ldx / 4;
     float4 v[MAXV], gav[MAXV], bev[MAXV];
 #pragma unroll
-    for (int i = 0; i < MAXV; ++i) v[i] = stream_ld4<S16>(x, xr4 + (ln_own<RAG>(i, nv, lane, C) ? i * 64 + lane : (RAG ? 0 : lane)), h16);
+    for (int i = 0; i < MAXV; ++i) v[i] = stream_ld4<S16>(EMB ? emb_x : x, xr4 + (ln_own<RAG>(i, nv, lane, C) ? i * 64 + lane : (RAG ? 0 : lane)), h16);
+    if constexpr (EMB) {
+        const int t = row % T;
+        float4 pv[MAXV], cv[MAXV];
+#pragma unroll
+        for (int i = 0; i < MAXV; ++i) {
+            const int c4 = ln_own<RAG>(i, nv, lane, C) ? i * 64 + lane : (RAG ? 0 : lane);
+            pv[i] = reinterpret_cast<const float4*>(pos + (size_t)t * C)[c4];
+            cv[i] = reinterpret_cast<const float4*>(cls)[c4];
+        }
+#pragma unroll
+        for (int i = 0; i < MAXV; ++i) {
+            float4 u = make_float4(v[i].x + pv[i].x, v[i].y + pv[i].y, v[i].z + pv[i].z, v[i].w + pv[i].w);
+            if (t == 0) { u.x += cv[i].x; u.y += cv[i].y; u.z += cv[i].z; u.w += cv[i].w; }
+            v[i] = u;
+            if (ln_own<RAG>(i, nv, lane, C)) reinterpret_cast<float4*>(emb_x)[xr4 + i * 64 + lane] = u;
+        }
+    }
 #pragma unroll
     for (int i = 0; i < MAXV; ++i) {
         gav[i] = reinterpret_cast<const float4*>(gamma)[(ln_own<RAG>(i, nv, lane, C) ? i * 64 + lane : (RAG ? 0 : lane))];
@@ -328,8 +471,10 @@
 
 int prx_groupnorm_fwd(const void* x, const float* gamma, const float* beta, double* stats, bf16_t* out_bf16,
                       float* out_f32, int NB, int P, int C, int swish, float eps, hipStream_t s, int zero_stats,
-                      int stats_ready, int h16, int s16) {
+                      int stats_ready, int h16, int s16, int wide, int xcd, int* took_wide) {
     PRX_REQUIRE(C % 32 == 0 && (C / 32) % 4 == 0 && 256 % (C / 4) == 0, "groupnorm: unsupported C=%d", C);
+    if (took_wide) *took_wide = 0;
+    if (xcd < 0) xcd = prx_xcd_local();
     GNArgs a{};
     a.x = x; a.gamma = gamma; a.beta = beta; a.stats = stats; a.P = P; a.C = C; a.swish = swish; a.eps = eps; a.s16 = s16; a.h16 = h16;
     if (!stats_ready) {
@@ -342,10 +487,13 @@
     }
     if (out_bf16 || out_f32) {
         PRX_REQUIRE((unsigned long long)NB * P * C / 4 < (1ull << 31), "groupnorm: %d x %d x %d elements exceed the 32-bit index range", NB, P, C);
-        if (s16) hipLaunchKernelGGL(gn_apply_fwd_kernel<true>, dim3(gn_grid((size_t)NB * P * C / 4)), dim3(256), 0, s, a, out_bf16,
-                                    out_f32, NB, prx_xcd_local(), h16);
+        if ((unsigned long long)NB * P * C < (1ull << 23) && gn_wide_ok(wide, s16, NB, P, C, x, out_bf16, out_f32, nullptr, nullptr)) {
+            hipLaunchKernelGGL(gn_apply_fwd8_kernel, dim3(gn_grid((size_t)NB * P * C / 8)), dim3(256), 0, s, a, out_bf16, out_f32, NB, xcd, h16);
+            if (took_wide) *took_wide = 1;
+        } else if (s16) hipLaunchKernelGGL(gn_apply_fwd_kernel<true>, dim3(gn_grid((size_t)NB * P * C / 4)), dim3(256), 0, s, a, out_bf16,
+                                           out_f32, NB, xcd, h16);
         else hipLaunchKernelGGL(gn_apply_fwd_kernel<false>, dim3(gn_grid((size_t)NB * P * C / 4)), dim3(256), 0, s, a, out_bf16,
-                                out_f32, NB, prx_xcd_local(), h16);
+                                out_f32, NB, xcd, h16);
         PRX_LAUNCH_CHECK();
     }
     return 0;
@@ -366,8 +514,10 @@
 
 int prx_groupnorm_bwd(const void* g, const void* x, const float* gamma, const float* beta, const double* fstats,
                       double* bstats, const void* add, float* dx, bf16_t* dx_bf16, int NB, int P, int C, int swish,
-                      float eps, hipStream_t s, int zero_stats, int stats_ready, int h16, int s16) {
+                      float eps, hipStream_t s, int zero_stats, int stats_ready, int h16, int s16, int wide, int xcd, int* took_wide) {
     PRX_REQUIRE(256 % (C / 4) == 0 && (C / 32) % 4 == 0, "groupnorm bwd: unsupported C=%d", C);
+    if (took_wide) *took_wide = 0;
+    if (xcd < 0) xcd = prx_xcd_local();
     GNArgs a{};
     a.x = x; a.g = g; a.fstats = fstats; a.gamma = gamma; a.beta = beta; a.stats = bstats;
     a.P = P; a.C = C; a.swish = swish; a.eps = eps; a.s16 = s16; a.h16 = h16;
@@ -380,29 +530,43 @@
         PRX_LAUNCH_CHECK();
     }
     PRX_REQUIRE((unsigned long long)NB * P * C / 4 < (1ull << 31), "groupnorm bwd: %d x %d x %d elements exceed the 32-bit index range", NB, P, C);
-    if (s16) hipLaunchKernelGGL(gn_apply_bwd_kernel<true>, dim3(gn_grid((size_t)NB * P * C / 4)), dim3(256), 0, s, a, bstats, add, dx,
-                                dx_bf16, NB, prx_xcd_local(), h16);
+    if (gn_wide_ok(wide, s16, NB, P, C, x, g, add, dx, dx_bf16)) {
+        hipLaunchKernelGGL(gn_apply_bwd8_kernel, dim3(gn_grid((size_t)NB * P * C / 8)), dim3(256), 0, s, a, bstats, add, dx, dx_bf16, NB, xcd, h16);
+        if (took_wide) *took_wide = 1;
+    } else if (s16) hipLaunchKernelGGL(gn_apply_bwd_kernel<true>, dim3(gn_grid((size_t)NB * P * C / 4)), dim3(256), 0, s, a, bstats, add, dx,
+                                       dx_bf16, NB, xcd, h16);
     else hipLaunchKernelGGL(gn_apply_bwd_kernel<false>, dim3(gn_grid((size_t)NB * P * C / 4)), dim3(256), 0, s, a, bstats, add, dx,
-                            dx_bf16, NB, prx_xcd_local(), h16);
+                            dx_bf16, NB, xcd, h16);
     PRX_LAUNCH_CHECK();
     return 0;
 }
 
 int prx_layernorm_fwd(const void* x, long long ldx, const float* gamma, const float* beta, bf16_t* out_bf16,
-                      float* out_f32, float* mean, float* rstd, int rows, int C, float eps, hipStream_t s, int h16, int s16, int ragged) {
+                      float* out_f32, float* mean, float* rstd, int rows, int C, float eps, hipStream_t s, int h16, int s16, int ragged,
+                      const float* emb_cls, const float* emb_pos, int emb_T) {
     PRX_REQUIRE((C % 256 == 0 || (ragged && C % 128 == 0 && C <= 1024)) && C <= 2048 && ldx % 4 == 0,
                 "layernorm: C must be a multiple of 256 and <= 2048 (C=%d), ldx a multiple of 4", C);
     dim3 grid(ceil_div(rows, 4));
+    if (emb_pos) {
+        PRX_REQUIRE(!s16 && emb_cls && emb_T >= 1, "layernorm: the token-completing form takes fp32 rows, a class token and T >= 1");
+        float* xw = (float*)x;
+#define PRX_LN_FWD_E(MAXV, RAG) hipLaunchKernelGGL((ln_fwd_kernel<MAXV, false, RAG, true>), grid, dim3(256), 0, s, nullptr, gamma, beta, out_bf16, out_f32, \
+                                                   mean, rstd, rows, C, ldx, eps, prx_xcd_local(), h16, xw, emb_cls, emb_pos, emb_T)
+        if (C % 256 != 0) PRX_LN_FWD_E(4, true); else if (C <= 1024) PRX_LN_FWD_E(4, false); else PRX_LN_FWD_E(8, false);
+#undef PRX_LN_FWD_E
+        PRX_LAUNCH_CHECK();
+        return 0;
+    }
     if (C % 256 != 0) {
 #define PRX_LN_FWD_R(S16) hipLaunchKernelGGL((ln_fwd_kernel<4, S16, true>), grid, dim3(256), 0, s, x, gamma, beta, out_bf16, out_f32, mean, rstd, \
-                                             rows, C, ldx, eps, prx_xcd_local(), h16)
+                                             rows, C, ldx, eps, prx_xcd_local(), h16, nullptr, nullptr, nullptr, 1)
         if (s16) PRX_LN_FWD_R(true); else PRX_LN_FWD_R(false);
 #undef PRX_LN_FWD_R
         PRX_LAUNCH_CHECK();
         return 0;
     }
 #define PRX_LN_FWD(MAXV, S16) hipLaunchKernelGGL((ln_fwd_kernel<MAXV, S16>), grid, dim3(256), 0, s, x, gamma, beta, out_bf16, out_f32, mean, rstd, \
-                                                 rows, C, ldx, eps, prx_xcd_local(), h16)
+                                                 rows, C, ldx, eps, prx_xcd_local(), h16, nullptr, nullptr, nullptr, 1)
     if (C <= 1024) { if (s16) PRX_LN_FWD(4, true); else PRX_LN_FWD(4, false); }
     else { if (s16) PRX_LN_FWD(8, true); else PRX_LN_FWD(8, false); }
 #undef PRX_LN_FWD
diff --git a/pixray_amd/csrc/prompt_vq.h b/pixray_amd/csrc/prompt_vq.h
--- a/pixray_amd/csrc/prompt_vq.h
+++ b/pixray_amd/csrc/prompt_vq.h
@@ -4,6 +4,9 @@
                     float* rowloss, float* grad, float* loss, unsigned* ticket, hipStream_t s);
 int prx_l2norm_fwd(const float* e, float* out, int n, int D, hipStream_t s);
 int prx_l2norm_bwd(const float* e, const float* g, float* de, int n, int D, hipStream_t s);
+#define PRX_HEAD_BWD_MAX 65536
+int prx_l2norm_bwd_scaled(const float* e, const float* g, float* de, bf16_t* de16, int n, int D, int target_log2, float* scale2, int h16,
+                          hipStream_t s);
 int prx_sqnorm_rows(const float* w, float* out, int rows, int D, hipStream_t s);
 int prx_vq_nearest(const float* z, long long tok_stride, long long ch_stride, const float* codebook, const float* cnorm,
-                   int P, int NC, int D, float* pmin, int* pidx, int* idx_out, float* zq, hipStream_t s);
+                   int P, int NC, int D, float* pmin, int* pidx, int* idx_out, float* zq, hipStream_t s, int* idx_out2 = nullptr);
diff --git a/pixray_amd/csrc/prompt_vq.hip b/pixray_amd/csrc/prompt_vq.hip
--- a/pixray_amd/csrc/prompt_vq.hip
+++ b/pixray_amd/csrc/prompt_vq.hip
@@ -102,6 +102,78 @@
         float v = e[(size_t)i * D + c];
         de[(size_t)i * D + c] = (g[(size_t)i * D + c] - v * dot / ss) * inv;
     }
+}
+
+__global__ __launch_bounds__(1024) void l2norm_bwd_scaled_kernel(const float* __restrict__ e, const float* __restrict__ g, float* __restrict__ de,
+                                                                 bf16_t* __restrict__ de16, int n, int D, int target_log2,
+                                                                 float* __restrict__ scale2, int h16) {
+    const int lane = threadIdx.x & 63, wave = threadIdx.x >> 6;
+    float m = 0.f;
+    for (int i = wave; i < n; i += 32) {
+        const bool two = i + 16 < n;
+        const float* er[2] = {e + (size_t)i * D, e + (size_t)(two ? i + 16 : i) * D};
+        const float* gr[2] = {g + (size_t)i * D, g + (size_t)(two ? i + 16 : i) * D};
+        float ss[2] = {0.f, 0.f}, dot[2] = {0.f, 0.f};
+        for (int c0 = 0; c0 < D; c0 += 512) {
+            float ev[2][8], gv[2][8];
+#pragma unroll
+            for (int r = 0; r < 2; ++r)
+#pragma unroll
+                for (int k = 0; k < 8; ++k) { const int c = c0 + 64 * k + lane, cc = c < D ? c : 0; ev[r][k] = er[r][cc]; gv[r][k] = gr[r][cc]; }
+#pragma unroll
+            for (int r = 0; r < 2; ++r)
+#pragma unroll
+                for (int k = 0; k < 8; ++k)
+                    if (c0 + 64 * k + lane < D) { const float v = ev[r][k]; ss[r] += v * v; dot[r] += v * gv[r][k]; }
+        }
+        float inv[2];
+#pragma unroll
+        for (int r = 0; r < 2; ++r) { ss[r] = wave_sum(ss[r]); dot[r] = wave_sum(dot[r]); inv[r] = 1.f / sqrtf(ss[r]); }
+        for (int c0 = 0; c0 < D; c0 += 512) {
+            float ev[2][8], gv[2][8];
+#pragma unroll
+            for (int r = 0; r < 2; ++r)
+#pragma unroll
+                for (int k = 0; k < 8; ++k) { const int c = c0 + 64 * k + lane, cc = c < D ? c : 0; ev[r][k] = er[r][cc]; gv[r][k] = gr[r][cc]; }
+#pragma unroll
+            for (int r = 0; r < 2; ++r)
+#pragma unroll
+                for (int k = 0; k < 8; ++k) {
+                    const int c = c0 + 64 * k + lane;
+                    if (c < D && (r == 0 || two)) {
+                        float v = ev[r][k];
+                        const float d = (gv[r][k] - v * dot[r] / ss[r]) * inv[r];
+                        de[(size_t)(i + 16 * r) * D + c] = d;
+                        const float a = fabsf(d);
+                        m = fmaxf(m, a == a ? a : INFINITY);
+                    }
+                }
+        }
+    }
+    m = wave_max(m);
+    __shared__ float sm[16];
+    if (lane == 0) sm[wave] = m;
+    __syncthreads();
+    m = sm[0];
+#pragma unroll
+    for (int w = 1; w < 16; ++w) m = fmaxf(m, sm[w]);
+    const float S = grad_scale_pow2(m, target_log2);
+    if (threadIdx.x == 0) { scale2[0] = S; scale2[1] = 1.f / S; }
+    for (int i = wave; i < n; i += 16)
+        for (int c0 = 0; c0 < D; c0 += 512) {
+            float dv[8];
+#pragma unroll
+            for (int k = 0; k < 8; ++k) { const int c = c0 + 64 * k + lane; dv[k] = de[(size_t)i * D + (c < D ? c : lane < D ? lane : 0)]; }
+#pragma unroll
+            for (int k = 0; k < 8; ++k) {
+                const int c = c0 + 64 * k + lane;
+                if (c < D) {
+                    const float v = dv[k] * S;
+                    de[(size_t)i * D + c] = v;
+                    if (de16) de16[(size_t)i * D + c] = to_op16(v, h16);
+                }
+            }
+        }
 }
 
 __global__ __launch_bounds__(256) void sqnorm_rows_kernel(const float* __restrict__ w, float* __restrict__ out, int rows, int D) {
@@ -212,7 +284,8 @@
 
 __global__ __launch_bounds__(256) void vq_select_kernel(const float* __restrict__ pmin, const int* __restrict__ pidx,
                                                         int ntiles, const float* __restrict__ codebook, int D,
-                                                        int* __restrict__ idx_out, float* __restrict__ zq, int P) {
+                                                        int* __restrict__ idx_out, float* __restrict__ zq, int P,
+                                                        int* __restrict__ idx_out2) {
     const int p = blockIdx.x;
     __shared__ float sv[256];
     __shared__ int si[256];
@@ -232,6 +305,7 @@
     }
     const int sel = si[0];
     if (threadIdx.x == 0 && idx_out) idx_out[p] = sel;
+    if (threadIdx.x == 0 && idx_out2) idx_out2[p] = sel;
     for (int c = threadIdx.x; c < D; c += blockDim.x) zq[(size_t)p * D + c] = codebook[(size_t)sel * D + c];
 }
 
@@ -256,20 +330,27 @@
     PRX_LAUNCH_CHECK();
     return 0;
 }
+int prx_l2norm_bwd_scaled(const float* e, const float* g, float* de, bf16_t* de16, int n, int D, int target_log2, float* scale2, int h16,
+                          hipStream_t s) {
+    PRX_REQUIRE(n >= 1 && D >= 1 && (long long)n * D <= PRX_HEAD_BWD_MAX, "l2norm_bwd_scaled: %d x %d floats are more than one workgroup takes", n, D);
+    hipLaunchKernelGGL(l2norm_bwd_scaled_kernel, dim3(1), dim3(1024), 0, s, e, g, de, de16, n, D, target_log2, scale2, h16);
+    PRX_LAUNCH_CHECK();
+    return 0;
+}
 int prx_sqnorm_rows(const float* w, float* out, int rows, int D, hipStream_t s) {
     hipLaunchKernelGGL(sqnorm_rows_kernel, dim3(ceil_div(rows, 4)), dim3(256), 0, s, w, out, rows, D);
     PRX_LAUNCH_CHECK();
     return 0;
 }
 int prx_vq_nearest(const float* z, long long tok_stride, long long ch_stride, const float* codebook, const float* cnorm,
-                   int P, int NC, int D, float* pmin, int* pidx, int* idx_out, float* zq, hipStream_t s) {
+                   int P, int NC, int D, float* pmin, int* pidx, int* idx_out, float* zq, hipStream_t s, int* idx_out2) {
     PRX_REQUIRE(D % 16 == 0, "vq: D %% 16 != 0");
     PRX_REQUIRE(((uintptr_t)codebook & 15) == 0, "vq: the codebook must be 16-byte aligned");
     const int ntiles = ceil_div(NC, VQ_CODES);
     hipLaunchKernelGGL(vq_dist_kernel, dim3(ntiles, ceil_div(P, 64)), dim3(256), 0, s, z, tok_stride, ch_stride, codebook,
                        cnorm, P, NC, D, pmin, pidx);
     PRX_LAUNCH_CHECK();
-    hipLaunchKernelGGL(vq_select_kernel, dim3(P), dim3(256), 0, s, pmin, pidx, ntiles, codebook, D, idx_out, zq, P);
-    PRX_LAUNCH_CHECK();
-    return 0;
-}
+    hipLaunchKernelGGL(vq_select_kernel, dim3(P), dim3(256), 0, s, pmin, pidx, ntiles, codebook, D, idx_out, zq, P, idx_out2);
+    PRX_LAUNCH_CHECK();
+    return 0;
+}
diff --git a/pixray_amd/csrc/vit.hip b/pixray_amd/csrc/vit.hip
--- a/pixray_amd/csrc/vit.hip
+++ b/pixray_amd/csrc/vit.hip
@@ -151,6 +151,7 @@
     int lean;
     VitFamily fam;
     float* bp;
+    int fold;
     int cls_tail;
     float* ws; size_t ws_bytes;
     int cur_n;
@@ -207,6 +208,7 @@
     }
     { const char* e = getenv("PRX_LEAN"); v->lean = (v->h16 && !(e && atoi(e) == 0)) ? 1 : 0; }
     { const char* e = getenv("PRX_VIT_CLS_TAIL"); v->cls_tail = (e && atoi(e) == 0) ? 0 : 1; }
+    { const char* e = getenv("PRX_GLUE_FOLD"); v->fold = (e && atoi(e) == 0) ? 0 : 1; }
     v->T = T; v->max_n = max_n; v->KP = (3 * patch * patch + 7) / 8 * 8; v->cur_n = 0;
     const int W = width, KP = v->KP;
     int r;
@@ -284,7 +286,10 @@
     if (v->f32) { v->dx_bf = v->dx; v->dh_bf = v->dh; }
     else { DEV_ALLOC(m, alloc_op, v->dx_bf, R * W, f32); DEV_ALLOC(m, alloc_op, v->dh_bf, R * W, f32); }
     DEV_ALLOC(m, alloc, v->dhpost, (size_t)max_n * W); DEV_ALLOC(m, alloc, v->mm_part, 2 * 1024);
-    if (v->h16) DEV_ALLOC(m, alloc, v->gs, 2 + 64);
+    if (v->h16) {
+        DEV_ALLOC(m, alloc, v->gs, 2 + 64);
+        PRX_CHECK_HIP(hipMemsetAsync(v->gs + 2 + 63, 0, sizeof(float), s));
+    }
     v->ws_bytes = (size_t)64 << 20;
     DEV_ALLOC(m, alloc, v->ws, v->ws_bytes / sizeof(float));
     *out = guard.release();
@@ -338,9 +343,9 @@
     const int lean = v->lean;
     void* x0 = v->layers > 0 ? v->L[0].x_in : v->x_final;
     if (v->fam.ln_pre) {
-        if ((r = prx_vit_add_cls_pos(v->xpre, v->cls, v->pos, n, T, W, s))) return r;
+        if (!v->fold && (r = prx_vit_add_cls_pos(v->xpre, v->cls, v->pos, n, T, W, s))) return r;
         if ((r = prx_layernorm_fwd(v->xpre, W, v->lnpre_g, v->lnpre_b, lean ? (bf16_t*)x0 : nullptr, lean ? nullptr : (float*)x0, v->mean_pre,
-                                   v->rstd_pre, R, W, v->fam.eps, s, v->h16, 0, 1))) return r;
+                                   v->rstd_pre, R, W, v->fam.eps, s, v->h16, 0, 1, v->fold ? v->cls : nullptr, v->fold ? v->pos : nullptr, T))) return r;
     } else {
         if ((r = prx_vit_embed_tokens(v->xpre, v->cls, v->pos, x0, lean, n, T, W, s))) return r;
     }
@@ -396,11 +401,15 @@
     PRX_REQUIRE(n >= 1, "vit backward: no forward in flight on this handle");
     const int W = v->width, T = v->T, R = n * T, KP = v->KP, AW = v->aw;
     int r;
-    if ((r = prx_l2norm_bwd(v->e, d_embeds, v->de, n, v->out_dim, s))) return r;
+    const bool head1 = v->fold && v->h16 && (long long)n * v->out_dim <= PRX_HEAD_BWD_MAX;
+    if (head1) { if ((r = prx_l2norm_bwd_scaled(v->e, d_embeds, v->de, (bf16_t*)v->de16, n, v->out_dim, prx_grad_target_log2(), v->gs, v->h16, s))) return r; }
+    else if ((r = prx_l2norm_bwd(v->e, d_embeds, v->de, n, v->out_dim, s))) return r;
     {   GemmDesc d; d.A = v->de; d.a_is_f32 = 1; d.lda = v->out_dim; d.B = v->proj; d.ldb = v->out_dim;
         d.M = n; d.N = W; d.K = v->out_dim; d.out_f32 = v->dhpost; d.ldc_f32 = W;
-        if (v->h16) {
-            if ((r = prx_grad_scale(v->de, (size_t)n * v->out_dim, v->gs + 2, 64, prx_grad_target_log2(), v->gs, s))) return r;
+        if (head1) { d.A = v->de16; d.a_is_f32 = 0; }
+        else if (v->h16) {
+            if ((r = prx_grad_scale(v->de, (size_t)n * v->out_dim, v->gs + 2, v->fold ? 63 : 64, prx_grad_target_log2(), v->gs, s,
+                                    v->fold ? (unsigned*)(v->gs + 2 + 63) : nullptr))) return r;
             if ((r = prx_scale_dev(v->de, (size_t)n * v->out_dim, v->gs, s, (bf16_t*)v->de16, v->h16))) return r;
             d.A = v->de16; d.a_is_f32 = 0;
         }
@@ -428,7 +437,8 @@
             if (lean) { d.out_bf16 = v->dh_bf; d.ldc_bf16 = W; } else { d.out_f32 = v->dh; d.ldc_f32 = W; }
             if ((r = vit_gemm(v, d, s))) return r; }
         if ((r = ln_bwd_op(v, dhs, W, y.x_mid, ldt, y.ln2_g, y.mean2, y.rstd2, dxs, ldt, v->dx, ldt, v->dx_bf, rows, s, 0, lean ? 7 : 0))) return r;
-        if (tail)
+        const bool row0 = tail && v->fold && v->hp != 96 && !v->f32 && T <= 64;
+        if (tail && !row0)
             PRX_CHECK_HIP(hipMemsetAsync(v->do_, 0, op_esz(v->f32) * (size_t)R * AW, s));
         {   GemmDesc d; d.A = v->dx_bf; d.lda = ldt; d.B = y.WoT; d.ldb = W; d.M = rows; d.N = AW; d.K = W;
             d.out_bf16 = v->do_; d.ldc_bf16 = tail ? T * AW : AW;
@@ -439,7 +449,7 @@
                                            1.f / sqrtf((float)v->hd), s, v->h16))) return r;
         }
         else if (v->f32) { if ((r = prx_mha_bwd_f32((const float*)y.qkv, (const float*)y.o_save, (const float*)v->do_, y.lse, (float*)v->dqkv, n, T, AW, v->heads, s))) return r; }
-        else if (T <= 64) { if ((r = prx_mha_bwd((const bf16_t*)y.qkv, (const bf16_t*)v->do_, (bf16_t*)v->dqkv, n, T, AW, v->heads, s, v->h16))) return r; }
+        else if (T <= 64) { if ((r = prx_mha_bwd((const bf16_t*)y.qkv, (const bf16_t*)v->do_, (bf16_t*)v->dqkv, n, T, AW, v->heads, s, v->h16, row0 ? 1 : 0))) return r; }
         else { if ((r = prx_mha_bwd_gen((const bf16_t*)y.qkv, (const bf16_t*)y.o_save, (const bf16_t*)v->do_, y.lse, (bf16_t*)v->dqkv, n, T, AW, v->heads, s, v->h16))) return r; }
         {   GemmDesc d; d.A = v->dqkv; d.lda = 3 * AW; d.B = y.WqkvT; d.ldb = 3 * AW; d.M = R; d.N = W; d.K = 3 * AW;
             if (lean) { d.out_bf16 = v->dh_bf; d.ldc_bf16 = W; } else { d.out_f32 = v->dh; d.ldc_f32 = W; }
diff --git a/pixray_amd/csrc/vqgan.hip b/pixray_amd/csrc/vqgan.hip
--- a/pixray_amd/csrc/vqgan.hip
+++ b/pixray_amd/csrc/vqgan.hip
@@ -85,6 +85,8 @@
     int prec;
     int f32, h16;
     int lean;
+    int gn_wide;
+    int fold;
     float* gs;
     GemmCtx gctx;
     DevArena mem;
@@ -218,6 +220,8 @@
     v->prec = precision; v->f32 = prec_is_f32(precision); v->h16 = prec_is_h16(precision);
     v->gs = nullptr;
     { const char* e = getenv("PRX_LEAN"); v->lean = (v->h16 && !(e && atoi(e) == 0)) ? 1 : 0; }
+    { const char* e = getenv("PRX_GN_WIDE"); v->gn_wide = (e && atoi(e) == 0) ? 0 : 1; }
+    { const char* e = getenv("PRX_GLUE_FOLD"); v->fold = (e && atoi(e) == 0) ? 0 : 1; }
     v->n_gn = 0; v->zc = z_channels; v->D = embed_dim; v->NC = n_embed; v->ch = ch; v->out_ch = out_ch; v->h0 = h0; v->w0 = w0;
     WCursor cur{w, n_w, 0};
     int r;
@@ -302,7 +306,10 @@
     }
     v->ws_bytes = (size_t)64 << 20;
     DEV_ALLOC(m, alloc, v->ws, v->ws_bytes / sizeof(float));
-    if (v->h16) DEV_ALLOC(m, alloc, v->gs, 2 + 256);
+    if (v->h16) {
+        DEV_ALLOC(m, alloc, v->gs, 2 + 256);
+        PRX_CHECK_HIP(hipMemsetAsync(v->gs + 2 + 255, 0, sizeof(float), s));
+    }
     *out = guard.release();
     return 0;
 }
@@ -389,12 +396,12 @@
 }
 static int gn_fwd(PrxVqgan* v, const GN& g, const void* x, int P, int swish, hipStream_t s, bool stats_ready = false) {
     return prx_groupnorm_fwd(x, g.g, g.b, g.stats, v->f32 ? nullptr : (bf16_t*)v->a, v->f32 ? (float*)v->a : nullptr, 1, P, g.C, swish,
-                             1e-6f, s, 0, stats_ready ? 1 : 0, v->h16, v->lean);
+                             1e-6f, s, 0, stats_ready ? 1 : 0, v->h16, v->lean, v->gn_wide);
 }
 static int gn_bwd(PrxVqgan* v, const GN& g, const void* grad, const void* x, const void* add, void* dx,
                   void* dx_bf, int P, int swish, hipStream_t s, bool stats_ready = false) {
     return prx_groupnorm_bwd(grad, x, g.g, g.b, g.stats, g.bstats, add, v->lean ? nullptr : (float*)dx, v->f32 ? nullptr : (bf16_t*)dx_bf, 1, P, g.C,
-                             swish, 1e-6f, s, 0, stats_ready && fusable(v, g.C) ? 1 : 0, v->h16, v->lean);
+                             swish, 1e-6f, s, 0, stats_ready && fusable(v, g.C) ? 1 : 0, v->h16, v->lean, v->gn_wide);
 }
 
 int prx_vqgan_bounds_impl(PrxVqgan* v, float* zmin, float* zmax, hipStream_t s) {
@@ -408,8 +415,8 @@
     int r;
     PRX_CHECK_HIP(hipMemsetAsync(v->all_stats, 0, sizeof(double) * (size_t)v->n_gn * 64, s));
     if (quantize) {
-        if ((r = prx_vq_nearest(z, 1, P0, v->codebook, v->cnorm, P0, v->NC, v->D, v->pmin, v->pidx, v->idx, v->zq, s))) return r;
-        if (indices) PRX_CHECK_HIP(hipMemcpyAsync(indices, v->idx, sizeof(int) * P0, hipMemcpyDeviceToDevice, s));
+        if ((r = prx_vq_nearest(z, 1, P0, v->codebook, v->cnorm, P0, v->NC, v->D, v->pmin, v->pidx, v->idx, v->zq, s, v->fold ? indices : nullptr))) return r;
+        if (indices && !v->fold) PRX_CHECK_HIP(hipMemcpyAsync(indices, v->idx, sizeof(int) * P0, hipMemcpyDeviceToDevice, s));
     } else {
         if ((r = prx_nchw_to_nhwc(z, v->zq, nullptr, 1, v->zc, P0, v->zc, s))) return r;
     }
@@ -508,7 +515,8 @@
     int r;
     PRX_REQUIRE(v->x_last != nullptr, "vqgan backward: no forward in flight on this handle");
     PRX_CHECK_HIP(hipMemsetAsync(v->all_stats + (size_t)v->n_gn * 64, 0, sizeof(double) * (size_t)v->n_gn * 64, s));
-    if (v->h16 && (r = prx_grad_scale(g_img, (size_t)v->out_ch * PH, v->gs + 2, 256, prx_grad_target_log2(), v->gs, s))) return r;
+    if (v->h16 && (r = prx_grad_scale(g_img, (size_t)v->out_ch * PH, v->gs + 2, v->fold ? 255 : 256, prx_grad_target_log2(), v->gs, s,
+                                      v->fold ? (unsigned*)(v->gs + 2 + 255) : nullptr))) return r;
     struct GB { void* f; void* b; };
     GB g{v->g0, v->g0b}, t1{v->g1, v->g1b}, t2{v->g2, v->g2b};
     if (v->dycol) {
```

Result: no change. 166.5 (-0.3%).
